# kowaalczyk/reformer-tts

Measured on AMD Instinct MI355X. Metric: mel-frames/sec training step, LJSpeech-shape batch, higher is better.
Workload: dtype bf16; 1 GPU; config/baseline.yml full Reformer-TTS training step (enc 3 / dec 3 layers, d=512, LSH 8 rounds, buckets 64/128), per-GPU batch 12, text 200->256, mel 1024x80; global_batch=12, parallelism=dp1, reversible_recompute=full

## Files before the change

### include/rtts.h

```cpp
#ifndef RTTS_H
#define RTTS_H

#include <stdint.h>

#ifdef __cplusplus
extern "C" {
#endif

#define RTTS_VERSION 1

int rtts_version(void);
const char* rtts_last_error(void);

int rtts_lsh_hash_sort(const void* qk, int64_t ld_qk, const float* rotations, int rot_rows,
                       int B, int H, int T, int dh, int n_hashes, int bucket_size,
                       int32_t* buckets, int32_t* st, int32_t* undo, void* stream);
int rtts_lsh_hash_sort_launches(int T);

int rtts_lsh_hash_sort_hf(const void* qk, int64_t ld_qk, const float* rotations, const uint8_t* mask,
                          int B, int H, int T, int dh, int n_hashes, int chunk, int n_buckets,
                          int32_t* buckets, int32_t* st, int32_t* undo, void* stream);

int rtts_lsh_attn_fwd(const void* qk, const void* v, int64_t ld, const int32_t* st, const uint8_t* mask,
                      int B, int H, int T, int dh, int n_hashes, int bucket_size, int causal,
                      void* o, float* lse, float drop_p, uint32_t drop_seed, const uint32_t* seed_dev, void* stream);
int rtts_lsh_attn_fwd_run_length(int B, int H, int T, int n_hashes, int bucket_size);
int rtts_debug_set_walk(int fwd_run, int bwd_run);

int rtts_lsh_combine_fwd(const void* o, const float* lse, int B, int H, int T, int dh, int n_hashes,
                         void* out, int64_t ld_out, float* lse_tot, void* stream);

int rtts_lsh_bwd_qk_slots(void);
int rtts_lsh_attn_bwd_run_length(int B, int H, int T, int n_hashes, int bucket_size);
int rtts_lsh_bwd_delta(const void* out, int64_t ld_out, const void* dout, int64_t ld_dout,
                       int B, int H, int T, int dh, float* delta, void* stream);
int rtts_lsh_attn_bwd(const void* qk, const void* v, int64_t ld, const int32_t* st, const uint8_t* mask,
                      const void* dout, int64_t ld_dout, const float* lse_tot, const float* delta,
                      int B, int H, int T, int dh, int n_hashes, int bucket_size, int causal,
                      void* dqk_part, void* dv_part, uint8_t* row_flags, float drop_p, uint32_t drop_seed, const uint32_t* seed_dev,
                      void* stream);
int rtts_lsh_bwd_reduce(const void* dqk_part, const void* dv_part, int B, int H, int T, int dh, int n_hashes,
                        void* dqk, void* dv, int64_t ld_d, const uint8_t* row_flags, void* stream);

int rtts_grad_clip_scale(const float* grads, int64_t n, float grad_mult, float max_norm, float* partial_ws,
                         float* scale_out, void* stream);
int rtts_adamw_step(float* params, const float* grads, float* exp_avg, float* exp_avg_sq, const uint8_t* decay_mask,
                    int64_t n, const float* scale, const float* hyper, float beta1, float beta2, float eps,
                    float weight_decay, void* bf16_mirror, void* stream);

int rtts_ln_fwd(const float* x, const float* gamma, const float* beta, void* xn, float* mean, float* rstd,
                int M, int d, void* stream);
int rtts_ln_bwd(const void* dxn, const float* x, const float* mean, const float* rstd, const float* gamma,
                float* dx_io, float* dgamma, float* dbeta, float* partial_ws, int M, int d,
                void* dyb_next, float* partial_next, float drop_p, uint32_t seed, const uint32_t* seed_dev, void* stream);
int rtts_ln_bwd_to(const void* dxn, const float* x, const float* mean, const float* rstd, const float* gamma, const float* dx_in,
                   float* dx_out, float* dgamma, float* dbeta, float* partial_ws, int M, int d,
                   void* dyb_next, float* partial_next, float drop_p, uint32_t seed, const uint32_t* seed_dev, void* stream);
int rtts_ln_bwd_join(const void* dxn, const float* x, const float* mean, const float* rstd, const float* gamma, const float* dx_in,
                     const float* addend, float* dx_out, float* dgamma, float* dbeta, float* partial_ws, int M, int d,
                     void* dyb_next, float* partial_next, float drop_p, uint32_t seed, const uint32_t* seed_dev, void* stream);
int rtts_cast_colsum(const float* dy, void* dyb, float* dbias, float* partial_ws, int M, int d, float drop_p, uint32_t seed,
                     const uint32_t* seed_dev, const float* scale_dev, void* stream);
int rtts_colsum_bf16(void* dh, const void* h, int64_t ld, float* dbias, float* partial_ws, int M, int d,
                     int relu_gate, float gate_scale, void* gated_out, void* stream);
#define RTTS_COLSUM_MAX_GROUP 48
typedef struct {
    const float* partial;
    float* out;
    int32_t nrows, n;
    int32_t ld, reserved;
} rtts_colsum_job;
int rtts_colsum_partial_rows(int M);
int rtts_colsum_final_grouped(const rtts_colsum_job* jobs, int n, void* stream);
int rtts_residual_epilogue(const float* x, const void* g, const float* bias, float sign, float* y,
                           int64_t M, int d, float drop_p, uint32_t seed, const uint32_t* seed_dev, void* stream);
int rtts_residual_ln(float* x, const void* g, const float* bias, float sign, const float* gamma, const float* beta,
                     void* xn, float* mean, float* rstd, int M, int d, float drop_p, uint32_t seed, const uint32_t* seed_dev,
                     float* y, void* stream);
int rtts_sum_streams(const float* a, const float* b, int64_t n, float* out, void* out_bf16, void* stream);
int rtts_bias_act(void* h, const float* bias, int64_t M, int d, int relu, void* stream);
int rtts_cast_f32_bf16(const float* src, void* dst, int64_t n, void* stream);

int rtts_xattn_key_chunks(int Tk);
int rtts_xattn_fwd(const void* q, int64_t ld_q, const void* kv, int64_t ld_kv, const uint8_t* kvalid,
                   int B, int H, int Tq, int Tk, int dh, void* o, int64_t ld_o, float* lse,
                   float drop_p, uint32_t seed, const uint32_t* seed_dev, void* stream);
int rtts_xattn_bwd(const void* q, int64_t ld_q, const void* kv, int64_t ld_kv, const uint8_t* kvalid,
                   const void* dout, int64_t ld_dout, const float* lse, const float* delta,
                   int B, int H, int Tq, int Tk, int dh, void* dq, int64_t ld_dq, void* dkv_part,
                   float drop_p, uint32_t seed, const uint32_t* seed_dev, void* dq_chunks, void* stream);
int rtts_sum_slabs(const void* part, int nslabs, int64_t n, void* out, void* stream);
int rtts_xattn_probs_mean(const void* q, int64_t ld_q, const void* kv, int64_t ld_kv, const uint8_t* kvalid,
                          const float* lse, int B, int H, int Tq, int Tk, int dh, float* a, int64_t ld_a, void* stream);

int rtts_conv1d_k5(const void* x, int64_t ldx, const void* wp, int64_t ldw, int transposed, int M, int C_out, int C_in,
                   void* y, int64_t ldy, const float* bias, int out_f32, void* stream);
int rtts_to_halo(const void* src, int64_t ld_src, int64_t src_batch_stride, int C_src, int src_f32, int B, int L, int halo, int C,
                 void* dst, int lead, int64_t rows, void* stream);
int rtts_conv_w_perm(const float* w, int Co, int Ci, int CP, void* wp, void* stream);
int rtts_conv_dw_unperm(const float* dwp, int Co, int Ci, int CP, float* dw, void* stream);
#define RTTS_CONV_PERM_MAX_GROUP 8
typedef struct {
    const float* w;
    void* wp;
    int32_t Co, Ci, CP, reserved;
} rtts_conv_perm_job;
int rtts_conv_w_perm_grouped(const rtts_conv_perm_job* jobs, int n, void* stream);
int rtts_conv_dw_unperm_grouped(const rtts_conv_perm_job* jobs, int n, void* stream);
int rtts_conv1d_k5_moments(const void* x, int64_t ldx, const void* wp, int64_t ldw, int M, int C_out, int C_in, void* y, int64_t ldy,
                           int B, int L, int halo, float* partial, void* stream);
int rtts_bn_stats_from_partials(const float* partial, int nrows, int B, int L, int C, float* mean, float* rstd, float* run_mean,
                                float* run_var, const float* mean_shift, int64_t* num_batches, void* stream);
int rtts_bn_stats(const float* y, int B, int L, int halo, int C, float* mean, float* rstd, float* run_mean, float* run_var,
                  const float* mean_shift, int64_t* num_batches, float* partial_ws, void* stream);
int rtts_bn_act_fwd(const float* y, const float* mean, const float* rstd, const float* gamma, const float* beta, int act,
                    float drop_p, uint32_t seed, const uint32_t* seed_dev, int B, int L, int halo, int C, void* z, int z_halo,
                    int z_lead, int64_t z_rows, void* stream);
int rtts_bn_act_bwd(const float* y, const void* dz, int dz_halo, const float* mean, const float* rstd, const float* gamma,
                    const float* beta, int act, float drop_p, uint32_t seed, const uint32_t* seed_dev, int B, int L, int halo, int C,
                    void* dy, int dy_lead, int64_t dy_rows, float* dgamma, float* dbeta, float* partial_ws, void* stream);
int rtts_bn_moments(const float* y, int B, int L, int halo, int C, float* moments, float* partial_ws, void* stream);
int rtts_bn_from_moments(const float* moments, int64_t count, int C, float* mean, float* rstd, float* run_mean, float* run_var,
                         const float* mean_shift, int64_t* num_batches, void* stream);
int rtts_bn_act_bwd_sums(const float* y, const void* dz, int dz_halo, const float* mean, const float* rstd, const float* gamma,
                         const float* beta, int act, float drop_p, uint32_t seed, const uint32_t* seed_dev, int B, int L, int halo, int C,
                         float* sums, float* dgamma, float* dbeta, float* partial_ws, void* stream);
int rtts_bn_act_bwd_apply(const float* y, const void* dz, int dz_halo, const float* mean, const float* rstd, const float* gamma,
                          const float* beta, int act, float drop_p, uint32_t seed, const uint32_t* seed_dev, int B, int L, int halo, int C,
                          const float* sums, int64_t count, void* dy, int dy_lead, int64_t dy_rows, void* stream);
int rtts_tts_loss(const float* raw, const float* post, int64_t ld_mel, const float* tgt, const float* mask, const float* stop,
                  int64_t ld_stop, const float* tstop, int rows, int NM, int kind, float pos_weight, float w_raw, float w_post,
                  float w_stop, float* d_raw, float* d_post, int64_t ld_grad, float* d_stop, float* losses, float* partial_ws,
                  int padded_len, int valid_len, const float* res, int64_t ld_res, int halo, int dpost_lead, int64_t dpost_rows,
                  int64_t tgt_batch_stride, const int32_t* valid_len_dev, int64_t mask_batch_stride, int64_t tstop_batch_stride,
                  void* stream);
int rtts_heads_grad(const float* d_raw, const float* d_post, int dpost_lead, const float* dx0, int64_t ld_dx0, const float* d_stop,
                    int B, int L, int halo, int n_mels, int width, float* dheads, const float* scale_dev, void* stream);

#define RTTS_SEGMENTS_MAX 12
enum { RTTS_SEG_COPY_F32 = 0, RTTS_SEG_COPY_BF16 = 1, RTTS_SEG_ADD_F32 = 2, RTTS_SEG_CAST_F32_BF16 = 3 };
typedef struct {
    void* dst;
    const void* src;
    int64_t count;
    int32_t kind, reserved;
} rtts_segment;
int rtts_segments(const rtts_segment* jobs, int n, void* stream);

int rtts_pe_add(const void* y, const float* table, const float* alpha, float drop_p, uint32_t seed, const uint32_t* seed_dev,
                int T, int64_t M, int d, float* out, void* stream);
int rtts_pe_dalpha(const float* dy, const float* table, float drop_p, uint32_t seed, const uint32_t* seed_dev, int T, int64_t M,
                   int d, float* dalpha, float* partial_ws, void* stream);
int rtts_relu_drop(void* h, float drop_p, uint32_t seed, const uint32_t* seed_dev, int64_t n, void* stream);

int rtts_batch_masks(const int64_t* phonemes, int64_t ph_stride, int B, int Lp, int Lp_pad, const float* loss_mask, int64_t lm_bstride,
                     int64_t lm_rstride, int Lm, int Lm_pad, int n_mels, int64_t* pad_phonemes, uint8_t* phoneme_mask,
                     uint8_t* phoneme_pad_mask, uint8_t* frame_mask, void* stream);

int rtts_embedding_fwd(const int64_t* ids, const float* E, int rows, int C, int n_embeddings, float drop_p, uint32_t seed,
                       const uint32_t* seed_dev, float* out, void* stream);
int rtts_embedding_bwd(const int64_t* ids, const float* dx, int rows, int C, int n_embeddings, int padding_idx, float* dE,
                       float drop_p, uint32_t seed, const uint32_t* seed_dev, void* stream);
int rtts_embedding_bwd_strided(const int64_t* ids, const float* dx, int64_t batch_stride, int64_t row_stride, int L, int rows, int C,
                               int n_embeddings, int padding_idx, float* dE, float drop_p, uint32_t seed, const uint32_t* seed_dev, void* stream);

int rtts_gemm_tn(const void* a, int64_t lda, const void* b, int64_t ldb, int M, int N, int K, float* c, int64_t ldc,
                 int accumulate, float* slab_ws, int64_t slab_ws_floats, void* stream);

#define RTTS_GEMM_TN_MAX_GROUP 16
typedef struct {
    const void* a; int64_t lda;
    const void* b; int64_t ldb;
    float* c;      int64_t ldc;
    int32_t M, N, K, accumulate;
} rtts_gemm_tn_problem;
int rtts_gemm_tn_grouped(const rtts_gemm_tn_problem* problems, int n, float* slab_ws, int64_t slab_ws_floats, void* stream);

int rtts_gemm_nt(const void* a, int64_t lda, const void* w, int64_t ldw, int w_is_kn, int M, int N, int K, void* c,
                 int64_t ldc, const float* bias, int epilogue, const void* gate, int64_t ldg, float* colsum_partial,
                 void* stream);
int rtts_gemm_nt_partial_rows(int M, int N);
typedef struct {
    const void* a; int64_t lda;
    const void* w; int64_t ldw;
    void* c; int64_t ldc;
    const float* bias;
    const void* aux; int64_t ld_aux;
    float* aux_out;
    int32_t M, N, K, epilogue;
    int32_t T, H, accumulate, reserved;
} rtts_gemm_nt_problem;
#define RTTS_GEMM_NT_MAX_GROUP 4
int rtts_gemm_nt_grouped(const rtts_gemm_nt_problem* problems, int n, int w_is_kn, void* stream);
int rtts_debug_set_gemm_mode(int mode);
int64_t rtts_gemm_nt_gate_words(int M, int N);
int rtts_gemm_nt_gated(const void* a, int64_t lda, const void* w, int64_t ldw, int w_is_kn, int M, int N, int K, void* c,
                       int64_t ldc, const float* bias, int epilogue, uint64_t* gate_words, float* colsum_partial, void* stream);

int rtts_peak_copy(const void* src, void* dst, int64_t bytes, void* stream);
int rtts_comm_probe(const void* src, void* dst, int64_t bytes, int workgroups, int sleep, void* stream);
int rtts_debug_stamp(void* buf, int slot, void* stream);
int rtts_peak_mfma(float* sink, int workgroups, int iters, void* stream);

int rtts_sw_depthwise_k3(const float* x, const float* w, const float* bias, int B, int L, int C, void* y,
                         const float* edge_lo, const float* edge_hi, void* stream);
int rtts_sw_gate(const void* pw, const void* cond, int64_t ld_cond, int cond_offset, int upsample, int B, int L, int Lm, int C,
                 void* acts, void* stream);
int rtts_sw_coupling_inv(float* audio, int64_t ld_audio, const float* wn_out, int64_t rows, int half, void* stream);
int rtts_sw_depthwise_k3_seg(const float* x, const float* w, const float* bias, const int32_t* moff, int nseg, int upsample,
                             int64_t rows, int C, void* y, const float* edge_lo, const float* edge_hi, void* stream);
int rtts_sw_pack_mel(const float* mel, int64_t stride_b, int64_t stride_c, int64_t stride_t, int L, int n_mel, const int32_t* moff,
                     int nseg, int64_t rows, float* dst, int64_t ld_dst, void* stream);
int rtts_sw_coupling_inv1x1(const float* audio, int64_t ld_audio, const float* wn_out, int64_t ld_wn, const float* winv, int n,
                            int64_t rows, float* out, int64_t ld_out, void* stream);
int rtts_sw_coupling_fwd1x1(const float* x, int64_t ld_x, const float* wn_out, int64_t ld_wn, const float* w, int n_in, int n_early,
                            int64_t rows, float* out, int64_t ld_out, float* z, int64_t ld_z, int z_col, float* ls_row, void* stream);
int rtts_sw_nll_reduce(const float* z, int64_t ld_z, int C, const float* ls_row, const int32_t* moff, int nseg, int upsample, int64_t L,
                       int64_t rows, double* out, void* stream);
int rtts_sw_pack_audio(const float* src, int64_t n_src, const int64_t* start, const int32_t* moff, int nseg, int upsample, int C,
                       int64_t rows, float* dst, void* stream);
int rtts_sw_gate_bwd(const void* pw, const void* cond, int64_t ld_cond, int cond_offset, int upsample, int B, int L, int Lm, int C,
                     const void* dacts, void* dpw, void* dcond, int64_t ld_dcond, void* stream);
int rtts_sw_dwbn_bwd_partial_floats(int64_t rows, int C);
int rtts_sw_dwbn_bwd_sums(const float* h, const void* dy, const float* mean, const float* rstd, const float* gamma, const float* beta,
                          const float* w, int B, int L, int C, float* sums, float* partial_ws, void* stream);
int rtts_sw_dwbn_bwd_apply(const float* h, const void* dy, const float* mean, const float* rstd, const float* gamma, const float* beta,
                           const float* w, const float* sums, int B, int L, int C, float* dh, void* stream);
int rtts_sw_boundary_bwd_blocks(int64_t rows);
int rtts_sw_boundary_bwd(const float* x, int64_t ld_x, const float* wn_out, int64_t ld_wn, const float* w, int n_in, int n_early,
                         int64_t rows, const float* dout, int64_t ld_dout, const float* z, int64_t ld_z, int z_col, float z_scale,
                         float inv_n, float* dx, int64_t ld_dx, float* dwn, int64_t ld_dwn, float* dw, float* partial_ws, void* stream);
#define RTTS_SW_FACTOR_MAX_COUNT 16
#define RTTS_SW_FACTOR_MAX_N 128
int rtts_sw_inv1x1_factor(const float* const* w, const int* n, int count, float* const* winv, double* slogdet, void* stream);
int rtts_sw_draw_segments(const void* audio, int in_format, int64_t n_audio, const int64_t* sample_offsets, const float* mel,
                          int64_t ld_mel, const int64_t* frame_offsets, int n_utt, const int32_t* order, int n_order,
                          const int64_t* state, uint32_t seed, const int32_t* picks_in, int B, int seg_frames, int hop, int C,
                          int n_mel, float* audio_rows, float* mel_rows, int64_t ld_mel_rows, int32_t* picks_out, void* stream);
int rtts_tts_collate(const float* mel, int64_t ld_mel, const int64_t* frame_offsets, const int32_t* phoneme_ids, int64_t n_phonemes,
                     const int64_t* phoneme_offsets, int n_utt, const int32_t* ids, int B, int n_mel, int lm, int64_t* phonemes, int LP,
                     float* spectrogram_input, int R_in, int valid_in, float* spectrogram_target, int R_target, float* stop_tokens,
                     int R_stop, float* loss_mask, int R_mask, int32_t* valid_len, float noise_std, uint32_t seed, void* stream);
int rtts_infer_metrics_tiles(int lm);
int rtts_infer_metrics(const float* gen, int64_t gs_b, int64_t gs_mel, int64_t gs_t, int L, const int64_t* gen_stop, const float* truth,
                       int64_t ts_mel, int64_t ts_t, int64_t truth_frames, const int64_t* frame_offsets, int n_utt, const int32_t* ids,
                       const int64_t* starts, const int32_t* lengths, int B, int n_mel, int lm, int longest, double* partials, double* sse,
                       double* stop_err, double* totals, void* stream);

int64_t rtts_mel_frames(int64_t n_samples, int hop);
int rtts_mel_spectrogram(const float* audio, const int64_t* sample_offsets_host, const int64_t* frame_offsets_host,
                         const int64_t* sample_offsets, const int64_t* frame_offsets, int nseg, const float* dft_basis,
                         const float* mel_basis, int n_fft, int hop, int n_mels, int power, float clip, float* out, int64_t ld_out,
                         void* stream);

#define RTTS_RESAMPLE_TILE 1024
#define RTTS_RESAMPLE_MAX_TAPS 256
#define RTTS_RESAMPLE_MAX_TABLE (1 << 22)
int64_t rtts_resample_len(int64_t n_samples, int orig, int new_);
int rtts_resample(const void* audio, int in_format, int channels, const int64_t* in_offsets_host, const int64_t* out_offsets_host,
                  const int64_t* in_offsets, const int64_t* out_offsets, int nseg, const int32_t* first, const float* taps_table,
                  int orig_red, int new_red, int taps, float* out, void* stream);

#ifdef __cplusplus
}
#endif
#endif
```

### reformer-tts_amd/_lib.py

```python
from __future__ import annotations

import ctypes as C
import os

_HERE = os.path.dirname(os.path.abspath(__file__))
LIB_PATH = os.environ.get("RTTS_LIB") or os.path.join(_HERE, "lib", "librtts_hip.so")

_i64, _i32, _vp, _f32, _u32 = C.c_int64, C.c_int, C.c_void_p, C.c_float, C.c_uint32

class GemmTnProblem(C.Structure):
    _fields_ = [("a", _vp), ("lda", _i64), ("b", _vp), ("ldb", _i64), ("c", _vp), ("ldc", _i64),
                ("M", C.c_int32), ("N", C.c_int32), ("K", C.c_int32), ("accumulate", C.c_int32)]


GEMM_TN_MAX_GROUP = 16


class GemmNtProblem(C.Structure):
    _fields_ = [("a", _vp), ("lda", _i64), ("w", _vp), ("ldw", _i64), ("c", _vp), ("ldc", _i64), ("bias", _vp), ("aux", _vp),
                ("ld_aux", _i64), ("aux_out", _vp), ("M", C.c_int32), ("N", C.c_int32), ("K", C.c_int32), ("epilogue", C.c_int32),
                ("T", C.c_int32), ("H", C.c_int32), ("accumulate", C.c_int32), ("reserved", C.c_int32)]


GEMM_NT_MAX_GROUP = 4


class ColsumJob(C.Structure):
    _fields_ = [("partial", _vp), ("out", _vp), ("nrows", C.c_int32), ("n", C.c_int32), ("ld", C.c_int32), ("reserved", C.c_int32)]


COLSUM_MAX_GROUP = 48


class Segment(C.Structure):
    _fields_ = [("dst", _vp), ("src", _vp), ("count", C.c_int64), ("kind", C.c_int32), ("reserved", C.c_int32)]


SEGMENTS_MAX = 12
SEG_COPY_F32, SEG_COPY_BF16, SEG_ADD_F32, SEG_CAST_F32_BF16 = 0, 1, 2, 3


class ConvPermJob(C.Structure):
    _fields_ = [("w", _vp), ("wp", _vp), ("Co", C.c_int32), ("Ci", C.c_int32), ("CP", C.c_int32), ("reserved", C.c_int32)]


CONV_PERM_MAX_GROUP = 8
SW_FACTOR_MAX_COUNT, SW_FACTOR_MAX_N = 16, 128

SIGNATURES = {
    "rtts_lsh_hash_sort": [_vp, _i64, _vp, _i32, _i32, _i32, _i32, _i32, _i32, _i32, _vp, _vp, _vp, _vp],
    "rtts_lsh_attn_fwd": [_vp, _vp, _i64, _vp, _vp, _i32, _i32, _i32, _i32, _i32, _i32, _i32, _vp, _vp, _f32, _u32, _vp, _vp],
    "rtts_lsh_hash_sort_launches": [_i32],
    "rtts_lsh_hash_sort_hf": [_vp, _i64, _vp, _vp, _i32, _i32, _i32, _i32, _i32, _i32, _i32, _vp, _vp, _vp, _vp],
    "rtts_lsh_attn_fwd_run_length": [_i32, _i32, _i32, _i32, _i32],
    "rtts_lsh_combine_fwd": [_vp, _vp, _i32, _i32, _i32, _i32, _i32, _vp, _i64, _vp, _vp],
    "rtts_lsh_bwd_delta": [_vp, _i64, _vp, _i64, _i32, _i32, _i32, _i32, _vp, _vp],
    "rtts_lsh_attn_bwd": [_vp, _vp, _i64, _vp, _vp, _vp, _i64, _vp, _vp, _i32, _i32, _i32, _i32, _i32, _i32, _i32, _vp, _vp, _vp, _f32, _u32, _vp,
                          _vp],
    "rtts_lsh_bwd_qk_slots": [],
    "rtts_lsh_attn_bwd_run_length": [_i32, _i32, _i32, _i32, _i32],
    "rtts_debug_set_walk": [_i32, _i32],
    "rtts_lsh_bwd_reduce": [_vp, _vp, _i32, _i32, _i32, _i32, _i32, _vp, _vp, _i64, _vp, _vp],
    "rtts_grad_clip_scale": [_vp, _i64, _f32, _f32, _vp, _vp, _vp],
    "rtts_ln_fwd": [_vp, _vp, _vp, _vp, _vp, _vp, _i32, _i32, _vp],
    "rtts_ln_bwd": [_vp, _vp, _vp, _vp, _vp, _vp, _vp, _vp, _vp, _i32, _i32, _vp, _vp, _f32, _u32, _vp, _vp],
    "rtts_ln_bwd_to": [_vp, _vp, _vp, _vp, _vp, _vp, _vp, _vp, _vp, _vp, _i32, _i32, _vp, _vp, _f32, _u32, _vp, _vp],
    "rtts_ln_bwd_join": [_vp, _vp, _vp, _vp, _vp, _vp, _vp, _vp, _vp, _vp, _vp, _i32, _i32, _vp, _vp, _f32, _u32, _vp, _vp],
    "rtts_cast_colsum": [_vp, _vp, _vp, _vp, _i32, _i32, _f32, _u32, _vp, _vp, _vp],
    "rtts_colsum_bf16": [_vp, _vp, _i64, _vp, _vp, _i32, _i32, _i32, _f32, _vp, _vp],
    "rtts_sum_streams": [_vp, _vp, _i64, _vp, _vp, _vp],
    "rtts_residual_epilogue": [_vp, _vp, _vp, _f32, _vp, _i64, _i32, _f32, _u32, _vp, _vp],
    "rtts_colsum_partial_rows": [_i32],
    "rtts_colsum_final_grouped": [C.POINTER(ColsumJob), _i32, _vp],
    "rtts_residual_ln": [_vp, _vp, _vp, _f32, _vp, _vp, _vp, _vp, _vp, _i32, _i32, _f32, _u32, _vp, _vp, _vp],
    "rtts_bias_act": [_vp, _vp, _i64, _i32, _i32, _vp],
    "rtts_cast_f32_bf16": [_vp, _vp, _i64, _vp],
    "rtts_xattn_fwd": [_vp, _i64, _vp, _i64, _vp, _i32, _i32, _i32, _i32, _i32, _vp, _i64, _vp, _f32, _u32, _vp, _vp],
    "rtts_xattn_bwd": [_vp, _i64, _vp, _i64, _vp, _vp, _i64, _vp, _vp, _i32, _i32, _i32, _i32, _i32, _vp, _i64, _vp, _f32, _u32, _vp, _vp, _vp],
    "rtts_xattn_key_chunks": [_i32],
    "rtts_xattn_probs_mean": [_vp, _i64, _vp, _i64, _vp, _vp, _i32, _i32, _i32, _i32, _i32, _vp, _i64, _vp],
    "rtts_sum_slabs": [_vp, _i32, _i64, _vp, _vp],
    "rtts_conv1d_k5": [_vp, _i64, _vp, _i64, _i32, _i32, _i32, _i32, _vp, _i64, _vp, _i32, _vp],
    "rtts_to_halo": [_vp, _i64, _i64, _i32, _i32, _i32, _i32, _i32, _i32, _vp, _i32, _i64, _vp],
    "rtts_heads_grad": [_vp, _vp, _i32, _vp, _i64, _vp, _i32, _i32, _i32, _i32, _i32, _vp, _vp, _vp],
    "rtts_segments": [C.POINTER(Segment), _i32, _vp],
    "rtts_conv_w_perm": [_vp, _i32, _i32, _i32, _vp, _vp],
    "rtts_conv_dw_unperm": [_vp, _i32, _i32, _i32, _vp, _vp],
    "rtts_conv_w_perm_grouped": [C.POINTER(ConvPermJob), _i32, _vp],
    "rtts_conv_dw_unperm_grouped": [C.POINTER(ConvPermJob), _i32, _vp],
    "rtts_conv1d_k5_moments": [_vp, _i64, _vp, _i64, _i32, _i32, _i32, _vp, _i64, _i32, _i32, _i32, _vp, _vp],
    "rtts_bn_stats_from_partials": [_vp, _i32, _i32, _i32, _i32, _vp, _vp, _vp, _vp, _vp, _vp, _vp],
    "rtts_bn_stats": [_vp, _i32, _i32, _i32, _i32, _vp, _vp, _vp, _vp, _vp, _vp, _vp, _vp],
    "rtts_bn_act_fwd": [_vp, _vp, _vp, _vp, _vp, _i32, _f32, _u32, _vp, _i32, _i32, _i32, _i32, _vp, _i32, _i32, _i64, _vp],
    "rtts_bn_act_bwd": [_vp, _vp, _i32, _vp, _vp, _vp, _vp, _i32, _f32, _u32, _vp, _i32, _i32, _i32, _i32, _vp, _i32, _i64, _vp, _vp, _vp, _vp],
    "rtts_bn_moments": [_vp, _i32, _i32, _i32, _i32, _vp, _vp, _vp],
    "rtts_bn_from_moments": [_vp, _i64, _i32, _vp, _vp, _vp, _vp, _vp, _vp, _vp],
    "rtts_bn_act_bwd_sums": [_vp, _vp, _i32, _vp, _vp, _vp, _vp, _i32, _f32, _u32, _vp, _i32, _i32, _i32, _i32, _vp, _vp, _vp, _vp, _vp],
    "rtts_bn_act_bwd_apply": [_vp, _vp, _i32, _vp, _vp, _vp, _vp, _i32, _f32, _u32, _vp, _i32, _i32, _i32, _i32, _vp, _i64, _vp, _i32, _i64, _vp],
    "rtts_tts_loss": [_vp, _vp, _i64, _vp, _vp, _vp, _i64, _vp, _i32, _i32, _i32, _f32, _f32, _f32, _f32, _vp, _vp, _i64, _vp, _vp, _vp, _i32, _i32,
                      _vp, _i64, _i32, _i32, _i64, _i64, _vp, _i64, _i64, _vp],
    "rtts_pe_add": [_vp, _vp, _vp, _f32, _u32, _vp, _i32, _i64, _i32, _vp, _vp],
    "rtts_debug_stamp": [_vp, _i32, _vp],
    "rtts_batch_masks": [_vp, _i64, _i32, _i32, _i32, _vp, _i64, _i64, _i32, _i32, _i32, _vp, _vp, _vp, _vp, _vp],
    "rtts_pe_dalpha": [_vp, _vp, _f32, _u32, _vp, _i32, _i64, _i32, _vp, _vp, _vp],
    "rtts_relu_drop": [_vp, _f32, _u32, _vp, _i64, _vp],
    "rtts_embedding_bwd": [_vp, _vp, _i32, _i32, _i32, _i32, _vp, _f32, _u32, _vp, _vp],
    "rtts_embedding_bwd_strided": [_vp, _vp, _i64, _i64, _i32, _i32, _i32, _i32, _i32, _vp, _f32, _u32, _vp, _vp],
    "rtts_embedding_fwd": [_vp, _vp, _i32, _i32, _i32, _f32, _u32, _vp, _vp, _vp],
    "rtts_gemm_tn": [_vp, _i64, _vp, _i64, _i32, _i32, _i32, _vp, _i64, _i32, _vp, _i64, _vp],
    "rtts_gemm_tn_grouped": [C.POINTER(GemmTnProblem), _i32, _vp, _i64, _vp],
    "rtts_gemm_nt": [_vp, _i64, _vp, _i64, _i32, _i32, _i32, _i32, _vp, _i64, _vp, _i32, _vp, _i64, _vp, _vp],
    "rtts_gemm_nt_partial_rows": [_i32, _i32],
    "rtts_gemm_nt_grouped": [C.POINTER(GemmNtProblem), _i32, _i32, _vp],
    "rtts_debug_set_gemm_mode": [_i32],
    "rtts_gemm_nt_gate_words": [_i32, _i32],
    "rtts_gemm_nt_gated": [_vp, _i64, _vp, _i64, _i32, _i32, _i32, _i32, _vp, _i64, _vp, _i32, _vp, _vp, _vp],
    "rtts_peak_copy": [_vp, _vp, _i64, _vp],
    "rtts_comm_probe": [_vp, _vp, _i64, _i32, _i32, _vp],
    "rtts_peak_mfma": [_vp, _i32, _i32, _vp],
    "rtts_sw_depthwise_k3": [_vp, _vp, _vp, _i32, _i32, _i32, _vp, _vp, _vp, _vp],
    "rtts_sw_gate": [_vp, _vp, _i64, _i32, _i32, _i32, _i32, _i32, _i32, _vp, _vp],
    "rtts_sw_coupling_inv": [_vp, _i64, _vp, _i64, _i32, _vp],
    "rtts_sw_depthwise_k3_seg": [_vp, _vp, _vp, _vp, _i32, _i32, _i64, _i32, _vp, _vp, _vp, _vp],
    "rtts_sw_pack_mel": [_vp, _i64, _i64, _i64, _i32, _i32, _vp, _i32, _i64, _vp, _i64, _vp],
    "rtts_sw_coupling_inv1x1": [_vp, _i64, _vp, _i64, _vp, _i32, _i64, _vp, _i64, _vp],
    "rtts_sw_coupling_fwd1x1": [_vp, _i64, _vp, _i64, _vp, _i32, _i32, _i64, _vp, _i64, _vp, _i64, _i32, _vp, _vp],
    "rtts_sw_nll_reduce": [_vp, _i64, _i32, _vp, _vp, _i32, _i32, _i64, _i64, _vp, _vp],
    "rtts_sw_pack_audio": [_vp, _i64, _vp, _vp, _i32, _i32, _i32, _i64, _vp, _vp],
    "rtts_sw_gate_bwd": [_vp, _vp, _i64, _i32, _i32, _i32, _i32, _i32, _i32, _vp, _vp, _vp, _i64, _vp],
    "rtts_sw_dwbn_bwd_partial_floats": [_i64, _i32],
    "rtts_sw_dwbn_bwd_sums": [_vp, _vp, _vp, _vp, _vp, _vp, _vp, _i32, _i32, _i32, _vp, _vp, _vp],
    "rtts_sw_dwbn_bwd_apply": [_vp, _vp, _vp, _vp, _vp, _vp, _vp, _vp, _i32, _i32, _i32, _vp, _vp],
    "rtts_sw_boundary_bwd_blocks": [_i64],
    "rtts_sw_boundary_bwd": [_vp, _i64, _vp, _i64, _vp, _i32, _i32, _i64, _vp, _i64, _vp, _i64, _i32, _f32, _f32, _vp, _i64, _vp, _i64, _vp, _vp,
                             _vp],
    "rtts_sw_inv1x1_factor": [C.POINTER(_vp), C.POINTER(_i32), _i32, C.POINTER(_vp), _vp, _vp],
    "rtts_sw_draw_segments": [_vp, _i32, _i64, _vp, _vp, _i64, _vp, _i32, _vp, _i32, _vp, _u32, _vp, _i32, _i32, _i32, _i32, _i32, _vp, _vp, _i64,
                              _vp, _vp],
    "rtts_tts_collate": [_vp, _i64, _vp, _vp, _i64, _vp, _i32, _vp, _i32, _i32, _i32, _vp, _i32, _vp, _i32, _i32, _vp, _i32, _vp, _i32, _vp, _i32,
                         _vp, _f32, _u32, _vp],
    "rtts_infer_metrics_tiles": [_i32],
    "rtts_infer_metrics": [_vp, _i64, _i64, _i64, _i32, _vp, _vp, _i64, _i64, _i64, _vp, _i32, _vp, _vp, _vp, _i32, _i32, _i32, _i32, _vp, _vp, _vp,
                           _vp, _vp],
    "rtts_adamw_step": [_vp, _vp, _vp, _vp, _vp, _i64, _vp, _vp, _f32, _f32, _f32, _f32, _vp, _vp],
    "rtts_mel_frames": [_i64, _i32],
    "rtts_mel_spectrogram": [_vp, C.POINTER(_i64), C.POINTER(_i64), _vp, _vp, _i32, _vp, _vp, _i32, _i32, _i32, _i32, _f32, _vp, _i64, _vp],
    "rtts_resample_len": [_i64, _i32, _i32],
    "rtts_resample": [_vp, _i32, _i32, C.POINTER(_i64), C.POINTER(_i64), _vp, _vp, _i32, _vp, _vp, _i32, _i32, _i32, _vp, _vp],
}

_lib = None


class RttsError(RuntimeError):
    pass


_NOTED = set()
PATHS_LEFT = []


def note_general_path(where: str, reason: str) -> None:
    key = (where, reason)
    if key in _NOTED:
        return
    _NOTED.add(key)
    PATHS_LEFT.append(key)
    import logging
    logging.getLogger("reformer_tts_amd").warning("%s: general (eager) path instead of the explicit HIP executor -- %s", where, reason)


def log_once(key: str, message: str) -> None:
    if key in _NOTED:
        return
    _NOTED.add(key)
    import logging
    logging.getLogger("reformer_tts_amd").warning("%s", message)


def load() -> C.CDLL:
    global _lib
    if _lib is None:
        if not os.path.exists(LIB_PATH):
            raise RttsError(
                f"{LIB_PATH} is missing: build it with `python reformer-tts_amd/build.py` "
                "(or __graft_entry__.build()). There is no CPU fallback for the HIP path.")
        import torch
        lib = C.CDLL(LIB_PATH)
        lib.rtts_version.restype = C.c_int
        lib.rtts_last_error.restype = C.c_char_p
        for name, args in SIGNATURES.items():
            fn = getattr(lib, name)
            fn.argtypes = args
            fn.restype = C.c_int
        lib.rtts_gemm_nt_gate_words.restype = C.c_int64
        lib.rtts_mel_frames.restype = C.c_int64
        lib.rtts_resample_len.restype = C.c_int64
        _lib = lib
        fw, bw = os.environ.get("RTTS_LSH_FWD_WALK"), os.environ.get("RTTS_LSH_BWD_WALK")
        if fw is not None or bw is not None:
            _WALK[:] = [-1 if fw is None else int(fw), -1 if bw is None else int(bw)]
            lib.rtts_debug_set_walk(*_WALK)
        gs = os.environ.get("RTTS_GEMM_STORE")
        if gs is not None:
            lib.rtts_debug_set_gemm_mode(10 + int(gs))
    return _lib


_WALK = [-1, -1]


class forced_walk:

    def __init__(self, fwd=None, bwd=None):
        self.want = (fwd, bwd)

    def __enter__(self):
        self.old = list(_WALK)
        new = [o if w is None else int(w) for o, w in zip(self.old, self.want)]
        call("rtts_debug_set_walk", *new)
        _WALK[:] = new
        return self

    def __exit__(self, *exc):
        call("rtts_debug_set_walk", *self.old)
        _WALK[:] = self.old
        return False


def call(name: str, *args) -> None:
    lib = load()
    rc = getattr(lib, name)(*args)
    if rc != 0:
        raise RttsError(lib.rtts_last_error().decode() or f"{name} failed with code {rc}")
```

### reformer-tts_amd/csrc/edges.hip

```cpp
#include "rtts_common.h"

#define ED_THREADS 256
#define ED_PBLOCKS 256

#define ed_drop rtts_drop_keep

struct EdHalo {
    int B, L, P, H;
};
__device__ __forceinline__ bool ed_valid(const EdHalo& g, long long m, int& b, int& t) {
    if (m < 0 || m >= (long long)g.B * g.P) return false;
    const int mi = (int)m;
    int q = (int)((float)mi * __builtin_amdgcn_rcpf((float)g.P));
    int r = mi - q * g.P;
    if (r < 0) { --q; r += g.P; }
    if (r >= g.P) { ++q; r -= g.P; }
    b = q;
    t = r - g.H;
    return (unsigned)t < (unsigned)g.L;
}
__device__ __forceinline__ void ed_row_col(unsigned e, int C, int cshift, unsigned& row, int& c) {
    if (cshift >= 0) {
        row = e >> cshift;
        c = (int)(e & (unsigned)(C - 1));
    } else {
        row = e / (unsigned)C;
        c = (int)(e - row * (unsigned)C);
    }
}
static inline int ed_cshift(int C) { return (C & (C - 1)) == 0 ? __builtin_ctz((unsigned)C) : -1; }
__device__ __forceinline__ float ed_tanh(float x) {
    const float t = __builtin_amdgcn_exp2f(x * 2.885390081777927f);
    return 1.f - 2.f * __builtin_amdgcn_rcpf(t + 1.f);
}
static inline EdHalo ed_halo(int B, int L, int halo) { return EdHalo{B, L, L + 2 * halo, halo}; }

template <bool SRC_F32>
__global__ __launch_bounds__(ED_THREADS) void to_halo_kernel(const void* __restrict__ src, int64_t ld_src, int64_t bs_src, int C_src, EdHalo g, int C,
                                                             int lead, long long rows, bf16_t* __restrict__ dst) {
    const int pieces = C / 8;
    const size_t total = (size_t)rows * pieces;
    for (size_t i = (size_t)blockIdx.x * blockDim.x + threadIdx.x; i < total; i += (size_t)gridDim.x * blockDim.x) {
        const int pc = (int)(i % pieces);
        const long long r = (long long)(i / pieces);
        int b, t;
        uint4 o = make_uint4(0, 0, 0, 0);
        if (pc * 8 < C_src && ed_valid(g, r - lead, b, t)) {
            const size_t soff = (size_t)b * bs_src + (size_t)t * ld_src;
            if (SRC_F32) {
                const float* p = reinterpret_cast<const float*>(src) + soff + pc * 8;
                const float4 v0 = *reinterpret_cast<const float4*>(p), v1 = *reinterpret_cast<const float4*>(p + 4);
                o.x = pack_bf16x2(v0.x, v0.y); o.y = pack_bf16x2(v0.z, v0.w);
                o.z = pack_bf16x2(v1.x, v1.y); o.w = pack_bf16x2(v1.z, v1.w);
            } else {
                o = *reinterpret_cast<const uint4*>(reinterpret_cast<const bf16_t*>(src) + soff + pc * 8);
            }
        }
        *reinterpret_cast<uint4*>(dst + (size_t)r * C + pc * 8) = o;
    }
}

__global__ __launch_bounds__(ED_THREADS) void conv_w_perm_kernel(const float* __restrict__ w, int Co, int Ci, int CP, bf16_t* __restrict__ wp) {
    const size_t total = (size_t)Co * 5 * CP;
    for (size_t i = (size_t)blockIdx.x * blockDim.x + threadIdx.x; i < total; i += (size_t)gridDim.x * blockDim.x) {
        const int ci = (int)(i % CP), k = (int)((i / CP) % 5), co = (int)(i / ((size_t)CP * 5));
        wp[i] = ci < Ci ? f32_to_bf16(w[((size_t)co * Ci + ci) * 5 + k]) : (bf16_t)0;
    }
}
struct CwGroup {
    rtts_conv_perm_job j[RTTS_CONV_PERM_MAX_GROUP];
    int blk_start[RTTS_CONV_PERM_MAX_GROUP + 1];
    int n;
};
__global__ __launch_bounds__(ED_THREADS) void conv_w_perm_grouped_kernel(const CwGroup g) {
    int ji = 0;
#pragma unroll
    for (int i = 1; i < RTTS_CONV_PERM_MAX_GROUP; ++i)
        if (i < g.n && (int)blockIdx.x >= g.blk_start[i]) ji = i;
    const rtts_conv_perm_job& J = g.j[ji];
    const int Co = J.Co, Ci = J.Ci, CP = J.CP;
    const float* __restrict__ w = J.w;
    bf16_t* __restrict__ wp = (bf16_t*)J.wp;
    const size_t total = (size_t)Co * CP;
    const size_t nthr = (size_t)(g.blk_start[ji + 1] - g.blk_start[ji]) * blockDim.x;
    for (size_t i = (size_t)((int)blockIdx.x - g.blk_start[ji]) * blockDim.x + threadIdx.x; i < total; i += nthr) {
        const int ci = (int)(i % CP), co = (int)(i / CP);
        float t[5] = {0.f, 0.f, 0.f, 0.f, 0.f};
        if (ci < Ci) {
            const float* src = w + ((size_t)co * Ci + ci) * 5;
#pragma unroll
            for (int k = 0; k < 5; ++k) t[k] = src[k];
        }
#pragma unroll
        for (int k = 0; k < 5; ++k) wp[((size_t)co * 5 + k) * CP + ci] = f32_to_bf16(t[k]);
    }
}
__global__ __launch_bounds__(ED_THREADS) void conv_dw_unperm_grouped_kernel(const CwGroup g) {
    int ji = 0;
#pragma unroll
    for (int i = 1; i < RTTS_CONV_PERM_MAX_GROUP; ++i)
        if (i < g.n && (int)blockIdx.x >= g.blk_start[i]) ji = i;
    const rtts_conv_perm_job& J = g.j[ji];
    const int Co = J.Co, Ci = J.Ci, CP = J.CP;
    const float* __restrict__ dwp = J.w;
    float* __restrict__ dw = (float*)J.wp;
    const size_t total = (size_t)Co * Ci;
    const size_t nthr = (size_t)(g.blk_start[ji + 1] - g.blk_start[ji]) * blockDim.x;
    for (size_t i = (size_t)((int)blockIdx.x - g.blk_start[ji]) * blockDim.x + threadIdx.x; i < total; i += nthr) {
        const int ci = (int)(i % Ci), co = (int)(i / Ci);
        float* dst = dw + i * 5;
#pragma unroll
        for (int k = 0; k < 5; ++k) dst[k] += dwp[((size_t)co * 5 + k) * CP + ci];
    }
}
__global__ __launch_bounds__(ED_THREADS) void conv_dw_unperm_kernel(const float* __restrict__ dwp, int Co, int Ci, int CP, float* __restrict__ dw) {
    const size_t total = (size_t)Co * Ci * 5;
    for (size_t i = (size_t)blockIdx.x * blockDim.x + threadIdx.x; i < total; i += (size_t)gridDim.x * blockDim.x) {
        const int k = (int)(i % 5), ci = (int)((i / 5) % Ci), co = (int)(i / ((size_t)Ci * 5));
        dw[i] += dwp[((size_t)co * 5 + k) * CP + ci];
    }
}

template <int MODE>
__global__ __launch_bounds__(ED_THREADS) void col_partial_kernel(const float* __restrict__ y, const bf16_t* __restrict__ dz,
                                                                 const float* __restrict__ mean, const float* __restrict__ rstd,
                                                                 const float* __restrict__ gamma, const float* __restrict__ beta, int act,
                                                                 uint32_t seed, const uint32_t* __restrict__ seed_dev, uint32_t thresh, float dscale, EdHalo g,
                                                                 int dz_halo, int C, float* __restrict__ partial) {
    if (seed_dev) seed += seed_dev[0];
    const int M = g.B * g.P;
    const int cq = threadIdx.x & 63, rl = threadIdx.x >> 6;
    const int c = blockIdx.y * 256 + cq * 4;
    __shared__ float red[2][4][256];
    float sa[4] = {0, 0, 0, 0}, sb[4] = {0, 0, 0, 0};
    if (c < C) {
        float mu[4] = {0, 0, 0, 0}, rs[4] = {1, 1, 1, 1}, ga[4] = {1, 1, 1, 1}, be[4] = {0, 0, 0, 0};
        if (MODE == 1) {
#pragma unroll
            for (int j = 0; j < 4; ++j) { mu[j] = mean[c + j]; rs[j] = rstd[c + j]; ga[j] = gamma[c + j]; be[j] = beta[c + j]; }
        }
        for (int row = blockIdx.x * 4 + rl; row < M; row += gridDim.x * 4) {
            int sb_, st_;
            if (!ed_valid(g, row, sb_, st_)) continue;
            const float4 yv = *reinterpret_cast<const float4*>(y + (size_t)row * C + c);
            const float yy[4] = {yv.x, yv.y, yv.z, yv.w};
            if (MODE == 0) {
#pragma unroll
                for (int j = 0; j < 4; ++j) { sa[j] += yy[j]; sb[j] = __builtin_fmaf(yy[j], yy[j], sb[j]); }
            } else {
                const size_t drow = dz_halo ? (size_t)row : (size_t)sb_ * g.L + st_;
                const uint2 dv = *reinterpret_cast<const uint2*>(dz + drow * C + c);
                const float dd[4] = {__uint_as_float(dv.x << 16), __uint_as_float(dv.x & 0xffff0000u), __uint_as_float(dv.y << 16),
                                     __uint_as_float(dv.y & 0xffff0000u)};
#pragma unroll
                for (int j = 0; j < 4; ++j) {
                    const float yh = (yy[j] - mu[j]) * rs[j];
                    const float pre = __builtin_fmaf(yh, ga[j], be[j]);
                    float da;
                    if (act == 1) da = pre > 0.f ? 1.f : 0.f;
                    else { const float th = ed_tanh(pre); da = 1.f - th * th; }
                    const float g = dd[j] * da * (thresh ? ed_drop(seed, (uint32_t)((size_t)row * C + c + j), thresh, dscale) : 1.f);
                    sa[j] += g;
                    sb[j] = __builtin_fmaf(g, yh, sb[j]);
                }
            }
        }
    }
#pragma unroll
    for (int j = 0; j < 4; ++j) { red[0][rl][cq * 4 + j] = sa[j]; red[1][rl][cq * 4 + j] = sb[j]; }
    __syncthreads();
    const int t = threadIdx.x;
    if (blockIdx.y * 256 + t < C) {
        float* prow = partial + (size_t)blockIdx.x * 2 * C;
        prow[blockIdx.y * 256 + t] = (red[0][0][t] + red[0][1][t]) + (red[0][2][t] + red[0][3][t]);
        prow[C + blockIdx.y * 256 + t] = (red[1][0][t] + red[1][1][t]) + (red[1][2][t] + red[1][3][t]);
    }
}

#define ED_FIN_WAVES 16
__device__ __forceinline__ void ed_reduce_partials(const float* __restrict__ partial, int nrows, int C, int c, float& s, float& q,
                                                   float (*red)[ED_FIN_WAVES][64]) {
    const int lane = threadIdx.x & 63, wave = threadIdx.x >> 6;
    float a = 0.f, b = 0.f;
    if (c < C) {
        float va[16], vb[16];
        for (int r0 = wave; r0 < nrows; r0 += ED_FIN_WAVES * 16) {
#pragma unroll
            for (int u = 0; u < 16; ++u) {
                const int r = r0 + u * ED_FIN_WAVES;
                va[u] = r < nrows ? partial[(size_t)r * 2 * C + c] : 0.f;
                vb[u] = r < nrows ? partial[(size_t)r * 2 * C + C + c] : 0.f;
            }
#pragma unroll
            for (int u = 0; u < 16; ++u) {
                a += va[u];
                b += vb[u];
            }
        }
    }
    red[0][wave][lane] = a;
    red[1][wave][lane] = b;
    __syncthreads();
    s = 0.f;
    q = 0.f;
#pragma unroll
    for (int w = 0; w < ED_FIN_WAVES; ++w) {
        s += red[0][w][lane];
        q += red[1][w][lane];
    }
}

__global__ __launch_bounds__(64 * ED_FIN_WAVES) void bn_finalize_stats_kernel(const float* __restrict__ partial, int nrows, int M, int C,
                                                                       float* __restrict__ mean, float* __restrict__ rstd,
                                                                       float* __restrict__ run_mean, float* __restrict__ run_var,
                                                                       const float* __restrict__ mean_shift, long long* __restrict__ num_batches) {
    __shared__ float red[2][ED_FIN_WAVES][64];
    const int c = blockIdx.x * 64 + (threadIdx.x & 63);
    float s, q;
    ed_reduce_partials(partial, nrows, C, c, s, q, red);
    if (num_batches && blockIdx.x == 0 && threadIdx.x == 0) num_batches[0] += 1;
    if (threadIdx.x >= 64 || c >= C) return;
    const float mu = s / M;
    const float var = fmaxf(q / M - mu * mu, 0.f);
    mean[c] = mu;
    rstd[c] = rsqrtf(var + 1e-5f);
    if (run_mean) {
        run_mean[c] = 0.9f * run_mean[c] + 0.1f * (mu + (mean_shift ? mean_shift[c] : 0.f));
        run_var[c] = 0.9f * run_var[c] + 0.1f * var * ((float)M / (float)(M > 1 ? M - 1 : 1));
    }
}

__global__ __launch_bounds__(64 * ED_FIN_WAVES) void bn_finalize_bwd_kernel(const float* __restrict__ partial, int nrows, int C,
                                                                     float* __restrict__ sums, float* __restrict__ dgamma,
                                                                     float* __restrict__ dbeta) {
    __shared__ float red[2][ED_FIN_WAVES][64];
    const int c = blockIdx.x * 64 + (threadIdx.x & 63);
    float s, q;
    ed_reduce_partials(partial, nrows, C, c, s, q, red);
    if (threadIdx.x >= 64 || c >= C) return;
    sums[c] = s;
    sums[C + c] = q;
    dbeta[c] += s;
    dgamma[c] += q;
}

__global__ __launch_bounds__(64 * ED_FIN_WAVES) void bn_moments_kernel(const float* __restrict__ partial, int nrows, int C, float* __restrict__ moments) {
    __shared__ float red[2][ED_FIN_WAVES][64];
    const int c = blockIdx.x * 64 + (threadIdx.x & 63);
    float s, q;
    ed_reduce_partials(partial, nrows, C, c, s, q, red);
    if (threadIdx.x >= 64 || c >= C) return;
    moments[c] = s;
    moments[C + c] = q;
}
__global__ void bn_from_moments_kernel(const float* __restrict__ moments, float count, int C, float* __restrict__ mean, float* __restrict__ rstd,
                                       float* __restrict__ run_mean, float* __restrict__ run_var, const float* __restrict__ mean_shift,
                                       long long* __restrict__ num_batches) {
    const int c = blockIdx.x * blockDim.x + threadIdx.x;
    if (num_batches && c == 0) num_batches[0] += 1;
    if (c >= C) return;
    if (count <= 0.f) count = moments[2 * C];
    const float mu = moments[c] / count;
    const float var = fmaxf(moments[C + c] / count - mu * mu, 0.f);
    mean[c] = mu;
    rstd[c] = rsqrtf(var + 1e-5f);
    if (run_mean) {
        run_mean[c] = 0.9f * run_mean[c] + 0.1f * (mu + (mean_shift ? mean_shift[c] : 0.f));
        run_var[c] = 0.9f * run_var[c] + 0.1f * var * (count / (count > 1.f ? count - 1.f : 1.f));
    }
}

__global__ __launch_bounds__(ED_THREADS) void bn_act_fwd_kernel(const float* __restrict__ y, const float* __restrict__ mean,
                                                                const float* __restrict__ rstd, const float* __restrict__ gamma,
                                                                const float* __restrict__ beta, int act, uint32_t seed, const uint32_t* __restrict__ seed_dev,
                                                                uint32_t thresh, float dscale, EdHalo g, int z_halo, int z_lead, size_t n4, int C,
                                                                int cshift, bf16_t* __restrict__ z) {
    if (seed_dev) seed += seed_dev[0];
    for (size_t i = (size_t)blockIdx.x * blockDim.x + threadIdx.x; i < n4; i += (size_t)gridDim.x * blockDim.x) {
        unsigned zrow;
        int c;
        ed_row_col((unsigned)i * 4u, C, cshift, zrow, c);
        const long long zr = (long long)zrow;
        long long ym;
        bool ok = true;
        if (z_halo) {
            int b, t;
            ym = zr - z_lead;
            ok = ed_valid(g, ym, b, t);
        } else {
            const long long b = zr / g.L;
            ym = b * g.P + g.H + (zr - b * g.L);
        }
        uint2 pk = make_uint2(0u, 0u);
        if (ok) {
            const size_t e = (size_t)ym * C + c;
            const float4 yv = *reinterpret_cast<const float4*>(y + e);
            const float yy[4] = {yv.x, yv.y, yv.z, yv.w};
            const float4 m4 = *reinterpret_cast<const float4*>(mean + c), r4 = *reinterpret_cast<const float4*>(rstd + c);
            const float4 g4 = *reinterpret_cast<const float4*>(gamma + c), b4 = *reinterpret_cast<const float4*>(beta + c);
            const float mu[4] = {m4.x, m4.y, m4.z, m4.w}, rs[4] = {r4.x, r4.y, r4.z, r4.w};
            const float ga[4] = {g4.x, g4.y, g4.z, g4.w}, be[4] = {b4.x, b4.y, b4.z, b4.w};
            float o[4];
#pragma unroll
            for (int j = 0; j < 4; ++j) {
                const float pre = __builtin_fmaf((yy[j] - mu[j]) * rs[j], ga[j], be[j]);
                float a = act == 1 ? fmaxf(pre, 0.f) : ed_tanh(pre);
                if (thresh) a *= ed_drop(seed, (uint32_t)(e + j), thresh, dscale);
                o[j] = a;
            }
            pk.x = pack_bf16x2(o[0], o[1]);
            pk.y = pack_bf16x2(o[2], o[3]);
        }
        reinterpret_cast<uint2*>(z)[i] = pk;
    }
}

__global__ __launch_bounds__(ED_THREADS) void bn_act_bwd_apply_kernel(const float* __restrict__ y, const bf16_t* __restrict__ dz,
                                                                      const float* __restrict__ mean, const float* __restrict__ rstd,
                                                                      const float* __restrict__ gamma, const float* __restrict__ beta, int act,
                                                                      uint32_t seed, const uint32_t* __restrict__ seed_dev, uint32_t thresh, float dscale,
                                                                      const float* __restrict__ sums, float inv_m, EdHalo g, int dz_halo, int dy_lead,
                                                                      size_t n4, int C, int cshift, bf16_t* __restrict__ dy) {
    if (seed_dev) seed += seed_dev[0];
    if (inv_m < 0.f) inv_m = 1.f / sums[2 * C];
    for (size_t i = (size_t)blockIdx.x * blockDim.x + threadIdx.x; i < n4; i += (size_t)gridDim.x * blockDim.x) {
        unsigned drow_;
        int c;
        ed_row_col((unsigned)i * 4u, C, cshift, drow_, c);
        const long long ym = (long long)drow_ - dy_lead;
        int b, t;
        uint2 pk = make_uint2(0u, 0u);
        if (ed_valid(g, ym, b, t)) {
            const size_t e = (size_t)ym * C + c;
            const float4 yv = *reinterpret_cast<const float4*>(y + e);
            const size_t drow = dz_halo ? (size_t)ym : (size_t)b * g.L + t;
            const uint2 dv = *reinterpret_cast<const uint2*>(dz + drow * C + c);
            const float yy[4] = {yv.x, yv.y, yv.z, yv.w};
            const float dd[4] = {__uint_as_float(dv.x << 16), __uint_as_float(dv.x & 0xffff0000u), __uint_as_float(dv.y << 16),
                                 __uint_as_float(dv.y & 0xffff0000u)};
            const float4 m4 = *reinterpret_cast<const float4*>(mean + c), r4 = *reinterpret_cast<const float4*>(rstd + c);
            const float4 g4 = *reinterpret_cast<const float4*>(gamma + c), b4 = *reinterpret_cast<const float4*>(beta + c);
            const float4 s0 = *reinterpret_cast<const float4*>(sums + c), s1 = *reinterpret_cast<const float4*>(sums + C + c);
            const float mu4[4] = {m4.x, m4.y, m4.z, m4.w}, rs4[4] = {r4.x, r4.y, r4.z, r4.w};
            const float ga4[4] = {g4.x, g4.y, g4.z, g4.w}, be4[4] = {b4.x, b4.y, b4.z, b4.w};
            const float sa4[4] = {s0.x, s0.y, s0.z, s0.w}, sb4[4] = {s1.x, s1.y, s1.z, s1.w};
            float o[4];
#pragma unroll
            for (int j = 0; j < 4; ++j) {
                const float rs = rs4[j], ga = ga4[j];
                const float yh = (yy[j] - mu4[j]) * rs;
                const float pre = __builtin_fmaf(yh, ga, be4[j]);
                float da;
                if (act == 1) da = pre > 0.f ? 1.f : 0.f;
                else { const float th = ed_tanh(pre); da = 1.f - th * th; }
                const float gg = dd[j] * da * (thresh ? ed_drop(seed, (uint32_t)(e + j), thresh, dscale) : 1.f);
                o[j] = ga * rs * (gg - sa4[j] * inv_m - yh * sb4[j] * inv_m);
            }
            pk.x = pack_bf16x2(o[0], o[1]);
            pk.y = pack_bf16x2(o[2], o[3]);
        }
        reinterpret_cast<uint2*>(dy)[i] = pk;
    }
}

__global__ __launch_bounds__(ED_THREADS) void tts_loss_kernel(const float* __restrict__ raw, const float* __restrict__ post, int64_t ld_mel,
                                                              const float* __restrict__ tgt, const float* __restrict__ mask,
                                                              const float* __restrict__ stop, int64_t ld_stop, const float* __restrict__ tstop,
                                                              int rows, int NM, int kind, float pos_weight, float w_raw, float w_post,
                                                              float w_stop, float* __restrict__ d_raw, float* __restrict__ d_post,
                                                              int64_t ld_grad, float* __restrict__ d_stop, float* __restrict__ partial,
                                                              int Lp, int Lv, const float* __restrict__ res, int64_t ld_res, int hp, int dp_lead,
                                                              long long dp_rows, long long tgt_bs, const int* __restrict__ lv_dev,
                                                              long long mask_bs, long long tstop_bs, int vec4) {
    if (lv_dev) Lv = min(max(lv_dev[0], 1), Lv);
    const int PH = Lp + 2 * hp;
    float s_raw = 0.f, s_post = 0.f, s_stop = 0.f;
    const size_t nel = (size_t)rows * NM;
    const size_t vrows = (size_t)(rows / Lp) * Lv;
    const float inv_el = 1.f / ((float)vrows * NM), inv_rows = 1.f / (float)vrows;
    if (vec4) {
        const unsigned NQ = (unsigned)NM / 4, nq = (unsigned)rows * NQ;
        for (unsigned i = blockIdx.x * blockDim.x + threadIdx.x; i < nq; i += gridDim.x * blockDim.x) {
            const unsigned row = i / NQ, c = (i % NQ) * 4;
            const unsigned t = row % (unsigned)Lp, bi = row / (unsigned)Lp;
            const size_t hrow = (size_t)bi * PH + hp + t;
            const size_t prow = (size_t)dp_lead + hrow;
            float4 gr = make_float4(0.f, 0.f, 0.f, 0.f), gp = gr;
            if ((int)t < Lv) {
                const float4 mk = *reinterpret_cast<const float4*>(mask + (size_t)bi * mask_bs + (size_t)t * NM + c);
                const float4 tg = *reinterpret_cast<const float4*>(tgt + (size_t)bi * tgt_bs + (size_t)t * NM + c);
                const float4 rv = *reinterpret_cast<const float4*>(raw + (size_t)row * ld_mel + c);
                float4 pv;
                if (res) {
                    const float4 rs = *reinterpret_cast<const float4*>(res + hrow * ld_res + c);
                    pv = make_float4(rv.x + rs.x, rv.y + rs.y, rv.z + rs.z, rv.w + rs.w);
                } else {
                    pv = *reinterpret_cast<const float4*>(post + (size_t)row * ld_mel + c);
                }
                const float mkv[4] = {mk.x, mk.y, mk.z, mk.w}, tgv[4] = {tg.x, tg.y, tg.z, tg.w};
                const float rvv[4] = {rv.x, rv.y, rv.z, rv.w}, pvv[4] = {pv.x, pv.y, pv.z, pv.w};
                float grv[4], gpv[4];
#pragma unroll
                for (int e = 0; e < 4; ++e) {
                    const float r = rvv[e] * mkv[e] - tgv[e], p = pvv[e] * mkv[e] - tgv[e];
                    if (kind == 0) {
                        s_raw = __builtin_fmaf(r, r, s_raw);
                        s_post = __builtin_fmaf(p, p, s_post);
                        grv[e] = w_raw * 2.f * r * mkv[e] * inv_el;
                        gpv[e] = w_post * 2.f * p * mkv[e] * inv_el;
                    } else {
                        s_raw += fabsf(r);
                        s_post += fabsf(p);
                        grv[e] = w_raw * (r > 0.f ? 1.f : (r < 0.f ? -1.f : 0.f)) * mkv[e] * inv_el;
                        gpv[e] = w_post * (p > 0.f ? 1.f : (p < 0.f ? -1.f : 0.f)) * mkv[e] * inv_el;
                    }
                }
                gr = make_float4(grv[0], grv[1], grv[2], grv[3]);
                gp = make_float4(gpv[0], gpv[1], gpv[2], gpv[3]);
            }
            *reinterpret_cast<float4*>(d_raw + (size_t)row * ld_grad + c) = gr;
            *reinterpret_cast<float4*>(d_post + prow * ld_grad + c) = gp;
        }
    } else
    for (size_t i = (size_t)blockIdx.x * blockDim.x + threadIdx.x; i < nel; i += (size_t)gridDim.x * blockDim.x) {
        const size_t row = i / NM;
        const int c = (int)(i % NM);
        const int t = (int)(row % Lp);
        const size_t hrow = (row / Lp) * PH + hp + t;
        const size_t prow = (size_t)dp_lead + hrow;
        if (t >= Lv) {
            d_raw[row * ld_grad + c] = 0.f;
            d_post[prow * ld_grad + c] = 0.f;
            continue;
        }
        const float mk = mask[(row / Lp) * (size_t)mask_bs + (size_t)t * NM + c], tg = tgt[(row / Lp) * (size_t)tgt_bs + (size_t)t * NM + c];
        const float rv = raw[row * ld_mel + c];
        const float pv = res ? rv + res[hrow * ld_res + c] : post[row * ld_mel + c];
        const float r = rv * mk - tg, p = pv * mk - tg;
        if (kind == 0) {
            s_raw = __builtin_fmaf(r, r, s_raw);
            s_post = __builtin_fmaf(p, p, s_post);
            d_raw[row * ld_grad + c] = w_raw * 2.f * r * mk * inv_el;
            d_post[prow * ld_grad + c] = w_post * 2.f * p * mk * inv_el;
        } else {
            s_raw += fabsf(r);
            s_post += fabsf(p);
            d_raw[row * ld_grad + c] = w_raw * (r > 0.f ? 1.f : (r < 0.f ? -1.f : 0.f)) * mk * inv_el;
            d_post[prow * ld_grad + c] = w_post * (p > 0.f ? 1.f : (p < 0.f ? -1.f : 0.f)) * mk * inv_el;
        }
    }
    const int npad = (int)ld_grad - NM;
    for (size_t i = (size_t)blockIdx.x * blockDim.x + threadIdx.x; i < (size_t)rows * npad; i += (size_t)gridDim.x * blockDim.x) {
        const size_t row = i / npad;
        const int c = NM + (int)(i % npad);
        d_raw[row * ld_grad + c] = 0.f;
        d_post[((size_t)dp_lead + (row / Lp) * PH + hp + row % Lp) * ld_grad + c] = 0.f;
    }
    if (hp > 0) {
        const EdHalo g{rows / Lp, Lp, PH, hp};
        for (size_t i = (size_t)blockIdx.x * blockDim.x + threadIdx.x; i < (size_t)dp_rows * ld_grad; i += (size_t)gridDim.x * blockDim.x) {
            int b, t;
            if (!ed_valid(g, (long long)(i / ld_grad) - dp_lead, b, t)) d_post[i] = 0.f;
        }
    }
    for (size_t i = (size_t)blockIdx.x * blockDim.x + threadIdx.x; i < (size_t)rows; i += (size_t)gridDim.x * blockDim.x) {
        const int tt = (int)(i % Lp);
        if (tt >= Lv) {
            d_stop[i] = 0.f;
            continue;
        }
        const float x = stop[i * ld_stop], t = tstop[(i / Lp) * (size_t)tstop_bs + tt];
        const float lw = 1.f + (pos_weight - 1.f) * t;
        const float sp = fmaxf(-x, 0.f) + log1pf(expf(-fabsf(x)));
        s_stop += (1.f - t) * x + lw * sp;
        const float sig = 1.f / (1.f + expf(-x));
        d_stop[i] = w_stop * ((1.f - t) - lw * (1.f - sig)) * inv_rows;
    }
    __shared__ float red[3][ED_THREADS / 64];
#pragma unroll
    for (int o = 32; o > 0; o >>= 1) {
        s_raw += __shfl_xor(s_raw, o);
        s_post += __shfl_xor(s_post, o);
        s_stop += __shfl_xor(s_stop, o);
    }
    if ((threadIdx.x & 63) == 0) {
        red[0][threadIdx.x >> 6] = s_raw;
        red[1][threadIdx.x >> 6] = s_post;
        red[2][threadIdx.x >> 6] = s_stop;
    }
    __syncthreads();
    if (threadIdx.x < 3) partial[blockIdx.x * 3 + threadIdx.x] = red[threadIdx.x][0] + red[threadIdx.x][1] + red[threadIdx.x][2] + red[threadIdx.x][3];
}

__global__ void tts_loss_finalize_kernel(const float* __restrict__ partial, int nblocks, float inv_el, float inv_rows, float w_raw,
                                         float w_post, float w_stop, float* __restrict__ losses, const int* __restrict__ lv_dev, int batch,
                                         int Lv, int NM) {
    if (lv_dev) {
        const float vrows = (float)batch * (float)min(max(lv_dev[0], 1), Lv);
        inv_el = 1.f / (vrows * NM);
        inv_rows = 1.f / vrows;
    }
    float a = 0.f, b = 0.f, c = 0.f;
    for (int i = threadIdx.x; i < nblocks; i += 64) { a += partial[i * 3]; b += partial[i * 3 + 1]; c += partial[i * 3 + 2]; }
#pragma unroll
    for (int o = 32; o > 0; o >>= 1) {
        a += __shfl_xor(a, o);
        b += __shfl_xor(b, o);
        c += __shfl_xor(c, o);
    }
    if (threadIdx.x != 0) return;
    a *= inv_el; b *= inv_el; c *= inv_rows;
    losses[0] = w_raw * a + w_post * b + w_stop * c;
    losses[1] = a; losses[2] = b; losses[3] = c;
}

__global__ __launch_bounds__(ED_THREADS) void heads_grad_kernel(const float* __restrict__ d_raw, const float* __restrict__ d_post, int dp_lead,
                                                                const float* __restrict__ dx0, int64_t ld_dx0, const float* __restrict__ d_stop,
                                                                EdHalo g, int NM, int W, float* __restrict__ out,
                                                                const float* __restrict__ scale_dev) {
    const float up = scale_dev ? scale_dev[0] : 1.f;
    const size_t total = (size_t)g.B * g.L * (W / 4);
    for (size_t i = (size_t)blockIdx.x * blockDim.x + threadIdx.x; i < total; i += (size_t)gridDim.x * blockDim.x) {
        const int c = (int)(i % (W / 4)) * 4;
        const size_t row = i / (W / 4);
        const size_t hrow = (row / g.L) * g.P + g.H + row % g.L;
        const float4 a = *reinterpret_cast<const float4*>(d_raw + row * W + c);
        const float4 b = *reinterpret_cast<const float4*>(d_post + ((size_t)dp_lead + hrow) * W + c);
        float o[4] = {(a.x + b.x) * up, (a.y + b.y) * up, (a.z + b.z) * up, (a.w + b.w) * up};
#pragma unroll
        for (int j = 0; j < 4; ++j) {
            if (c + j < NM) o[j] += dx0[hrow * ld_dx0 + c + j];
            else if (c + j == NM) o[j] = d_stop[row] * up;
        }
        *reinterpret_cast<float4*>(out + row * W + c) = make_float4(o[0], o[1], o[2], o[3]);
    }
}

__global__ __launch_bounds__(ED_THREADS) void embedding_bwd_kernel(const int64_t* __restrict__ ids, const float* __restrict__ dx, int64_t bstride,
                                                                   int64_t rstride, int L, int rows,
                                                                   int C, int padding_idx, float* __restrict__ dE, uint32_t seed,
                                                                   const uint32_t* __restrict__ seed_dev, uint32_t thresh, float dscale) {
    __shared__ float red[4][64];
    const int id = blockIdx.x;
    const int lane = threadIdx.x & 63, wave = threadIdx.x >> 6;
    const int c = blockIdx.y * 64 + lane;
    if (id == padding_idx) return;
    if (thresh && seed_dev) seed += seed_dev[0];
    float acc = 0.f;
    for (int base = wave * 64; base < rows; base += 4 * 64) {
        const int r = base + lane;
        unsigned long long m = __ballot(r < rows && ids[r] == (int64_t)id);
        while (m) {
            const int rr = base + __builtin_ctzll(m);
            m &= m - 1;
            const int bb = rr / L;
            if (c < C) acc += dx[(size_t)bb * bstride + (size_t)(rr - bb * L) * rstride + c] * (thresh ? rtts_drop_keep(seed, (uint32_t)rr * C + c, thresh, dscale) : 1.f);
        }
    }
    red[wave][lane] = acc;
    __syncthreads();
    if (wave == 0 && c < C) dE[(size_t)id * C + c] += (red[0][lane] + red[1][lane]) + (red[2][lane] + red[3][lane]);
}

__global__ __launch_bounds__(ED_THREADS) void embedding_fwd_kernel(const int64_t* __restrict__ ids, const float* __restrict__ E, size_t n4, int C,
                                                                   int n_emb, uint32_t seed, const uint32_t* __restrict__ seed_dev, uint32_t thresh,
                                                                   float dscale, float* __restrict__ out) {
    if (thresh && seed_dev) seed += seed_dev[0];
    for (size_t i = (size_t)blockIdx.x * blockDim.x + threadIdx.x; i < n4; i += (size_t)gridDim.x * blockDim.x) {
        const size_t e = i * 4, row = e / C;
        const int c = (int)(e % C);
        long long id = ids[row];
        id = id < 0 ? 0 : (id >= n_emb ? n_emb - 1 : id);
        float4 v = *reinterpret_cast<const float4*>(E + (size_t)id * C + c);
        if (thresh) {
            v.x *= rtts_drop_keep(seed, (uint32_t)e, thresh, dscale);
            v.y *= rtts_drop_keep(seed, (uint32_t)e + 1, thresh, dscale);
            v.z *= rtts_drop_keep(seed, (uint32_t)e + 2, thresh, dscale);
            v.w *= rtts_drop_keep(seed, (uint32_t)e + 3, thresh, dscale);
        }
        reinterpret_cast<float4*>(out)[i] = v;
    }
}

struct SgJob {
    void* dst;
    const void* src;
    long long count;
    int kind, blk_start;
};
struct SgGroup {
    SgJob j[RTTS_SEGMENTS_MAX];
    int n;
};
__global__ __launch_bounds__(ED_THREADS) void segments_kernel(const SgGroup grp) {
    int ji = 0;
#pragma unroll 1
    for (int i = 1; i < grp.n; ++i)
        if ((int)blockIdx.x >= grp.j[i].blk_start) ji = i;
    const SgJob& J = grp.j[ji];
    const int nblk = (ji + 1 < grp.n ? grp.j[ji + 1].blk_start : (int)gridDim.x) - J.blk_start;
    for (long long i = (long long)((int)blockIdx.x - J.blk_start) * ED_THREADS + threadIdx.x; i < J.count; i += (long long)nblk * ED_THREADS) {
        switch (J.kind) {
        case RTTS_SEG_COPY_F32: reinterpret_cast<float*>(J.dst)[i] = reinterpret_cast<const float*>(J.src)[i]; break;
        case RTTS_SEG_COPY_BF16: reinterpret_cast<bf16_t*>(J.dst)[i] = reinterpret_cast<const bf16_t*>(J.src)[i]; break;
        case RTTS_SEG_ADD_F32: reinterpret_cast<float*>(J.dst)[i] += reinterpret_cast<const float*>(J.src)[i]; break;
        default: reinterpret_cast<bf16_t*>(J.dst)[i] = f32_to_bf16(reinterpret_cast<const float*>(J.src)[i]); break;
        }
    }
}

__global__ __launch_bounds__(ED_THREADS) void pe_add_kernel(const bf16_t* __restrict__ y, const float* __restrict__ table,
                                                            const float* __restrict__ alpha, uint32_t seed, const uint32_t* __restrict__ seed_dev,
                                                            uint32_t thresh, float dscale, int T, size_t n4, int d, float* __restrict__ out) {
    if (seed_dev) seed += seed_dev[0];
    const float a = alpha[0];
    for (size_t i = (size_t)blockIdx.x * blockDim.x + threadIdx.x; i < n4; i += (size_t)gridDim.x * blockDim.x) {
        const size_t e = i * 4;
        const int c = (int)(e % d);
        const int t = (int)((e / d) % T);
        const uint2 yv = reinterpret_cast<const uint2*>(y)[i];
        const float4 tv = *reinterpret_cast<const float4*>(table + (size_t)t * d + c);
        const float tt[4] = {tv.x, tv.y, tv.z, tv.w};
        const float yy[4] = {__uint_as_float(yv.x << 16), __uint_as_float(yv.x & 0xffff0000u), __uint_as_float(yv.y << 16),
                             __uint_as_float(yv.y & 0xffff0000u)};
        float o[4];
#pragma unroll
        for (int j = 0; j < 4; ++j)
            o[j] = yy[j] + a * tt[j] * (thresh ? ed_drop(seed, (uint32_t)(t * d + c + j), thresh, dscale) : 1.f);
        reinterpret_cast<float4*>(out)[i] = make_float4(o[0], o[1], o[2], o[3]);
    }
}

__global__ __launch_bounds__(ED_THREADS) void pe_dalpha_partial_kernel(const float* __restrict__ dy, const float* __restrict__ table,
                                                                       uint32_t seed, const uint32_t* __restrict__ seed_dev, uint32_t thresh, float dscale, int T,
                                                                       size_t n4, int d, float* __restrict__ partial) {
    if (seed_dev) seed += seed_dev[0];
    float s = 0.f;
    for (size_t i = (size_t)blockIdx.x * blockDim.x + threadIdx.x; i < n4; i += (size_t)gridDim.x * blockDim.x) {
        const size_t e = i * 4;
        const int c = (int)(e % d);
        const int t = (int)((e / d) % T);
        const float4 dv = reinterpret_cast<const float4*>(dy)[i];
        const float4 tv = *reinterpret_cast<const float4*>(table + (size_t)t * d + c);
        const float dd[4] = {dv.x, dv.y, dv.z, dv.w}, tt[4] = {tv.x, tv.y, tv.z, tv.w};
#pragma unroll
        for (int j = 0; j < 4; ++j)
            s = __builtin_fmaf(dd[j], tt[j] * (thresh ? ed_drop(seed, (uint32_t)(t * d + c + j), thresh, dscale) : 1.f), s);
    }
    __shared__ float red[ED_THREADS / 64];
#pragma unroll
    for (int o = 32; o > 0; o >>= 1) s += __shfl_xor(s, o);
    if ((threadIdx.x & 63) == 0) red[threadIdx.x >> 6] = s;
    __syncthreads();
    if (threadIdx.x == 0) partial[blockIdx.x] = (red[0] + red[1]) + (red[2] + red[3]);
}
__global__ void pe_dalpha_final_kernel(const float* __restrict__ partial, int n, float* __restrict__ dalpha) {
    float s = 0.f;
    for (int i = threadIdx.x; i < n; i += 64) s += partial[i];
#pragma unroll
    for (int o = 32; o > 0; o >>= 1) s += __shfl_xor(s, o);
    if (threadIdx.x == 0) dalpha[0] += s;
}

__global__ __launch_bounds__(ED_THREADS) void relu_drop_kernel(bf16_t* __restrict__ h, uint32_t seed, const uint32_t* __restrict__ seed_dev,
                                                               uint32_t thresh, float dscale, size_t n8) {
    if (seed_dev) seed += seed_dev[0];
    for (size_t i = (size_t)blockIdx.x * blockDim.x + threadIdx.x; i < n8; i += (size_t)gridDim.x * blockDim.x) {
        uint4 t = reinterpret_cast<uint4*>(h)[i];
        uint32_t u[4] = {t.x, t.y, t.z, t.w};
#pragma unroll
        for (int j = 0; j < 4; ++j) {
            float lo = fmaxf(__uint_as_float(u[j] << 16), 0.f), hi = fmaxf(__uint_as_float(u[j] & 0xffff0000u), 0.f);
            if (thresh) {
                lo *= ed_drop(seed, (uint32_t)(i * 8 + 2 * j), thresh, dscale);
                hi *= ed_drop(seed, (uint32_t)(i * 8 + 2 * j + 1), thresh, dscale);
            }
            u[j] = pack_bf16x2(lo, hi);
        }
        t.x = u[0]; t.y = u[1]; t.z = u[2]; t.w = u[3];
        reinterpret_cast<uint4*>(h)[i] = t;
    }
}

static inline unsigned ed_grid(size_t items) {
    size_t b = (items + ED_THREADS - 1) / ED_THREADS;
    if (b > 4096) b = 4096;
    if (b < 1) b = 1;
    return (unsigned)b;
}
static inline uint32_t ed_thresh(float p) { return p <= 0.f ? 0u : (uint32_t)((double)p * 4294967296.0); }

extern "C" int rtts_to_halo(const void* src, int64_t ld_src, int64_t src_batch_stride, int C_src, int src_f32, int B, int L, int halo, int C,
                            void* dst, int lead, int64_t rows, void* stream) {
    RTTS_ENTER(stream);
    RTTS_REQUIRE(src && dst && B > 0 && L > 0 && halo >= 0 && C > 0 && C % 8 == 0 && C_src > 0 && C_src % 8 == 0 && C_src <= C && ld_src >= C_src &&
                     ld_src % (src_f32 ? 4 : 8) == 0, "rtts_to_halo: bad arguments");
    if (src_batch_stride == 0) src_batch_stride = (int64_t)L * ld_src;
    RTTS_REQUIRE(src_batch_stride >= (int64_t)L * ld_src && src_batch_stride % (src_f32 ? 4 : 8) == 0,
                 "rtts_to_halo: src_batch_stride must cover L rows and keep 16-byte alignment");
    RTTS_REQUIRE(lead >= 0 && rows >= lead + (int64_t)B * (L + 2 * halo), "rtts_to_halo: dst has %lld rows, needs %lld", (long long)rows,
                 (long long)(lead + (int64_t)B * (L + 2 * halo)));
    const dim3 grid(ed_grid((size_t)rows * (C / 8)));
    if (src_f32)
        hipLaunchKernelGGL(to_halo_kernel<true>, grid, dim3(ED_THREADS), 0, (hipStream_t)stream, src, ld_src, src_batch_stride, C_src, ed_halo(B, L, halo), C,
                           lead, (long long)rows, (bf16_t*)dst);
    else
        hipLaunchKernelGGL(to_halo_kernel<false>, grid, dim3(ED_THREADS), 0, (hipStream_t)stream, src, ld_src, src_batch_stride, C_src, ed_halo(B, L, halo), C,
                           lead, (long long)rows, (bf16_t*)dst);
    RTTS_LAUNCH_CHECK("rtts_to_halo");
    return 0;
}

extern "C" int rtts_heads_grad(const float* d_raw, const float* d_post, int dpost_lead, const float* dx0, int64_t ld_dx0, const float* d_stop,
                               int B, int L, int halo, int n_mels, int width, float* dheads, const float* scale_dev, void* stream) {
    RTTS_ENTER(stream);
    RTTS_REQUIRE(d_raw && d_post && dx0 && d_stop && dheads && B > 0 && L > 0 && halo >= 0 && width % 4 == 0 && n_mels < width && dpost_lead >= 0,
                 "rtts_heads_grad: bad arguments");
    hipLaunchKernelGGL(heads_grad_kernel, dim3(ed_grid((size_t)B * L * (width / 4))), dim3(ED_THREADS), 0, (hipStream_t)stream, d_raw, d_post,
                       dpost_lead, dx0, ld_dx0, d_stop, ed_halo(B, L, halo), n_mels, width, dheads, scale_dev);
    RTTS_LAUNCH_CHECK("rtts_heads_grad");
    return 0;
}

extern "C" int rtts_conv_w_perm(const float* w, int Co, int Ci, int CP, void* wp, void* stream) {
    RTTS_ENTER(stream);
    RTTS_REQUIRE(w && wp && Co > 0 && Ci > 0 && CP >= Ci, "rtts_conv_w_perm: bad arguments");
    hipLaunchKernelGGL(conv_w_perm_kernel, dim3(ed_grid((size_t)Co * 5 * CP)), dim3(ED_THREADS), 0, (hipStream_t)stream, w, Co, Ci, CP, (bf16_t*)wp);
    RTTS_LAUNCH_CHECK("rtts_conv_w_perm");
    return 0;
}

extern "C" int rtts_conv_w_perm_grouped(const rtts_conv_perm_job* jobs, int n, void* stream) {
    RTTS_ENTER(stream);
    RTTS_REQUIRE(jobs && n > 0 && n <= RTTS_CONV_PERM_MAX_GROUP, "rtts_conv_w_perm_grouped: 1..%d jobs", RTTS_CONV_PERM_MAX_GROUP);
    CwGroup g;
    g.n = n;
    int blk = 0;
    for (int i = 0; i < n; ++i) {
        RTTS_REQUIRE(jobs[i].w && jobs[i].wp && jobs[i].Co > 0 && jobs[i].Ci > 0 && jobs[i].CP >= jobs[i].Ci, "rtts_conv_w_perm_grouped: bad job %d", i);
        g.j[i] = jobs[i];
        g.blk_start[i] = blk;
        blk += (int)ed_grid((size_t)jobs[i].Co * jobs[i].CP);
    }
    for (int i = n; i <= RTTS_CONV_PERM_MAX_GROUP; ++i) g.blk_start[i] = blk;
    hipLaunchKernelGGL(conv_w_perm_grouped_kernel, dim3(blk), dim3(ED_THREADS), 0, (hipStream_t)stream, g);
    RTTS_LAUNCH_CHECK("rtts_conv_w_perm_grouped");
    return 0;
}

extern "C" int rtts_conv_dw_unperm_grouped(const rtts_conv_perm_job* jobs, int n, void* stream) {
    RTTS_ENTER(stream);
    RTTS_REQUIRE(jobs && n > 0 && n <= RTTS_CONV_PERM_MAX_GROUP, "rtts_conv_dw_unperm_grouped: 1..%d jobs", RTTS_CONV_PERM_MAX_GROUP);
    CwGroup g;
    g.n = n;
    int blk = 0;
    for (int i = 0; i < n; ++i) {
        RTTS_REQUIRE(jobs[i].w && jobs[i].wp && jobs[i].Co > 0 && jobs[i].Ci > 0 && jobs[i].CP >= jobs[i].Ci, "rtts_conv_dw_unperm_grouped: bad job %d", i);
        g.j[i] = jobs[i];
        g.blk_start[i] = blk;
        blk += (int)ed_grid((size_t)jobs[i].Co * jobs[i].Ci);
    }
    for (int i = 1; i < n; ++i)
        for (int k = 0; k < i; ++k)
            RTTS_REQUIRE((const float*)jobs[i].wp >= (const float*)jobs[k].wp + (size_t)jobs[k].Co * jobs[k].Ci * 5 ||
                             (const float*)jobs[k].wp >= (const float*)jobs[i].wp + (size_t)jobs[i].Co * jobs[i].Ci * 5,
                         "rtts_conv_dw_unperm_grouped: jobs %d and %d add into overlapping gradients (launch them one after the other)", k, i);
    for (int i = n; i <= RTTS_CONV_PERM_MAX_GROUP; ++i) g.blk_start[i] = blk;
    hipLaunchKernelGGL(conv_dw_unperm_grouped_kernel, dim3(blk), dim3(ED_THREADS), 0, (hipStream_t)stream, g);
    RTTS_LAUNCH_CHECK("rtts_conv_dw_unperm_grouped");
    return 0;
}

extern "C" int rtts_conv_dw_unperm(const float* dwp, int Co, int Ci, int CP, float* dw, void* stream) {
    RTTS_ENTER(stream);
    RTTS_REQUIRE(dwp && dw && Co > 0 && Ci > 0 && CP >= Ci, "rtts_conv_dw_unperm: bad arguments");
    hipLaunchKernelGGL(conv_dw_unperm_kernel, dim3(ed_grid((size_t)Co * Ci * 5)), dim3(ED_THREADS), 0, (hipStream_t)stream, dwp, Co, Ci, CP, dw);
    RTTS_LAUNCH_CHECK("rtts_conv_dw_unperm");
    return 0;
}

static inline dim3 ed_col_grid(int M, int C) {
    int slabs = (M + 3) / 4;
    if (slabs > ED_PBLOCKS) slabs = ED_PBLOCKS;
    return dim3(slabs, (C + 255) / 256);
}

extern "C" int rtts_bn_stats(const float* y, int B, int L, int halo, int C, float* mean, float* rstd, float* run_mean, float* run_var,
                             const float* mean_shift, int64_t* num_batches, float* partial_ws, void* stream) {
    RTTS_ENTER(stream);
    RTTS_REQUIRE(y && mean && rstd && partial_ws && B > 0 && L > 0 && halo >= 0 && C > 0 && C % 4 == 0, "rtts_bn_stats: bad arguments");
    const EdHalo g = ed_halo(B, L, halo);
    const dim3 grid = ed_col_grid(B * g.P, C);
    hipLaunchKernelGGL((col_partial_kernel<0>), grid, dim3(ED_THREADS), 0, (hipStream_t)stream, y, (const bf16_t*)nullptr, (const float*)nullptr,
                       (const float*)nullptr, (const float*)nullptr, (const float*)nullptr, 0, 0u, (const uint32_t*)nullptr, 0u, 1.f, g, 1, C,
                       partial_ws);
    hipLaunchKernelGGL(bn_finalize_stats_kernel, dim3((C + 63) / 64), dim3(64 * ED_FIN_WAVES), 0, (hipStream_t)stream, partial_ws,
                       (int)grid.x, B * L, C, mean, rstd, run_mean, run_var, mean_shift, (long long*)num_batches);
    RTTS_LAUNCH_CHECK("rtts_bn_stats");
    return 0;
}

extern "C" int rtts_bn_stats_from_partials(const float* partial, int nrows, int B, int L, int C, float* mean, float* rstd, float* run_mean,
                                           float* run_var, const float* mean_shift, int64_t* num_batches, void* stream) {
    RTTS_ENTER(stream);
    RTTS_REQUIRE(partial && mean && rstd && nrows > 0 && B > 0 && L > 0 && C > 0 && C % 4 == 0, "rtts_bn_stats_from_partials: bad arguments");
    hipLaunchKernelGGL(bn_finalize_stats_kernel, dim3((C + 63) / 64), dim3(64 * ED_FIN_WAVES), 0, (hipStream_t)stream, partial, nrows, B * L, C, mean,
                       rstd, run_mean, run_var, mean_shift, (long long*)num_batches);
    RTTS_LAUNCH_CHECK("rtts_bn_stats_from_partials");
    return 0;
}

extern "C" int rtts_bn_act_fwd(const float* y, const float* mean, const float* rstd, const float* gamma, const float* beta, int act,
                               float drop_p, uint32_t seed, const uint32_t* seed_dev, int B, int L, int halo, int C, void* z, int z_halo,
                               int z_lead, int64_t z_rows, void* stream) {
    RTTS_ENTER(stream);
    RTTS_REQUIRE(y && mean && rstd && gamma && beta && z && B > 0 && L > 0 && halo >= 0 && C % 4 == 0 && (act == 1 || act == 2) && drop_p >= 0.f &&
                     drop_p < 1.f, "rtts_bn_act_fwd: bad arguments");
    const EdHalo g = ed_halo(B, L, halo);
    RTTS_REQUIRE(z_halo ? (halo > 0 && z_lead >= 0 && z_rows >= z_lead + (int64_t)B * g.P) : (z_rows == (int64_t)B * L && z_lead == 0),
                 "rtts_bn_act_fwd: z must be a halo array with room for B*(L+2*halo) rows behind its lead-in, or B*L plain rows");
    const size_t n4 = (size_t)z_rows * C / 4;
    RTTS_REQUIRE(n4 < (1ull << 30), "rtts_bn_act_fwd: more than 2^32 elements");
    hipLaunchKernelGGL(bn_act_fwd_kernel, dim3(ed_grid(n4)), dim3(ED_THREADS), 0, (hipStream_t)stream, y, mean, rstd, gamma, beta, act, seed, seed_dev,
                       ed_thresh(drop_p), 1.f / (1.f - drop_p), g, z_halo, z_lead, n4, C, ed_cshift(C), (bf16_t*)z);
    RTTS_LAUNCH_CHECK("rtts_bn_act_fwd");
    return 0;
}

extern "C" int rtts_bn_act_bwd(const float* y, const void* dz, int dz_halo, const float* mean, const float* rstd, const float* gamma,
                               const float* beta, int act, float drop_p, uint32_t seed, const uint32_t* seed_dev, int B, int L, int halo, int C,
                               void* dy, int dy_lead, int64_t dy_rows, float* dgamma, float* dbeta, float* partial_ws, void* stream) {
    RTTS_ENTER(stream);
    RTTS_REQUIRE(y && dz && mean && rstd && gamma && beta && dy && dgamma && dbeta && partial_ws && B > 0 && L > 0 && halo >= 0 && C % 4 == 0 &&
                     (act == 1 || act == 2), "rtts_bn_act_bwd: bad arguments");
    RTTS_REQUIRE(drop_p >= 0.f && drop_p < 1.f, "rtts_bn_act_bwd: drop_p must be in [0, 1)");
    const EdHalo g = ed_halo(B, L, halo);
    RTTS_REQUIRE(dy_lead >= 0 && dy_rows >= dy_lead + (int64_t)B * g.P,
                 "rtts_bn_act_bwd: dy needs room for B*(L+2*halo) rows behind its lead-in");
    const size_t n4 = (size_t)dy_rows * C / 4;
    RTTS_REQUIRE(n4 < (1ull << 30), "rtts_bn_act_bwd: more than 2^32 elements");
    const dim3 grid = ed_col_grid(B * g.P, C);
    const uint32_t th = ed_thresh(drop_p);
    const float ds = 1.f / (1.f - drop_p);
    float* sums = partial_ws + (size_t)ED_PBLOCKS * 2 * C;
    const int dzh = (halo > 0 && dz_halo) ? 1 : 0;
    hipLaunchKernelGGL((col_partial_kernel<1>), grid, dim3(ED_THREADS), 0, (hipStream_t)stream, y, (const bf16_t*)dz, mean, rstd, gamma, beta, act,
                       seed, seed_dev, th, ds, g, dzh, C, partial_ws);
    hipLaunchKernelGGL(bn_finalize_bwd_kernel, dim3((C + 63) / 64), dim3(64 * ED_FIN_WAVES), 0, (hipStream_t)stream, partial_ws,
                       (int)grid.x, C, sums, dgamma, dbeta);
    hipLaunchKernelGGL(bn_act_bwd_apply_kernel, dim3(ed_grid(n4)), dim3(ED_THREADS), 0, (hipStream_t)stream, y, (const bf16_t*)dz, mean, rstd,
                       gamma, beta, act, seed, seed_dev, th, ds, sums, 1.f / (float)((size_t)B * L), g, dzh, dy_lead, n4, C, ed_cshift(C), (bf16_t*)dy);
    RTTS_LAUNCH_CHECK("rtts_bn_act_bwd");
    return 0;
}

extern "C" int rtts_bn_moments(const float* y, int B, int L, int halo, int C, float* moments, float* partial_ws, void* stream) {
    RTTS_ENTER(stream);
    RTTS_REQUIRE(y && moments && partial_ws && B > 0 && L > 0 && halo >= 0 && C > 0 && C % 4 == 0, "rtts_bn_moments: bad arguments");
    const EdHalo g = ed_halo(B, L, halo);
    const dim3 grid = ed_col_grid(B * g.P, C);
    hipLaunchKernelGGL((col_partial_kernel<0>), grid, dim3(ED_THREADS), 0, (hipStream_t)stream, y, (const bf16_t*)nullptr, (const float*)nullptr,
                       (const float*)nullptr, (const float*)nullptr, (const float*)nullptr, 0, 0u, (const uint32_t*)nullptr, 0u, 1.f, g, 1, C,
                       partial_ws);
    hipLaunchKernelGGL(bn_moments_kernel, dim3((C + 63) / 64), dim3(64 * ED_FIN_WAVES), 0, (hipStream_t)stream, partial_ws, (int)grid.x, C, moments);
    RTTS_LAUNCH_CHECK("rtts_bn_moments");
    return 0;
}

extern "C" int rtts_bn_from_moments(const float* moments, int64_t count, int C, float* mean, float* rstd, float* run_mean, float* run_var,
                                    const float* mean_shift, int64_t* num_batches, void* stream) {
    RTTS_ENTER(stream);
    RTTS_REQUIRE(moments && mean && rstd && count >= 0 && C > 0, "rtts_bn_from_moments: bad arguments");
    hipLaunchKernelGGL(bn_from_moments_kernel, dim3((C + 255) / 256), dim3(256), 0, (hipStream_t)stream, moments, (float)count, C, mean, rstd,
                       run_mean, run_var, mean_shift, (long long*)num_batches);
    RTTS_LAUNCH_CHECK("rtts_bn_from_moments");
    return 0;
}

extern "C" int rtts_bn_act_bwd_sums(const float* y, const void* dz, int dz_halo, const float* mean, const float* rstd, const float* gamma,
                                    const float* beta, int act, float drop_p, uint32_t seed, const uint32_t* seed_dev, int B, int L, int halo,
                                    int C, float* sums, float* dgamma, float* dbeta, float* partial_ws, void* stream) {
    RTTS_ENTER(stream);
    RTTS_REQUIRE(y && dz && mean && rstd && gamma && beta && sums && dgamma && dbeta && partial_ws && B > 0 && L > 0 && halo >= 0 && C % 4 == 0 &&
                     (act == 1 || act == 2), "rtts_bn_act_bwd_sums: bad arguments");
    RTTS_REQUIRE(drop_p >= 0.f && drop_p < 1.f, "rtts_bn_act_bwd_sums: drop_p must be in [0, 1)");
    const EdHalo g = ed_halo(B, L, halo);
    const dim3 grid = ed_col_grid(B * g.P, C);
    const int dzh = (halo > 0 && dz_halo) ? 1 : 0;
    hipLaunchKernelGGL((col_partial_kernel<1>), grid, dim3(ED_THREADS), 0, (hipStream_t)stream, y, (const bf16_t*)dz, mean, rstd, gamma, beta, act,
                       seed, seed_dev, ed_thresh(drop_p), 1.f / (1.f - drop_p), g, dzh, C, partial_ws);
    hipLaunchKernelGGL(bn_finalize_bwd_kernel, dim3((C + 63) / 64), dim3(64 * ED_FIN_WAVES), 0, (hipStream_t)stream, partial_ws,
                       (int)grid.x, C, sums, dgamma, dbeta);
    RTTS_LAUNCH_CHECK("rtts_bn_act_bwd_sums");
    return 0;
}

extern "C" int rtts_bn_act_bwd_apply(const float* y, const void* dz, int dz_halo, const float* mean, const float* rstd, const float* gamma,
                                     const float* beta, int act, float drop_p, uint32_t seed, const uint32_t* seed_dev, int B, int L, int halo,
                                     int C, const float* sums, int64_t count, void* dy, int dy_lead, int64_t dy_rows, void* stream) {
    RTTS_ENTER(stream);
    RTTS_REQUIRE(y && dz && mean && rstd && gamma && beta && sums && dy && count >= 0 && B > 0 && L > 0 && halo >= 0 && C % 4 == 0 &&
                     (act == 1 || act == 2), "rtts_bn_act_bwd_apply: bad arguments");
    RTTS_REQUIRE(drop_p >= 0.f && drop_p < 1.f, "rtts_bn_act_bwd_apply: drop_p must be in [0, 1)");
    const EdHalo g = ed_halo(B, L, halo);
    RTTS_REQUIRE(dy_lead >= 0 && dy_rows >= dy_lead + (int64_t)B * g.P, "rtts_bn_act_bwd_apply: dy needs room for B*(L+2*halo) rows behind its lead-in");
    const int dzh = (halo > 0 && dz_halo) ? 1 : 0;
    const size_t n4 = (size_t)dy_rows * C / 4;
    RTTS_REQUIRE(n4 < (1ull << 30), "rtts_bn_act_bwd_apply: more than 2^32 elements");
    hipLaunchKernelGGL(bn_act_bwd_apply_kernel, dim3(ed_grid(n4)), dim3(ED_THREADS), 0, (hipStream_t)stream, y, (const bf16_t*)dz, mean, rstd,
                       gamma, beta, act, seed, seed_dev, ed_thresh(drop_p), 1.f / (1.f - drop_p), sums, count > 0 ? 1.f / (float)count : -1.f, g, dzh,
                       dy_lead, n4, C, ed_cshift(C), (bf16_t*)dy);
    RTTS_LAUNCH_CHECK("rtts_bn_act_bwd_apply");
    return 0;
}

extern "C" int rtts_tts_loss(const float* raw, const float* post, int64_t ld_mel, const float* tgt, const float* mask, const float* stop,
                             int64_t ld_stop, const float* tstop, int rows, int NM, int kind, float pos_weight, float w_raw, float w_post,
                             float w_stop, float* d_raw, float* d_post, int64_t ld_grad, float* d_stop, float* losses, float* partial_ws,
                             int padded_len, int valid_len, const float* res, int64_t ld_res, int halo, int dpost_lead, int64_t dpost_rows,
                             int64_t tgt_batch_stride, const int32_t* valid_len_dev, int64_t mask_batch_stride, int64_t tstop_batch_stride,
                             void* stream) {
    RTTS_ENTER(stream);
    RTTS_REQUIRE(raw && (post || res) && tgt && mask && stop && tstop && d_raw && d_post && d_stop && losses && partial_ws && rows > 0 && NM > 0 &&
                     ld_grad >= NM, "rtts_tts_loss: bad arguments");
    RTTS_REQUIRE(padded_len > 0 && valid_len > 0 && valid_len <= padded_len && rows % padded_len == 0,
                 "rtts_tts_loss: rows must be batch * padded_len and 0 < valid_len <= padded_len");
    RTTS_REQUIRE(kind == 0 || kind == 1, "rtts_tts_loss: Unsupported loss type: %d", kind);
    RTTS_REQUIRE(res ? (halo > 0 && ld_res >= NM && dpost_lead >= 0 &&
                        dpost_rows >= dpost_lead + (int64_t)(rows / padded_len) * (padded_len + 2 * halo))
                     : (halo == 0 && dpost_lead == 0),
                 "rtts_tts_loss: res / d_post in halo rows need halo > 0 and room for B*(L+2*halo) rows; without res: halo = lead = 0");
    if (tgt_batch_stride == 0) tgt_batch_stride = (int64_t)valid_len * NM;
    RTTS_REQUIRE(tgt_batch_stride >= (int64_t)valid_len * NM, "rtts_tts_loss: tgt_batch_stride below valid_len * NM");
    if (mask_batch_stride == 0) mask_batch_stride = (int64_t)valid_len * NM;
    if (tstop_batch_stride == 0) tstop_batch_stride = valid_len;
    RTTS_REQUIRE(mask_batch_stride >= (int64_t)valid_len * NM && tstop_batch_stride >= valid_len,
                 "rtts_tts_loss: mask / tstop batch strides below valid_len rows");
    const int blocks = 512;
    const uintptr_t bits = (uintptr_t)raw | (uintptr_t)post | (uintptr_t)res | (uintptr_t)tgt | (uintptr_t)mask | (uintptr_t)d_raw | (uintptr_t)d_post;
    const int vec4 = NM % 4 == 0 && (bits & 15) == 0 && ld_mel % 4 == 0 && ld_grad % 4 == 0 && (!res || ld_res % 4 == 0) &&
                     tgt_batch_stride % 4 == 0 && mask_batch_stride % 4 == 0 && (int64_t)rows * (NM / 4) < (1ll << 31);
    hipLaunchKernelGGL(tts_loss_kernel, dim3(blocks), dim3(ED_THREADS), 0, (hipStream_t)stream, raw, post, ld_mel, tgt, mask, stop, ld_stop,
                       tstop, rows, NM, kind, pos_weight, w_raw, w_post, w_stop, d_raw, d_post, ld_grad, d_stop, partial_ws, padded_len,
                       valid_len, res, ld_res, halo, dpost_lead, (long long)dpost_rows, (long long)tgt_batch_stride, valid_len_dev,
                       (long long)mask_batch_stride, (long long)tstop_batch_stride, vec4);
    const float vrows = (float)(rows / padded_len) * (float)valid_len;
    hipLaunchKernelGGL(tts_loss_finalize_kernel, dim3(1), dim3(64), 0, (hipStream_t)stream, partial_ws, blocks, 1.f / (vrows * NM),
                       1.f / vrows, w_raw, w_post, w_stop, losses, valid_len_dev, rows / padded_len, valid_len, NM);
    RTTS_LAUNCH_CHECK("rtts_tts_loss");
    return 0;
}

extern "C" int rtts_embedding_bwd(const int64_t* ids, const float* dx, int rows, int C, int n_embeddings, int padding_idx, float* dE,
                                  float drop_p, uint32_t seed, const uint32_t* seed_dev, void* stream) {
    RTTS_ENTER(stream);
    RTTS_REQUIRE(ids && dx && dE && rows > 0 && C > 0 && n_embeddings > 0 && drop_p >= 0.f && drop_p < 1.f, "rtts_embedding_bwd: bad arguments");
    hipLaunchKernelGGL(embedding_bwd_kernel, dim3(n_embeddings, (C + 63) / 64), dim3(ED_THREADS), 0, (hipStream_t)stream,
                       ids, dx, (int64_t)0, (int64_t)C, rows, rows, C, padding_idx, dE, seed, seed_dev, ed_thresh(drop_p), 1.f / (1.f - drop_p));
    RTTS_LAUNCH_CHECK("rtts_embedding_bwd");
    return 0;
}

extern "C" int rtts_embedding_bwd_strided(const int64_t* ids, const float* dx, int64_t batch_stride, int64_t row_stride, int L, int rows, int C,
                                          int n_embeddings, int padding_idx, float* dE, float drop_p, uint32_t seed, const uint32_t* seed_dev,
                                          void* stream) {
    RTTS_ENTER(stream);
    RTTS_REQUIRE(ids && dx && dE && rows > 0 && L > 0 && rows % L == 0 && C > 0 && row_stride >= C && batch_stride >= 0 && n_embeddings > 0 &&
                     drop_p >= 0.f && drop_p < 1.f, "rtts_embedding_bwd_strided: bad arguments");
    hipLaunchKernelGGL(embedding_bwd_kernel, dim3(n_embeddings, (C + 63) / 64), dim3(ED_THREADS), 0, (hipStream_t)stream,
                       ids, dx, batch_stride, row_stride, L, rows, C, padding_idx, dE, seed, seed_dev, ed_thresh(drop_p), 1.f / (1.f - drop_p));
    RTTS_LAUNCH_CHECK("rtts_embedding_bwd_strided");
    return 0;
}

extern "C" int rtts_embedding_fwd(const int64_t* ids, const float* E, int rows, int C, int n_embeddings, float drop_p, uint32_t seed,
                                  const uint32_t* seed_dev, float* out, void* stream) {
    RTTS_ENTER(stream);
    RTTS_REQUIRE(ids && E && out && rows > 0 && C > 0 && C % 4 == 0 && n_embeddings > 0 && drop_p >= 0.f && drop_p < 1.f,
                 "rtts_embedding_fwd: bad arguments");
    const size_t n4 = (size_t)rows * C / 4;
    hipLaunchKernelGGL(embedding_fwd_kernel, dim3(ed_grid(n4)), dim3(ED_THREADS), 0, (hipStream_t)stream, ids, E, n4, C, n_embeddings, seed,
                       seed_dev, ed_thresh(drop_p), 1.f / (1.f - drop_p), out);
    RTTS_LAUNCH_CHECK("rtts_embedding_fwd");
    return 0;
}

extern "C" int rtts_segments(const rtts_segment* jobs, int n, void* stream) {
    RTTS_ENTER(stream);
    RTTS_REQUIRE(jobs && n > 0 && n <= RTTS_SEGMENTS_MAX, "rtts_segments: 1..%d jobs", RTTS_SEGMENTS_MAX);
    SgGroup g;
    g.n = n;
    int blk = 0;
    for (int i = 0; i < n; ++i) {
        RTTS_REQUIRE(jobs[i].dst && jobs[i].src && jobs[i].count > 0 && jobs[i].kind >= 0 && jobs[i].kind <= RTTS_SEG_CAST_F32_BF16,
                     "rtts_segments: bad job %d", i);
        g.j[i].dst = jobs[i].dst;
        g.j[i].src = jobs[i].src;
        g.j[i].count = jobs[i].count;
        g.j[i].kind = jobs[i].kind;
        g.j[i].blk_start = blk;
        long long b = (jobs[i].count + ED_THREADS * 4 - 1) / (ED_THREADS * 4);
        blk += (int)(b > 256 ? 256 : b);
    }
    hipLaunchKernelGGL(segments_kernel, dim3(blk), dim3(ED_THREADS), 0, (hipStream_t)stream, g);
    RTTS_LAUNCH_CHECK("rtts_segments");
    return 0;
}

extern "C" int rtts_pe_add(const void* y, const float* table, const float* alpha, float drop_p, uint32_t seed, const uint32_t* seed_dev,
                           int T, int64_t M, int d, float* out, void* stream) {
    RTTS_ENTER(stream);
    RTTS_REQUIRE(y && table && alpha && out && T > 0 && M > 0 && d > 0 && d % 4 == 0 && M % T == 0 && drop_p >= 0.f && drop_p < 1.f,
                 "rtts_pe_add: bad arguments");
    const size_t n4 = (size_t)M * d / 4;
    hipLaunchKernelGGL(pe_add_kernel, dim3(ed_grid(n4)), dim3(ED_THREADS), 0, (hipStream_t)stream, (const bf16_t*)y, table, alpha, seed, seed_dev,
                       ed_thresh(drop_p), 1.f / (1.f - drop_p), T, n4, d, out);
    RTTS_LAUNCH_CHECK("rtts_pe_add");
    return 0;
}

extern "C" int rtts_pe_dalpha(const float* dy, const float* table, float drop_p, uint32_t seed, const uint32_t* seed_dev, int T, int64_t M,
                              int d, float* dalpha, float* partial_ws, void* stream) {
    RTTS_ENTER(stream);
    RTTS_REQUIRE(dy && table && dalpha && partial_ws && T > 0 && M > 0 && d % 4 == 0 && M % T == 0, "rtts_pe_dalpha: bad arguments");
    RTTS_REQUIRE(d > 0, "rtts_pe_dalpha: d must be positive");
    RTTS_REQUIRE(drop_p >= 0.f && drop_p < 1.f, "rtts_pe_dalpha: drop_p must be in [0, 1)");
    const size_t n4 = (size_t)M * d / 4;
    const int blocks = 512;
    hipLaunchKernelGGL(pe_dalpha_partial_kernel, dim3(blocks), dim3(ED_THREADS), 0, (hipStream_t)stream, dy, table, seed, seed_dev, ed_thresh(drop_p),
                       1.f / (1.f - drop_p), T, n4, d, partial_ws);
    hipLaunchKernelGGL(pe_dalpha_final_kernel, dim3(1), dim3(64), 0, (hipStream_t)stream, partial_ws, blocks, dalpha);
    RTTS_LAUNCH_CHECK("rtts_pe_dalpha");
    return 0;
}

__global__ __launch_bounds__(256) void batch_masks_kernel(const int64_t* __restrict__ phonemes, int64_t ph_stride, int B, int Lp, int Lp_pad,
                                                          const float* __restrict__ loss_mask, int64_t lm_bstride, int64_t lm_rstride, int Lm,
                                                          int Lm_pad, int n_mels, int64_t* __restrict__ pad_ph, uint8_t* __restrict__ ph_mask,
                                                          uint8_t* __restrict__ ph_not, uint8_t* __restrict__ sp_mask) {
    const int per_b = Lp_pad + Lm_pad;
    for (int i = blockIdx.x * blockDim.x + threadIdx.x; i < B * per_b; i += gridDim.x * blockDim.x) {
        const int b = i / per_b, j = i % per_b;
        if (j < Lp_pad) {
            const int64_t v = j < Lp ? phonemes[(int64_t)b * ph_stride + j] : 0;
            pad_ph[(size_t)b * Lp_pad + j] = v;
            ph_mask[(size_t)b * Lp_pad + j] = v != 0;
            ph_not[(size_t)b * Lp_pad + j] = v == 0;
        } else {
            const int t = j - Lp_pad;
            bool on = false;
            if (t < Lm) {
                const float* row = loss_mask + (int64_t)b * lm_bstride + (int64_t)t * lm_rstride;
                float sum = 0.f;
                for (int c = 0; c < n_mels; ++c) sum += row[c];
                on = (sum / (float)n_mels) != 0.f;
            }
            sp_mask[(size_t)b * Lm_pad + t] = on;
        }
    }
}

extern "C" int rtts_batch_masks(const int64_t* phonemes, int64_t ph_stride, int B, int Lp, int Lp_pad, const float* loss_mask, int64_t lm_bstride,
                                int64_t lm_rstride, int Lm, int Lm_pad, int n_mels, int64_t* pad_phonemes, uint8_t* phoneme_mask,
                                uint8_t* phoneme_pad_mask, uint8_t* frame_mask, void* stream) {
    RTTS_ENTER(stream);
    RTTS_REQUIRE(phonemes && loss_mask && pad_phonemes && phoneme_mask && phoneme_pad_mask && frame_mask, "rtts_batch_masks: null pointer");
    RTTS_REQUIRE(B > 0 && Lp > 0 && Lp_pad >= Lp && Lm > 0 && Lm_pad >= Lm && n_mels > 0 && ph_stride >= Lp, "rtts_batch_masks: bad shape");
    const int n = B * (Lp_pad + Lm_pad);
    hipLaunchKernelGGL(batch_masks_kernel, dim3((n + 255) / 256), dim3(256), 0, (hipStream_t)stream, phonemes, ph_stride, B, Lp, Lp_pad, loss_mask,
                       lm_bstride, lm_rstride, Lm, Lm_pad, n_mels, pad_phonemes, phoneme_mask, phoneme_pad_mask, frame_mask);
    RTTS_LAUNCH_CHECK("rtts_batch_masks");
    return 0;
}

extern "C" int rtts_relu_drop(void* h, float drop_p, uint32_t seed, const uint32_t* seed_dev, int64_t n, void* stream) {
    RTTS_ENTER(stream);
    RTTS_REQUIRE(h && n > 0 && n % 8 == 0 && drop_p >= 0.f && drop_p < 1.f, "rtts_relu_drop: bad arguments");
    hipLaunchKernelGGL(relu_drop_kernel, dim3(ed_grid((size_t)n / 8)), dim3(ED_THREADS), 0, (hipStream_t)stream, (bf16_t*)h, seed, seed_dev,
                       ed_thresh(drop_p), 1.f / (1.f - drop_p), (size_t)n / 8);
    RTTS_LAUNCH_CHECK("rtts_relu_drop");
    return 0;
}
```

### reformer-tts_amd/csrc/optim.hip

```cpp
#include "rtts_common.h"

#define OPT_THREADS 256
#define OPT_MAX_BLOCKS 2048

__global__ __launch_bounds__(OPT_THREADS) void sumsq_partial_kernel(const float* __restrict__ g, size_t n, float* __restrict__ partial) {
    float s = 0.f;
    const size_t n4 = n >> 2;
    const float4* g4 = reinterpret_cast<const float4*>(g);
    for (size_t i = (size_t)blockIdx.x * blockDim.x + threadIdx.x; i < n4; i += (size_t)gridDim.x * blockDim.x) {
        const float4 x = g4[i];
        s = __builtin_fmaf(x.x, x.x, s);
        s = __builtin_fmaf(x.y, x.y, s);
        s = __builtin_fmaf(x.z, x.z, s);
        s = __builtin_fmaf(x.w, x.w, s);
    }
    if (blockIdx.x == 0 && threadIdx.x < (n & 3)) {
        const float x = g[(n4 << 2) + threadIdx.x];
        s = __builtin_fmaf(x, x, s);
    }
    __shared__ float red[OPT_THREADS / 64];
#pragma unroll
    for (int o = 32; o > 0; o >>= 1) s += __shfl_xor(s, o);
    if ((threadIdx.x & 63) == 0) red[threadIdx.x >> 6] = s;
    __syncthreads();
    if (threadIdx.x == 0) partial[blockIdx.x] = red[0] + red[1] + red[2] + red[3];
}

__global__ __launch_bounds__(OPT_THREADS) void clip_scale_kernel(const float* __restrict__ partial, int nblocks, float grad_mult,
                                                                 float max_norm, float* __restrict__ scale) {
    float s = 0.f;
    for (int i = threadIdx.x; i < nblocks; i += OPT_THREADS) s += partial[i];
    __shared__ float red[OPT_THREADS / 64];
#pragma unroll
    for (int o = 32; o > 0; o >>= 1) s += __shfl_xor(s, o);
    if ((threadIdx.x & 63) == 0) red[threadIdx.x >> 6] = s;
    __syncthreads();
    if (threadIdx.x == 0) {
        const float norm = sqrtf(red[0] + red[1] + red[2] + red[3]) * grad_mult;
        float c = 1.f;
        if (max_norm > 0.f) c = fminf(1.f, max_norm / (norm + 1e-6f));
        scale[0] = grad_mult * c;
        scale[1] = norm;
    }
}

__global__ __launch_bounds__(OPT_THREADS) void adamw_kernel(float* __restrict__ p, const float* __restrict__ g, float* __restrict__ m,
                                                            float* __restrict__ v, const uint8_t* __restrict__ decay, size_t n4,
                                                            const float* __restrict__ scale, const float* __restrict__ hyper,
                                                            float b1, float b2, float eps, float wd, bf16_t* __restrict__ mirror) {
    const float gs = scale ? scale[0] : 1.f;
    const float lr = hyper[0], step_size = hyper[1];
    for (size_t i = (size_t)blockIdx.x * blockDim.x + threadIdx.x; i < n4; i += (size_t)gridDim.x * blockDim.x) {
        const float4 g4 = reinterpret_cast<const float4*>(g)[i];
        const float4 m4 = reinterpret_cast<const float4*>(m)[i];
        const float4 v4 = reinterpret_cast<const float4*>(v)[i];
        const float4 p4 = reinterpret_cast<const float4*>(p)[i];
        const uint32_t d4 = reinterpret_cast<const uint32_t*>(decay)[i];
        const float gg[4] = {g4.x, g4.y, g4.z, g4.w}, mm[4] = {m4.x, m4.y, m4.z, m4.w}, vv[4] = {v4.x, v4.y, v4.z, v4.w};
        const float pp[4] = {p4.x, p4.y, p4.z, p4.w};
        float mo[4], vo[4], po[4];
#pragma unroll
        for (int j = 0; j < 4; ++j) {
            const float gi = gg[j] * gs;
            mo[j] = b1 * mm[j] + (1.f - b1) * gi;
            vo[j] = b2 * vv[j] + (1.f - b2) * gi * gi;
            float pi = pp[j] - step_size * mo[j] / (sqrtf(vo[j]) + eps);
            if ((d4 >> (8 * j)) & 0xffu) pi -= lr * wd * pi;
            po[j] = pi;
        }
        reinterpret_cast<float4*>(m)[i] = make_float4(mo[0], mo[1], mo[2], mo[3]);
        reinterpret_cast<float4*>(v)[i] = make_float4(vo[0], vo[1], vo[2], vo[3]);
        reinterpret_cast<float4*>(p)[i] = make_float4(po[0], po[1], po[2], po[3]);
        if (mirror) {
            uint2 o;
            o.x = pack_bf16x2(po[0], po[1]);
            o.y = pack_bf16x2(po[2], po[3]);
            reinterpret_cast<uint2*>(mirror)[i] = o;
        }
    }
}

extern "C" int rtts_grad_clip_scale(const float* grads, int64_t n, float grad_mult, float max_norm, float* partial_ws,
                                    float* scale_out, void* stream) {
    RTTS_ENTER(stream);
    RTTS_REQUIRE(grads && partial_ws && scale_out && n > 0, "rtts_grad_clip_scale: bad arguments");
    RTTS_REQUIRE(((uintptr_t)grads & 15) == 0, "rtts_grad_clip_scale: grads must be 16-byte aligned");
    int blocks = (int)((n / 4 + OPT_THREADS - 1) / OPT_THREADS);
    if (blocks < 1) blocks = 1;
    if (blocks > OPT_MAX_BLOCKS) blocks = OPT_MAX_BLOCKS;
    hipLaunchKernelGGL(sumsq_partial_kernel, dim3(blocks), dim3(OPT_THREADS), 0, (hipStream_t)stream, grads, (size_t)n, partial_ws);
    hipLaunchKernelGGL(clip_scale_kernel, dim3(1), dim3(OPT_THREADS), 0, (hipStream_t)stream, partial_ws, blocks, grad_mult,
                       max_norm, scale_out);
    RTTS_LAUNCH_CHECK("rtts_grad_clip_scale");
    return 0;
}

extern "C" int rtts_adamw_step(float* params, const float* grads, float* exp_avg, float* exp_avg_sq, const uint8_t* decay_mask,
                               int64_t n, const float* scale, const float* hyper, float beta1, float beta2, float eps,
                               float weight_decay, void* bf16_mirror, void* stream) {
    RTTS_ENTER(stream);
    RTTS_REQUIRE(params && grads && exp_avg && exp_avg_sq && decay_mask && hyper && n > 0, "rtts_adamw_step: bad arguments");
    RTTS_REQUIRE(n % 4 == 0, "rtts_adamw_step: n must be a multiple of 4 (pad the flat buffers)");
    RTTS_REQUIRE((((uintptr_t)params | (uintptr_t)grads | (uintptr_t)exp_avg | (uintptr_t)exp_avg_sq) & 15) == 0 &&
                     ((uintptr_t)decay_mask & 3) == 0 && ((uintptr_t)bf16_mirror & 7) == 0,
                 "rtts_adamw_step: buffers must be 16-byte aligned (decay mask 4, mirror 8)");
    int blocks = (int)((n / 4 + OPT_THREADS - 1) / OPT_THREADS);
    if (blocks > OPT_MAX_BLOCKS) blocks = OPT_MAX_BLOCKS;
    hipLaunchKernelGGL(adamw_kernel, dim3(blocks), dim3(OPT_THREADS), 0, (hipStream_t)stream, params, grads, exp_avg, exp_avg_sq,
                       decay_mask, (size_t)n / 4, scale, hyper, beta1, beta2, eps, weight_decay, (bf16_t*)bf16_mirror);
    RTTS_LAUNCH_CHECK("rtts_adamw_step");
    return 0;
}
```

### reformer-tts_amd/edges.py

```python
from __future__ import annotations

import threading
from typing import List

import torch

from . import _lib
from . import engine as _engine
from .engine import WEIGHT_EPOCH, _WS, _bf16, _grad, bf16_twin, cast_colsum, gemm, wgrad

from ._seeds import _seed_counter, seed_base


def _s() -> int:
    return torch.cuda.current_stream().cuda_stream


def _ws(device, c: int) -> torch.Tensor:
    key = ("edge", device, c, torch.cuda.current_stream(device).cuda_stream)
    if key not in _WS._cache:
        _WS._cache[key] = torch.empty((2 * 256 + 2) * c, dtype=torch.float32, device=device)
    return _WS._cache[key]


def _pad128(c: int) -> int:
    return -(-c // 128) * 128


class Halo:
    H, LEAD, TILE = 2, 8, 256

    def __init__(self, b: int, l: int):
        self.b, self.l = b, l
        self.p = l + 2 * self.H
        self.rows = b * self.p
        self.mp = -(-self.rows // self.TILE) * self.TILE
        self.alloc = self.mp + 2 * self.LEAD

    def new(self, c: int, device, dtype=torch.bfloat16) -> torch.Tensor:
        return torch.empty(self.alloc, c, dtype=dtype, device=device)

    def body(self, buf: torch.Tensor, shift: int = 0) -> torch.Tensor:
        return buf[self.LEAD + shift:self.LEAD + shift + self.mp]

    def valid(self, body: torch.Tensor) -> torch.Tensor:
        return body[:self.rows].view(self.b, self.p, -1)[:, self.H:self.H + self.l]


import os as _os
CONVS_PER_WGRAD_LAUNCH = int(_os.environ.get("RTTS_CONVS_PER_WGRAD", "4"))


def flush_conv_wgrad(queue=None) -> None:
    queue = _engine._queue() if queue is None else queue
    q = queue.conv_gemms
    wide = [p for p in q if p[0][7] % 256 == 0 and p[0][8] % 256 == 0]
    rest = [p for p in q if not (p[0][7] % 256 == 0 and p[0][8] % 256 == 0)]
    del q[:]
    for part in (wide, rest):
        while part:
            chunk = part[:_lib.GEMM_TN_MAX_GROUP]
            del part[:len(chunk)]
            arr = (_lib.GemmTnProblem * len(chunk))()
            for dst, (fields, _keep) in zip(arr, chunk):
                dst.a, dst.lda, dst.b, dst.ldb, dst.c, dst.ldc, dst.M, dst.N, dst.K, dst.accumulate = fields
            ws = _engine._slab_ws(chunk[0][1][0].device, queue.stream)
            _lib.call("rtts_gemm_tn_grouped", arr, len(chunk), ws.data_ptr(), ws.numel(), queue.stream)


def flush_conv_dw(queue=None) -> None:
    queue = _engine._queue() if queue is None else queue
    flush_conv_wgrad(queue)
    pending = list(queue.conv_items)
    del queue.conv_items[:]
    for chunk in _engine.launch_groups(pending, _lib.CONV_PERM_MAX_GROUP,
                                       lambda a, b: _engine.spans_overlap(a[4].data_ptr(), 20 * a[1] * a[2], b[4].data_ptr(), 20 * b[1] * b[2])):
        jobs = (_lib.ConvPermJob * len(chunk))()
        for j, (dwp, co, ci, cp, gw) in zip(jobs, chunk):
            j.w, j.wp, j.Co, j.Ci, j.CP = dwp.data_ptr(), gw.data_ptr(), co, ci, cp
        _lib.call("rtts_conv_dw_unperm_grouped", jobs, len(chunk), queue.stream)


class ConvK5:

    instances = None

    def __init__(self, conv: torch.nn.Conv1d):
        self.conv = conv
        self.co, self.ci = conv.out_channels, conv.in_channels
        self.cp = _pad128(self.ci)
        self.cop = _pad128(self.co)
        self._wp = None
        self._wp_version = None
        if ConvK5.instances is None:
            import weakref
            ConvK5.instances = weakref.WeakSet()
        ConvK5.instances.add(self)

    def _version(self):
        w = self.conv.weight
        return (w._version, WEIGHT_EPOCH[0], w.data_ptr())

    @staticmethod
    def refresh_all(device) -> None:
        stale = [c for c in (ConvK5.instances or ()) if c.conv.weight.device == device and c._wp_version != c._version()]
        for i in range(0, len(stale), _lib.CONV_PERM_MAX_GROUP):
            chunk = stale[i:i + _lib.CONV_PERM_MAX_GROUP]
            jobs = (_lib.ConvPermJob * len(chunk))()
            for j, c in zip(jobs, chunk):
                if c._wp is None or c._wp.device != device:
                    c._wp = torch.zeros(c.cop, 5 * c.cp, dtype=torch.bfloat16, device=device)
                j.w, j.wp, j.Co, j.Ci, j.CP = c.conv.weight.data_ptr(), c._wp.data_ptr(), c.co, c.ci, c.cp
            _lib.call("rtts_conv_w_perm_grouped", jobs, len(chunk), _s())
            for c in chunk:
                c._wp_version = c._version()

    def weight_perm(self) -> torch.Tensor:
        w = self.conv.weight
        ver = (w._version, WEIGHT_EPOCH[0], w.data_ptr())
        if self._wp is None or self._wp_version != ver or self._wp.device != w.device:
            if self._wp is None or self._wp.device != w.device:
                self._wp = torch.zeros(self.cop, 5 * self.cp, dtype=torch.bfloat16, device=w.device)
            _lib.call("rtts_conv_w_perm", w.data_ptr(), self.co, self.ci, self.cp, self._wp.data_ptr(), _s())
            self._wp_version = ver
        return self._wp

    def forward(self, xh: torch.Tensor, g: Halo, bias=None) -> torch.Tensor:
        y = torch.empty(g.mp, self.cop, dtype=torch.float32, device=xh.device)
        wp = self.weight_perm()
        _lib.call("rtts_conv1d_k5", g.body(xh).data_ptr(), self.cp, wp.data_ptr(), 5 * self.cp, 0, g.mp, self.cop, self.cp, y.data_ptr(),
                  self.cop, None if bias is None else bias.data_ptr(), 1, _s())
        return y

    def forward_moments(self, xh: torch.Tensor, g: Halo):
        y = torch.empty(g.mp, self.cop, dtype=torch.float32, device=xh.device)
        nrows = _lib.load().rtts_gemm_nt_partial_rows(g.mp, self.cop)
        if nrows <= 0:
            raise _lib.RttsError(f"rtts_conv1d_k5_moments: no tile shape for {g.mp} x {self.cop}")
        partial = torch.empty(nrows, 2 * self.cop, dtype=torch.float32, device=xh.device)
        _lib.call("rtts_conv1d_k5_moments", g.body(xh).data_ptr(), self.cp, self.weight_perm().data_ptr(), 5 * self.cp, g.mp, self.cop, self.cp,
                  y.data_ptr(), self.cop, g.b, g.l, g.H, partial.data_ptr(), _s())
        return y, partial, nrows

    def backward(self, dyh: torch.Tensor, xh: torch.Tensor, g: Halo, need_dx: bool = True, dx_f32: bool = False):
        dev = dyh.device
        dwp = torch.empty(self.cop, 5 * self.cp, dtype=torch.float32, device=dev)
        dyb = g.body(dyh)
        dwq = _engine._queue()
        for k in range(5):
            xs, ck = g.body(xh, k - 2), dwp[:, k * self.cp:(k + 1) * self.cp]
            dwq.conv_gemms.append(((dyb.data_ptr(), self.cop, xs.data_ptr(), self.cp, ck.data_ptr(), 5 * self.cp, g.mp, self.cop, self.cp, 0),
                              (dyh, xh, dwp)))
        if len(dwq.conv_gemms) >= 5 * CONVS_PER_WGRAD_LAUNCH:
            flush_conv_wgrad(dwq)
        dwq.conv_items.append((dwp, self.co, self.ci, self.cp, _grad(self.conv.weight)))
        if len(dwq.conv_items) >= _lib.CONV_PERM_MAX_GROUP:
            flush_conv_dw(dwq)
        else:
            from .engine import _queue_final_flush
            _queue_final_flush()
        if not need_dx:
            return None
        dx = torch.empty(g.mp, self.cp, dtype=torch.float32 if dx_f32 else torch.bfloat16, device=dev)
        _lib.call("rtts_conv1d_k5", dyb.data_ptr(), self.cop, self.weight_perm().data_ptr(), 5 * self.cp, 1, g.mp, self.cp, self.cop,
                  dx.data_ptr(), self.cp, None, int(dx_f32), _s())
        return dx


SYNC_BN = None
CONV_MOMENTS = _os.environ.get("RTTS_CONV_MOMENTS", "1") != "0"


class ConvBNAct:

    def __init__(self, conv, bn, act: int, p: float):
        self.c = ConvK5(conv)
        self.bn, self.act, self.p = bn, act, float(p)

    def forward(self, xh, g: Halo, plain_out: bool = False):
        fused = SYNC_BN is None and CONV_MOMENTS
        y, partial, nrows = self.c.forward_moments(xh, g) if fused else (self.c.forward(xh, g), None, 0)
        c = y.shape[1]
        dev = y.device
        mean = torch.empty(c, dtype=torch.float32, device=dev)
        rstd = torch.empty(c, dtype=torch.float32, device=dev)
        bn = self.bn
        if fused:
            _lib.call("rtts_bn_stats_from_partials", partial.data_ptr(), nrows, g.b, g.l, c, mean.data_ptr(), rstd.data_ptr(),
                      bn.running_mean.data_ptr(), bn.running_var.data_ptr(), self.c.conv.bias.data_ptr(), bn.num_batches_tracked.data_ptr(), _s())
        elif SYNC_BN is None:
            _lib.call("rtts_bn_stats", y.data_ptr(), g.b, g.l, g.H, c, mean.data_ptr(), rstd.data_ptr(), bn.running_mean.data_ptr(),
                      bn.running_var.data_ptr(), self.c.conv.bias.data_ptr(), bn.num_batches_tracked.data_ptr(), _ws(dev, c).data_ptr(), _s())
        else:
            import torch.distributed as dist
            mom = torch.empty(2 * c + 1, dtype=torch.float32, device=dev)
            _lib.call("rtts_bn_moments", y.data_ptr(), g.b, g.l, g.H, c, mom.data_ptr(), _ws(dev, c).data_ptr(), _s())
            mom[2 * c:].fill_(float(g.b * g.l))
            dist.all_reduce(mom, group=SYNC_BN)
            _lib.call("rtts_bn_from_moments", mom.data_ptr(), 0, c, mean.data_ptr(), rstd.data_ptr(), bn.running_mean.data_ptr(),
                      bn.running_var.data_ptr(), self.c.conv.bias.data_ptr(), bn.num_batches_tracked.data_ptr(), _s())
        seed = next(_seed_counter) * 2654435761 % (1 << 32)
        if plain_out:
            z = torch.empty(g.b * g.l, c, dtype=torch.bfloat16, device=dev)
            zargs = (0, 0, g.b * g.l)
        else:
            z = g.new(c, dev)
            zargs = (1, g.LEAD, g.alloc)
        _lib.call("rtts_bn_act_fwd", y.data_ptr(), mean.data_ptr(), rstd.data_ptr(), bn.weight.data_ptr(), bn.bias.data_ptr(), self.act,
                  self.p, seed, seed_base(dev).data_ptr(), g.b, g.l, g.H, c, z.data_ptr(), *zargs, _s())
        return z, (xh, y, mean, rstd, seed)

    def backward(self, dz, dz_halo: bool, saved, g: Halo, need_dx=True, dx_f32=False):
        xh, y, mean, rstd, seed = saved
        c = y.shape[1]
        bn = self.bn
        dy = g.new(c, y.device)
        if SYNC_BN is None:
            _lib.call("rtts_bn_act_bwd", y.data_ptr(), dz.data_ptr(), int(dz_halo), mean.data_ptr(), rstd.data_ptr(), bn.weight.data_ptr(),
                      bn.bias.data_ptr(), self.act, self.p, seed, seed_base(y.device).data_ptr(), g.b, g.l, g.H, c, dy.data_ptr(), g.LEAD, g.alloc,
                      _grad(bn.weight).data_ptr(), _grad(bn.bias).data_ptr(), _ws(y.device, c).data_ptr(), _s())
        else:
            import torch.distributed as dist
            sums = torch.empty(2 * c + 1, dtype=torch.float32, device=y.device)
            _lib.call("rtts_bn_act_bwd_sums", y.data_ptr(), dz.data_ptr(), int(dz_halo), mean.data_ptr(), rstd.data_ptr(), bn.weight.data_ptr(),
                      bn.bias.data_ptr(), self.act, self.p, seed, seed_base(y.device).data_ptr(), g.b, g.l, g.H, c, sums.data_ptr(),
                      _grad(bn.weight).data_ptr(), _grad(bn.bias).data_ptr(), _ws(y.device, c).data_ptr(), _s())
            sums[2 * c:].fill_(float(g.b * g.l))
            dist.all_reduce(sums, group=SYNC_BN)
            _lib.call("rtts_bn_act_bwd_apply", y.data_ptr(), dz.data_ptr(), int(dz_halo), mean.data_ptr(), rstd.data_ptr(), bn.weight.data_ptr(),
                      bn.bias.data_ptr(), self.act, self.p, seed, seed_base(y.device).data_ptr(), g.b, g.l, g.H, c, sums.data_ptr(), 0,
                      dy.data_ptr(), g.LEAD, g.alloc, _s())
        _grad(self.c.conv.bias)
        return self.c.backward(dy, xh, g, need_dx, dx_f32)


class ConvStackFn(torch.autograd.Function):

    @staticmethod
    def forward(ctx, x, stack: List[ConvBNAct], training: bool):
        b, l, c = x.shape
        g = Halo(b, l)
        x2 = x.detach().reshape(b * l, c)
        if x2.dtype not in (torch.float32, torch.bfloat16) or x2.stride(1) != 1:
            x2 = x2.float().contiguous()
        cur = g.new(c, x.device)
        _lib.call("rtts_to_halo", x2.data_ptr(), x2.stride(0), 0, c, int(x2.dtype == torch.float32), b, l, g.H, c, cur.data_ptr(), g.LEAD, g.alloc, _s())
        saved = []
        for i, layer in enumerate(stack):
            cur, s = layer.forward(cur, g, plain_out=(i == len(stack) - 1))
            saved.append(s)
        ctx.stack, ctx.saved_state, ctx.geom, ctx.in_dtype = stack, saved, g, x.dtype
        return cur.view(b, l, -1)

    @staticmethod
    def backward(ctx, dz):
        g = ctx.geom
        if ctx.saved_state is None:
            raise RuntimeError("ConvStackFn.backward: state already consumed")
        cur = dz.reshape(g.b * g.l, -1).to(torch.bfloat16).contiguous()
        halo = False
        n = len(ctx.stack)
        for i in range(n - 1, -1, -1):
            cur = ctx.stack[i].backward(cur, halo, ctx.saved_state[i], g, need_dx=True, dx_f32=(i == 0))
            halo = True
        ctx.saved_state = None
        dx = g.valid(cur)
        return (dx if ctx.in_dtype == torch.float32 else dx.to(ctx.in_dtype)), None, None


def encoder_prenet_stack(prenet) -> List[ConvBNAct]:
    c = prenet.convolutions
    return [ConvBNAct(c.conv1, c.bn1, 1, c.dropout1.p), ConvBNAct(c.conv2, c.bn2, 1, c.dropout2.p),
            ConvBNAct(c.conv3, c.bn3, 1, c.dropout3.p)]


def segments(jobs):
    jobs = list(jobs)
    while jobs:
        group, jobs = jobs[:_lib.SEGMENTS_MAX], jobs[_lib.SEGMENTS_MAX:]
        arr = (_lib.Segment * len(group))()
        for j, (dst, src, kind) in zip(arr, group):
            if not (dst.is_contiguous() and src.is_contiguous() and dst.numel() == src.numel()):
                raise ValueError("segments: operands must be contiguous and of equal size")
            j.dst, j.src, j.count, j.kind = dst.data_ptr(), src.data_ptr(), dst.numel(), kind
        _lib.call("rtts_segments", arr, len(group), _s())


class PostnetLoss:

    def __init__(self, model, loss_mod):
        self.model, self.loss_mod = model, loss_mod
        pn = model.postnet.layers
        depth = (len(pn) - 1) // 4
        self.layers = [ConvBNAct(getattr(pn, f"conv{i}"), getattr(pn, f"bn{i}"), 2, getattr(pn, f"dropout{i}").p) for i in range(depth)]
        self.convend = ConvK5(pn.convend)
        self.nm = model.num_mel_coeffs
        self.pos_weight = float(loss_mod.pos_weight)
        self._wh = None

    def _operands(self):
        mel, stop = self.model.dec.mel_linear, self.model.dec.stop_linear
        d, dev = mel.weight.shape[1], mel.weight.device
        if self._wh is None or self._wh.device != dev:
            self._wh = torch.zeros(128, d, dtype=torch.bfloat16, device=dev)
            self._bh = torch.zeros(128, dtype=torch.float32, device=dev)
        c, nm = self.convend, self.nm
        if getattr(c, "_bias_pad", None) is None or c._bias_pad.device != dev:
            c._bias_pad = torch.zeros(c.cop, dtype=torch.float32, device=dev)
        wm, ws = _bf16(mel.weight), _bf16(stop.weight)
        kind_w = _lib.SEG_COPY_BF16 if wm.dtype == torch.bfloat16 else _lib.SEG_CAST_F32_BF16
        segments([(self._wh[:nm], wm.contiguous(), kind_w), (self._wh[nm:nm + 1], ws.contiguous(), kind_w),
                  (self._bh[:nm], mel.bias.detach(), _lib.SEG_COPY_F32), (self._bh[nm:nm + 1], stop.bias.detach(), _lib.SEG_COPY_F32),
                  (c._bias_pad[:c.co], c.conv.bias.detach(), _lib.SEG_COPY_F32)])
        return self._wh, self._bh, c._bias_pad

    def apply(self, y_dec, true_mel, true_stop, true_mask, valid_len=None):
        return _PostnetLossFn.apply(y_dec, true_mel, true_stop, true_mask, self, valid_len)


class _PostnetLossFn(torch.autograd.Function):
    @staticmethod
    def forward(ctx, y_dec, true_mel, true_stop, true_mask, ex: PostnetLoss, valid_len=None):
        b, lp, d = y_dec.shape
        l = true_mel.shape[1]
        nm, dev = ex.nm, y_dec.device
        m = b * lp
        g = Halo(b, lp)
        yb = bf16_twin(y_dec)
        yb = yb.view(m, d) if yb is not None else y_dec.detach().reshape(m, d).to(torch.bfloat16)
        wh, bh, bias_end = ex._operands()
        heads = gemm(yb, wh, bias=bh, out_f32=True)
        x0 = g.new(128, dev)
        _lib.call("rtts_to_halo", heads.data_ptr(), 128, 0, 128, 1, b, lp, g.H, 128, x0.data_ptr(), g.LEAD, g.alloc, _s())
        saved, cur = [], x0
        for layer in ex.layers:
            cur, s = layer.forward(cur, g)
            saved.append(s)
        res = ex.convend.forward(cur, g, bias=bias_end)
        lm = ex.loss_mod
        losses = torch.empty(4, dtype=torch.float32, device=dev)
        n_raw, n_post = m * 128, g.alloc * 128
        gbuf = torch.empty(n_raw + n_post + m, dtype=torch.float32, device=dev)
        d_raw, d_post, g_stop = gbuf[:n_raw].view(m, 128), gbuf[n_raw:n_raw + n_post].view(g.alloc, 128), gbuf[n_raw + n_post:]
        pw = torch.empty(512 * 3, dtype=torch.float32, device=dev)
        if true_mel.dtype != torch.float32 or true_mel.stride(2) != 1 or true_mel.stride(1) != nm:
            true_mel = true_mel.float().contiguous()
        if valid_len is not None and not (valid_len.dtype == torch.int32 and valid_len.is_cuda and valid_len.numel() == 1):
            raise ValueError("PostnetLoss: valid_len must be a one-element int32 device tensor")
        _lib.call("rtts_tts_loss", heads.data_ptr(), None, 128, true_mel.data_ptr(), true_mask.contiguous().data_ptr(),
                  heads[:, nm:].data_ptr(), 128, true_stop.contiguous().data_ptr(), m, nm, lm.kind, ex.pos_weight,
                  float(lm.raw_pred_loss_weight), float(lm.post_pred_loss_weight), float(lm.stop_loss_weight), d_raw.data_ptr(),
                  d_post.data_ptr(), 128, g_stop.data_ptr(), losses.data_ptr(), pw.data_ptr(), lp, l, res.data_ptr(), 128, g.H, g.LEAD,
                  g.alloc, true_mel.stride(0), None if valid_len is None else valid_len.data_ptr(), 0, 0, _s())
        ctx.ex, ctx.state = ex, (yb, wh, saved, cur, gbuf, g, d)
        ctx.set_materialize_grads(False)
        return losses[0], losses[1], losses[2], losses[3]

    @staticmethod
    def backward(ctx, g_total, g_raw, g_post, g_stop_loss):
        ex = ctx.ex
        if g_raw is not None or g_post is not None or g_stop_loss is not None:
            raise NotImplementedError("PostnetLoss: only the total loss is differentiable (the parts are reported values; "
                                      "model.TTSLoss differentiates all four)")
        if g_total is None:
            return None, None, None, None, None, None
        if ctx.state is None:
            raise RuntimeError("PostnetLoss.backward: state already consumed")
        yb, wh, saved, z_last, gbuf, g, d = ctx.state
        ctx.state = None
        nm, dev = ex.nm, yb.device
        b, lp = g.b, g.l
        m = b * lp
        up = g_total.detach().reshape(1)
        up = up if up.dtype == torch.float32 else up.float()
        n_raw, n_post = m * 128, g.alloc * 128
        d_raw, d_post, g_stop = gbuf[:n_raw].view(m, 128), gbuf[n_raw:n_raw + n_post].view(g.alloc, 128), gbuf[n_raw + n_post:]
        dresb = cast_colsum(d_post, [(0, nm, _grad(ex.convend.conv.bias))], scale=up)
        dz = ex.convend.backward(dresb, z_last, g)
        for layer, s in zip(reversed(ex.layers[1:]), reversed(saved[1:])):
            dz = layer.backward(dz, True, s, g)
        dx0 = ex.layers[0].backward(dz, True, saved[0], g, need_dx=True, dx_f32=True)
        dheads = torch.empty(m, 128, dtype=torch.float32, device=dev)
        _lib.call("rtts_heads_grad", d_raw.data_ptr(), d_post.data_ptr(), g.LEAD, dx0.data_ptr(), 128, g_stop.data_ptr(), b, lp, g.H, nm, 128,
                  dheads.data_ptr(), up.data_ptr(), _s())
        mel, stop = ex.model.dec.mel_linear, ex.model.dec.stop_linear
        dhb = cast_colsum(dheads, [(0, nm, _grad(mel.bias)), (nm, 1, _grad(stop.bias))])
        dwh = torch.empty(128, d, dtype=torch.float32, device=dev)
        wgrad(dwh, dhb, yb, accumulate=False)
        segments([(_grad(mel.weight), dwh[:nm], _lib.SEG_ADD_F32), (_grad(stop.weight), dwh[nm:nm + 1], _lib.SEG_ADD_F32)])
        dy = gemm(dhb, wh, kn=True, out_f32=True).view(b, lp, d)
        return dy, None, None, None, None, None


def _seed() -> int:
    return next(_seed_counter) * 2654435761 % (1 << 32)


def _pe_ws(device) -> torch.Tensor:
    key = ("pe", device, torch.cuda.current_stream(device).cuda_stream)
    if key not in _WS._cache:
        _WS._cache[key] = torch.empty(512, dtype=torch.float32, device=device)
    return _WS._cache[key]


class _ProjPEFn(torch.autograd.Function):

    @staticmethod
    def forward(ctx, z, lin, pe, _track):
        b, l, k = z.shape
        d = lin.out_features
        z2 = z.reshape(b * l, k)
        y = gemm(z2, _bf16(lin.weight), bias=lin.bias)
        table = pe.table(l, z.device).contiguous()
        out = torch.empty(b * l, d, dtype=torch.float32, device=z.device)
        p = pe.dropout.p if pe.training else 0.0
        seed = _seed()
        _lib.call("rtts_pe_add", y.data_ptr(), table.data_ptr(), pe.alpha.data_ptr(), float(p), seed, seed_base(z.device).data_ptr(), l, b * l, d,
                  out.data_ptr(), _s())
        ctx.mods, ctx.state = (lin, pe), (z2, table, p, seed, b, l, k, d)
        return out.view(b, l, d)

    @staticmethod
    def backward(ctx, dout):
        lin, pe = ctx.mods
        z2, table, p, seed, b, l, k, d = ctx.state
        dy = dout.reshape(b * l, d).float().contiguous()
        _lib.call("rtts_pe_dalpha", dy.data_ptr(), table.data_ptr(), float(p), seed, seed_base(dy.device).data_ptr(), l, b * l, d, _grad(pe.alpha).data_ptr(),
                  _pe_ws(dy.device).data_ptr(), _s())
        dyb = cast_colsum(dy, _grad(lin.bias))
        wgrad(_grad(lin.weight), dyb, z2)
        dz = gemm(dyb, _bf16(lin.weight), kn=True)
        return dz.view(b, l, k), None, None, None


def proj_pe(z, lin, pe):
    return _ProjPEFn.apply(z, lin, pe, lin.weight)


def _k_padded_weight(lin) -> torch.Tensor:
    w = lin.weight
    ver = (w._version, WEIGHT_EPOCH[0], w.data_ptr())
    cache = getattr(lin, "_rtts_kpad", None)
    if cache is None or cache[0] != ver or cache[1].device != w.device:
        buf = cache[1] if cache is not None and cache[1].device == w.device else torch.zeros(w.shape[0], 128, dtype=torch.bfloat16, device=w.device)
        buf[:, :w.shape[1]].copy_(_bf16(w))
        lin._rtts_kpad = cache = (ver, buf)
    return cache[1]


class _ReluDropLinearFn(torch.autograd.Function):

    @staticmethod
    def forward(ctx, x, lin, p, kpad, _track):
        h = gemm(x, _k_padded_weight(lin) if kpad else _bf16(lin.weight), bias=lin.bias, relu=True)
        seed = _seed()
        if p > 0.0:
            _lib.call("rtts_relu_drop", h.data_ptr(), float(p), seed, seed_base(h.device).data_ptr(), h.numel(), _s())
        ctx.lin, ctx.state = lin, (x, h, p, kpad)
        return h

    @staticmethod
    def backward(ctx, dh):
        from .engine import colsum_bf16
        lin = ctx.lin
        x, h, p, kpad = ctx.state
        if dh.dtype != torch.bfloat16 or not dh.is_contiguous():
            dh = dh.to(torch.bfloat16).contiguous()
        gated = torch.empty_like(dh)
        colsum_bf16(dh, _grad(lin.bias), h, 1.0 / (1.0 - p), out=gated)
        dh = gated
        if kpad:
            k = lin.weight.shape[1]
            tmp = torch.empty(lin.weight.shape[0], 128, dtype=torch.float32, device=dh.device)
            wgrad(tmp, dh, x, accumulate=False)
            _grad(lin.weight).add_(tmp[:, :k])
            return None, None, None, None, None
        wgrad(_grad(lin.weight), dh, x)
        return (gemm(dh, _bf16(lin.weight), kn=True) if ctx.needs_input_grad[0] else None), None, None, None, None


def decoder_prenet_pe(prenet, pe, spec):
    b, l, nm = spec.shape
    lyr = prenet.layer
    training = prenet.training
    m = b * l
    kpad = nm % 64 != 0
    if kpad:
        if nm % 8 != 0 or nm > 128:
            raise NotImplementedError(f"decoder prenet: {nm} mel channels (supported: multiples of 8 up to 128, or multiples of 64)")
        if spec.dtype != torch.float32 or spec.stride(2) != 1 or spec.stride(1) % 4 != 0 or spec.stride(0) % 4 != 0:
            spec = spec.float().contiguous()
        x = torch.empty(m, 128, dtype=torch.bfloat16, device=spec.device)
        _lib.call("rtts_to_halo", spec.data_ptr(), spec.stride(1), spec.stride(0), nm, 1, b, l, 0, 128, x.data_ptr(), 0, m, _s())
    else:
        x = spec.reshape(m, nm).to(torch.bfloat16)
    h = _ReluDropLinearFn.apply(x, lyr.fc1, lyr.dropout1.p if training else 0.0, kpad, lyr.fc1.weight)
    h = _ReluDropLinearFn.apply(h, lyr.fc2, lyr.dropout2.p if training else 0.0, False, lyr.fc2.weight)
    return proj_pe(h.view(b, l, -1), lyr.projection, pe)


def _padded_linear(lin) -> tuple:
    w = lin.weight
    ver = (w._version, WEIGHT_EPOCH[0], w.data_ptr(), None if lin.bias is None else lin.bias._version)
    cache = getattr(lin, "_rtts_padded", None)
    if cache is None or cache[1].device != w.device:
        n, k = w.shape
        npad, kpad = -(-n // 64) * 64, -(-k // 64) * 64
        wb = torch.zeros(npad, kpad, dtype=torch.bfloat16, device=w.device)
        bias = None if lin.bias is None else torch.zeros(npad, dtype=torch.float32, device=w.device)
        lin._rtts_padded = cache = [None, wb, bias]
    if cache[0] != ver:
        n, k = w.shape
# ... 98 lines not shown
```

### reformer-tts_amd/training/trainer.py

```python
from __future__ import annotations

import math
import os
import time
from typing import Dict, List, Optional

import torch
import torch.distributed as dist

from .. import _lib, engine
from .._graphs import capturing
from ..model import ReformerTTS, TTSLoss
from ..model.config import ReformerTTSConfig, TTSTrainingConfig, as_kwargs

NO_DECAY = ("bias", "norm.weight")


def build_model(cfg: ReformerTTSConfig, device=None, seed: int = 42) -> ReformerTTS:
    torch.manual_seed(seed)
    model = ReformerTTS(**as_kwargs(cfg))
    return model.to(device) if device is not None else model


def synthetic_batch(batch: int, text_len: int, mel_len: int, n_mels: int = 80, dict_size: int = 76, seed: int = 42,
# ... 71 lines not shown
        self._decorrelate_replicas()
        self._flatten()
        self._make_buckets()
        self._pending: List = []

    def _decorrelate_replicas(self):
        if self.rank == 0:
            return
        from ..model.lsh_attention import LSHSelfAttention
        for m in self.model.modules():
            if isinstance(m, LSHSelfAttention):
                m.seed = int(m.seed) + 1000003 * self.rank
                m._gen = None
        if self.device.type == "cuda":
            torch.cuda.manual_seed(torch.initial_seed() + 1000003 * self.rank)

    def step_seed(self, step_index: int) -> int:
        return (step_index * 2246822519 + 3266489917 + self.rank * 2654435769) % (1 << 31)

    def _flatten(self):
        named = [(n, p) for n, p in self.model.named_parameters() if p.requires_grad]
        align = 8
        starts, off = [], 0
        for _, p in named:
            starts.append(off)
            off += -(-p.numel() // align) * align
        total = off
        pad = 0
        dev = self.device
        self.flat_p = torch.zeros(total, dtype=torch.float32, device=dev)
        self.flat_g = torch.zeros_like(self.flat_p)
        self.flat_m = torch.zeros_like(self.flat_p)
        self.flat_v = torch.zeros_like(self.flat_p)
        self.decay_mask = torch.zeros(total, dtype=torch.uint8, device=dev)
        self.n_params = total
        self.offsets: Dict[str, tuple] = {}
        for (n, p), off in zip(named, starts):
            k = p.numel()
            self.flat_p[off:off + k].copy_(p.detach().reshape(-1))
            p.data = self.flat_p[off:off + k].view_as(p)
            p.grad = self.flat_g[off:off + k].view_as(p)
            if not any(nd in n for nd in NO_DECAY):
                self.decay_mask[off:off + k] = 1
            self.offsets[n] = (off, off + k)
        if dev.type == "cuda":
            self.ws_partial = torch.zeros(2048, dtype=torch.float32, device=dev)
            self.ws_scale = torch.zeros(2, dtype=torch.float32, device=dev)
            self.hyper = torch.zeros(2, dtype=torch.float32, device=dev)
            self._hyper_ring = [dict(hyper=torch.zeros(2, dtype=torch.float32).pin_memory(),
                                     seed=torch.zeros(1, dtype=torch.int32).pin_memory(), ev=None) for _ in range(8)]
            self._ring_next = 0
            self.flat_pb = torch.zeros(total + pad, dtype=torch.bfloat16, device=dev)
            for n, p in named:
                s, e = self.offsets[n]
                p._bf16_mirror = self.flat_pb[s:e].view_as(p)
            self.refresh_mirror()

    def refresh_mirror(self):
        _lib.call("rtts_cast_f32_bf16", self.flat_p.data_ptr(), self.flat_pb.data_ptr(), self.flat_p.numel(),
                  torch.cuda.current_stream().cuda_stream)

    def _make_buckets(self):
        self.block_bucket: Dict[tuple, tuple] = {}
        covered = []
        for stack_name, seq in (("enc", self.model.enc.reformer.layers), ("dec", self.model.dec.reformer.layers)):
            prefix = f"{stack_name}.reformer.layers.blocks."
            for i in range(len(seq.blocks)):
                rng = [self.offsets[n] for n in self.offsets if n.startswith(f"{prefix}{i}.")]
                if rng:
                    s, e = min(r[0] for r in rng), max(r[1] for r in rng)
                    self.block_bucket[(stack_name, i)] = (s, e)
                    covered.append((s, e))
            seq.block_done_hook = self._make_hook(stack_name)
        covered.sort()
        self.rest: List[tuple] = []
        cur = 0
        for s, e in covered:
            if s > cur:
                self.rest.append((cur, s))
            cur = max(cur, e)
        if cur < self.n_params:
            self.rest.append((cur, self.n_params))

    def _make_hook(self, stack_name):
        def hook(seq, i):
            if self.world > 1 and not self._bulk_allreduce and not self._accumulating and (stack_name, i) in self.block_bucket:
                s, e = self.block_bucket[(stack_name, i)]
                self._pending.append(dist.all_reduce(self.flat_g[s:e], group=self.pg, async_op=True))
        hook.active = lambda: self.world > 1 and not self._bulk_allreduce and not self._accumulating
        return hook

    use_fused_edges = True

    @staticmethod
    def _frames(batch):
        if "spectrogram_input" in batch:
            return batch["spectrogram_input"], batch["spectrogram_target"]
        spec = batch["spectrogram"]
        return spec[:, :-1], spec[:, 1:]

    def _fused_edges_ok(self, batch) -> bool:
        spec = self._frames(batch)[0]
        lm = spec.shape[1]
        lp = -(-lm // self.model.pad_base) * self.model.pad_base
        ok = self.use_fused_edges and self.device.type == "cuda" and self.model.training and (spec.shape[0] * lp) % 64 == 0
        if not ok and self.use_fused_edges and self.device.type == "cuda" and self.model.training:
            _lib.note_general_path("heads / postnet / loss", f"batch x padded length = {spec.shape[0]} x {lp} is not a multiple of 64")
        if ok:
            pn = self.model.postnet.layers
            width = pn.conv0.out_channels
            if width % 128 != 0 or self.model.num_mel_coeffs + 1 > 128 or self.model.num_mel_coeffs % 8 != 0:
                _lib.note_general_path("heads / postnet / loss", f"postnet width {width} (needs a multiple of 128) / {self.model.num_mel_coeffs} "
                                       "mel channels (a multiple of 8, at most 127)")
                ok = False
        return ok

    def _cut_at_encoder(self, keys):
        self._enc_out = keys
        self._enc_in = keys.detach().requires_grad_(True)
        for attr in ("_rtts_bf16", "_rtts_ready"):
            if hasattr(keys, attr):
                setattr(self._enc_in, attr, getattr(keys, attr))
        return self._enc_in

    def _cut_at_enc_stack(self, x):
        self._pre_out = x
        self._pre_in = x.detach().requires_grad_(True)
        return self._pre_in

    HBM_HEADROOM = 0.85

    def stash_estimate(self, batch, mode: str) -> int:
        pb = self.model.pad_base
        b, lp = batch["phonemes"].shape
        lm = self._frames(batch)[0].shape[1]
        te, td = -(-lp // pb) * pb, -(-lm // pb) * pb
        total = 0
        for seq, rows, keys in ((self.model.enc.reformer.layers, b * te, 0), (self.model.dec.reformer.layers, b * td, b * te)):
            if not getattr(seq, "_program_built", True):
                seq._program, seq._program_built = engine.build_program(seq), True
            prog = getattr(seq, "_program", None)
            if prog:
                total += engine.stash_bytes(prog, rows, self.model.dec.mel_linear.in_features, mode, keys)
        return total

    def resolve_recompute(self, batch, free_bytes: Optional[int] = None) -> str:
        key = self._shape_key(batch) if "spectrogram" in batch else tuple(batch["phonemes"].shape) + tuple(self._frames(batch)[0].shape[:2])
        hit = self._recompute_for.get(key)
        if hit is not None and free_bytes is None:
            return hit
        mode = self.recompute
        if self.device.type == "cuda" or free_bytes is not None:
            if free_bytes is None:
                free, _ = torch.cuda.mem_get_info(self.device)
                free += torch.cuda.memory_reserved(self.device) - torch.cuda.memory_allocated(self.device)
            else:
                free = int(free_bytes)
            rank = engine.RECOMPUTE_MODES.index(mode)
            while rank > 0 and self.stash_estimate(batch, engine.RECOMPUTE_MODES[rank]) > self.HBM_HEADROOM * free:
                rank -= 1
            if engine.RECOMPUTE_MODES[rank] != mode:
                need = self.stash_estimate(batch, mode)
                mode = engine.RECOMPUTE_MODES[rank]
                _lib.log_once(f"recompute:{key}", f"tts_training.recompute = {self.recompute!r} would hold ~{need / 2**30:.2f} GiB for the "
                              f"backward at batch shape {key}; {free / 2**30:.2f} GiB of HBM are free: running this shape in mode {mode!r}")
        self._recompute_for[key] = mode
        return mode

    def _apply_modes(self, batch):
        from .. import edges
        edges.SYNC_BN = self._sync_bn
        engine.set_recompute(self.resolve_recompute(batch))

    def forward_loss(self, batch, split: bool = False):
        self._apply_modes(batch)
        spec = self._frames(batch)[0]
        from ..model.lsh_attention import LSHSelfAttention
        if getattr(self, "_graph_rotations", False):
            LSHSelfAttention.rotation_pool = (torch.randn(1 << 18, device=spec.device, dtype=torch.float32), [0])
        if spec.device.type == "cuda":
            from ..edges import ConvK5
            ConvK5.refresh_all(spec.device)
        try:
            return self._forward_loss(batch, split)
        finally:
            LSHSelfAttention.rotation_pool = None

    def _forward_loss(self, batch, split: bool = False):
        spec_in, spec_tgt = self._frames(batch)
        side_enc = bool(split) and self.overlap_encoder and self.device.type == "cuda" and self._fused_edges_ok(batch)
        if side_enc:
            from ..model.lsh_attention import LSHSelfAttention
            if LSHSelfAttention.rotation_pool is not None:
                LSHSelfAttention.rotation_pool[0].record_stream(self._enc_stream())
        if self._fused_edges_ok(batch):
            from ..edges import PostnetLoss
            if getattr(self, "_postnet_loss", None) is None:
                self._postnet_loss = PostnetLoss(self.model, self.loss)
            overlap = split == "overlap"
            y = self.model.decoder_hidden(batch["phonemes"], spec_in, loss_mask=batch["loss_mask"],
                                          keys_hook=self._cut_at_encoder if split else None,
                                          enc_stack_hook=self._cut_at_enc_stack if (split and not overlap) else None,
                                          enc_stream=self._enc_stream() if side_enc else None)
            losses = self._postnet_loss.apply(y, spec_tgt, batch["stop_tokens"], batch["loss_mask"], batch.get("valid_len"))
            return losses[0], losses[1], losses[2], losses[3]
        raw, post, stop, _ = self.model(batch["phonemes"], spec_in, spectrogram_mask=batch["loss_mask"].mean(dim=-1))
        return self.loss(raw, post, stop.view(stop.shape[0], -1), spec_tgt, batch["stop_tokens"], batch["loss_mask"])

    def zero_grad(self):
        self.flat_g.zero_()

    def finish_allreduce(self):
        if self.world > 1 and not self._bulk_allreduce and not self._accumulating:
            for s, e in self.rest:
                self._pending.append(dist.all_reduce(self.flat_g[s:e], group=self.pg, async_op=True))
            for w in self._pending:
                w.wait()
            self._pending.clear()

    def _queue_keys(self):
        if self.device.type != "cuda":
            return None
        idx = self.device.index if self.device.index is not None else torch.cuda.current_device()
        keys = [(idx, torch.cuda.current_stream(self.device).cuda_stream)]
        if getattr(self, "_enc_stream_obj", None) is not None:
            keys.append((idx, self._enc_stream_obj.cuda_stream))
        return keys

    def _warm_stream(self):
        if getattr(self, "_warm_stream_obj", None) is None:
            self._warm_stream_obj = torch.cuda.Stream(self.device)
        return self._warm_stream_obj

    def _run_backward(self, loss):
        keys = self._queue_keys()
        one = getattr(self, "_one", None)
        if one is None or one.device != loss.device or one.dtype != loss.dtype:
            one = self._one = torch.ones((), dtype=loss.dtype, device=loss.device)
        try:
            loss.backward(one if loss.dim() == 0 else None)
            engine.flush_wgrad(keys=keys)
        except BaseException:
            engine.discard_pending(keys)
            raise
        left = engine.pending_all(keys)
        if left:
            engine.discard_pending(keys)
            raise RuntimeError(f"{left} deferred gradient launches were still queued after the flush")

    def backward(self, loss):
        self._run_backward(loss)
        self.finish_allreduce()

    def lr_now(self) -> float:
        return self.lr_now_for(self.global_step)

    def end_epoch(self) -> float:
        self.epoch += 1
        sch = self.cfg.lr_scheduler
        if sch is None:
            return 1.0
        if sch.start_schedule_epoch < 1:
            raise AssertionError("start_schedule_epoch has to be >= 1")
        end = sch.end_schedule_epoch if sch.end_schedule_epoch is not None else self.cfg.max_epochs
        if end is None:
            raise ValueError("lr_scheduler: end_schedule_epoch or max_epochs must be set")
        factor = 1.0
        if sch.start_schedule_epoch <= self.epoch <= end:
            gamma = (math.log(sch.initial_lr) - math.log(sch.final_lr)) / (end - sch.start_schedule_epoch)
            factor = math.exp(-gamma)
        self._lr *= factor
        return factor

    def take_lr(self, step_index: int) -> float:
        lr = self.lr_now_for(step_index)
        if self.cfg.warmup_steps is not None and step_index < self.cfg.warmup_steps:
            self._lr = lr
        return lr

    def set_step_hyper(self, step_index: int):
        lr = self.take_lr(step_index)
        t = step_index + 1
        slot = self._hyper_ring[self._ring_next % len(self._hyper_ring)]
        self._ring_next += 1
        if slot["ev"] is not None:
            slot["ev"].synchronize()
        slot["hyper"][0] = lr
        slot["hyper"][1] = lr * math.sqrt(1.0 - 0.999 ** t) / (1.0 - 0.9 ** t)
        self.hyper.copy_(slot["hyper"], non_blocking=True)
        from .._seeds import seed_base
        slot["seed"][0] = self.step_seed(step_index)
        seed_base(self.device).copy_(slot["seed"], non_blocking=True)
        slot["ev"] = torch.cuda.Event()
        slot["ev"].record(torch.cuda.current_stream())

    def optimizer_step(self, update_hyper: bool = True):
        if self.device.type != "cuda":
            raise _lib.RttsError("optimizer_step runs on the GPU only (no CPU fallback for the HIP path)")
        if update_hyper:
            self.set_step_hyper(self.global_step)
        self.global_step += 1
        n = self.flat_p.numel()
        stream = torch.cuda.current_stream().cuda_stream
        _lib.call("rtts_grad_clip_scale", self.flat_g.data_ptr(), n, 1.0 / self.world, float(self.cfg.gradient_clip_val),
                  self.ws_partial.data_ptr(), self.ws_scale.data_ptr(), stream)
        _lib.call("rtts_adamw_step", self.flat_p.data_ptr(), self.flat_g.data_ptr(), self.flat_m.data_ptr(),
                  self.flat_v.data_ptr(), self.decay_mask.data_ptr(), n, self.ws_scale.data_ptr(), self.hyper.data_ptr(), 0.9, 0.999,
                  1e-6, float(self.cfg.weight_decay), self.flat_pb.data_ptr(), stream)
        from ..engine import WEIGHT_EPOCH
        WEIGHT_EPOCH[0] += 1

    def lr_now_for(self, step: int) -> float:
        if self.cfg.warmup_steps is not None and step < self.cfg.warmup_steps:
            return min(1.0, float(step + 1) / self.cfg.warmup_steps) * self._base_lr
        return self._lr

    def train_step(self, batch, update_hyper: bool = True):
        self.model.train()
        self.zero_grad()
        total, raw_l, post_l, stop_l = self.forward_loss(batch)
        self.backward(total)
        if self._bulk_allreduce:
            self.bulk_allreduce()
        self.optimizer_step(update_hyper)
        return total.detach(), raw_l.detach(), post_l.detach(), stop_l.detach()

    overlap_encoder = True

    def _enc_stream(self):
        cur = torch.cuda.current_stream(self.device).cuda_stream
        s = getattr(self, "_enc_stream_obj", None)
        if s is None or s.cuda_stream == cur:
            for _ in range(64):
                s = torch.cuda.Stream(self.device)
                if s.cuda_stream != cur:
                    break
            else:
                raise RuntimeError("no stream other than the current one could be obtained for the encoder branch")
            self._enc_stream_obj = s
        return s

    def train_step_overlapped(self, batch, update_hyper: bool = True):
        if not self._fused_edges_ok(batch):
            return self.train_step(batch, update_hyper)
        self.model.train()
        self.zero_grad()
        total, raw_l, post_l, stop_l = self.forward_backward_overlapped(batch)
        if self._bulk_allreduce:
            self.bulk_allreduce()
        self.optimizer_step(update_hyper)
        return total.detach(), raw_l.detach(), post_l.detach(), stop_l.detach()

    handover_encoder_wgrads = os.environ.get("RTTS_HANDOVER_WGRADS", "1") != "0"

    def forward_backward_overlapped(self, batch, loss_scale=None):
        main, side = torch.cuda.current_stream(), self._enc_stream()
        dec_seq = self.model.dec.reformer.layers
        dec_seq.manual = {}
        try:
            engine.stamp("step: first kernel of the forward")
            total, raw_l, post_l, stop_l = self.forward_loss(batch, split="overlap")
            engine.stamp("forward + loss done")
            if "call" not in dec_seq.manual:
                raise RuntimeError("the decoder stack did not take the explicit executor: the overlapped step needs it")
            self._run_backward(total if loss_scale is None else total * loss_scale)
            ctx, dec_x, _, dec_out = dec_seq.manual["call"]
            gen = engine.stack_backward_steps(ctx, dec_out.grad, notify_dkeys=True)
            dx = None
            idx = self.device.index if self.device.index is not None else torch.cuda.current_device()
            steal = dict(src=(idx, side.cuda_stream), src_stream=side, pending=[]) if self.handover_encoder_wgrads else None
            while True:
                try:
                    with torch.no_grad():
                        _, item = next(gen)
                except StopIteration as fin:
                    dx = fin.value[0]
                    break
                if isinstance(item, tuple) and item[0] == "dkeys":
                    dkeys = item[1]
                    ev = torch.cuda.Event()
                    ev.record(main)
                    side.wait_event(ev)
                    dkeys.record_stream(side)
                    engine.stamp("backward: d(keys) complete (main stream)")
                    engine.STEAL = steal
                    try:
                        with torch.cuda.stream(side):
                            engine.stamp("encoder branch: backward starts")
                            self._enc_out.backward(dkeys)
                            engine.flush_wgrad()
                            engine.stamp("encoder branch: backward done")
                    finally:
                        engine.STEAL = None
            dec_x.backward(dx)
            engine.flush_wgrad()
            engine.stamp("decoder branch: backward done")
            if steal is not None and steal["pending"]:
                engine.run_handed_over(steal)
                engine.stamp("main stream: the encoder's weight gradients done")
            main.wait_stream(side)
            engine.stamp("backward joined")
            if engine.pending_all():
                raise RuntimeError("deferred gradient launches were still queued at the end of the overlapped step")
        finally:
            dec_seq.manual = None
            self._enc_out = self._enc_in = None
        return total, raw_l, post_l, stop_l

    _accumulating = False

    def train_accumulated(self, batches):
        batches = list(batches)
        n = len(batches)
        self.model.train()
        self.zero_grad()
        total = None
        for i, batch in enumerate(batches):
            self._accumulating = i + 1 < n
            loss = self.forward_loss(batch)[0]
            self._run_backward(loss * (1.0 / n))
            total = loss.detach() if total is None else total + loss.detach()
        self._accumulating = False
        if self.world > 1 and not self._bulk_allreduce:
            self.finish_allreduce()
        elif self._bulk_allreduce:
            self.bulk_allreduce()
        self.optimizer_step(True)
        return total / n

    @torch.no_grad()
    def validate(self, batch, return_attention: bool = False):
        was_training = self.model.training
        stacks = (self.model.enc.reformer.layers, self.model.dec.reformer.layers)
        dec = self.model.dec.reformer
        was_collect = dec.collect_attention
        self.model.eval()
        for st in stacks:
            st.fused_in_eval = True
        dec.collect_attention = bool(return_attention)
        try:
            spec = batch["spectrogram"]
            raw, post, stop, mats = self.model(batch["phonemes"], spec[:, :-1], spectrogram_mask=batch["loss_mask"].mean(dim=-1))
            stop2 = stop.view(stop.shape[0], -1)
            out = (*self.loss(raw, post, stop2, spec[:, 1:], batch["stop_tokens"], batch["loss_mask"]), stop_mae(stop2, batch["stop_tokens"]))
            if return_attention:
                out = (*out, trim_attention_matrices(list(mats), batch["stop_tokens"]))
            return out
        finally:
            for st in stacks:
                st.fused_in_eval = False
            dec.collect_attention = was_collect
            self.model.train(was_training)

    def state_dict(self) -> dict:
        moments = {n: (self.flat_m[s:e].detach().clone(), self.flat_v[s:e].detach().clone()) for n, (s, e) in self.offsets.items()}
        return {"model": {k: v.detach().clone() for k, v in self.model.state_dict().items()}, "adam": moments,
                "global_step": self.global_step, "epoch": self.epoch, "lr": self._lr}

    def load_state_dict(self, state: dict) -> None:
        self.model.load_state_dict(state["model"])
        for n, (m, v) in state["adam"].items():
            s, e = self.offsets[n]
            self.flat_m[s:e].copy_(m.reshape(-1))
            self.flat_v[s:e].copy_(v.reshape(-1))
        self.global_step = int(state["global_step"])
        self.epoch = int(state.get("epoch", 0))
        self._lr = float(state.get("lr", self._base_lr))
        if self.device.type == "cuda":
            self.refresh_mirror()
            engine.WEIGHT_EPOCH[0] += 1

    def fit(self, host_batches, log_every: int = 0, graphs: Optional[bool] = None):
        from ..dataset import BatchPrefetcher
        if getattr(self.cfg, "noise_std", None):
            _lib.note_general_path("Trainer.fit", "input noise (tts_training.noise_std) is applied by fit_corpus only: host batches train without it")
        losses, group = [], []
        acc = max(1, int(self.cfg.accumulate_grad_batches))
        from .. import edges
        use_graphs = (self.device.type == "cuda" and self.use_fused_edges and edges.SYNC_BN is None) if graphs is None else bool(graphs)

        def step(batches):
            if use_graphs:
                return self._train_group_graphed(batches)
            return self.train_step(batches[0])[0] if len(batches) == 1 else self.train_accumulated(batches)

        for batch in BatchPrefetcher(host_batches, self.device):
            group.append(batch)
            if len(group) == acc:
                losses.append(step(group))
                group = []
                if log_every and len(losses) % log_every == 0:
                    print(f"step {self.global_step}: loss {float(losses[-1]):.4f}", flush=True)
        if group:
            losses.append(step(group))
        self.end_epoch()
        return losses

    def fit_corpus(self, corpus, plan, log_every: int = 0, graphs: Optional[bool] = None):
        from .. import edges
        plan = [[int(i) for i in ids] for ids in plan]
        if not plan or any(not ids for ids in plan):
            raise ValueError("fit_corpus: the plan must be a non-empty list of non-empty utterance-id lists")
        use_graphs = (self.device.type == "cuda" and self.use_fused_edges and edges.SYNC_BN is None) if graphs is None else bool(graphs)
        flat = torch.tensor([i for ids in plan for i in ids], dtype=torch.int32).to(corpus.device)
        acc = max(1, int(self.cfg.accumulate_grad_batches))
        pb = self.model.pad_base
        losses, group, at = [], [], 0

        def step(micros):
            if use_graphs:
                return self._train_group_graphed(micros)
            batches = [m.eager(self._noise_seed(i)) for i, m in enumerate(micros)]
            return self.train_step(batches[0])[0] if len(batches) == 1 else self.train_accumulated(batches)

        for ids in plan:
            lp, lm = corpus._shape(ids)
            group.append(_CorpusMicro(corpus, ids, flat[at:at + len(ids)], lm, (len(ids), -(-lp // pb), -(-lm // pb)),
                                      getattr(self.cfg, "noise_std", None)))
            at += len(ids)
            if len(group) == acc:
                losses.append(step(group))
                group = []
                if log_every and len(losses) % log_every == 0:
                    print(f"step {self.global_step}: loss {float(losses[-1]):.4f}", flush=True)
        if group:
            losses.append(step(group))
        self.end_epoch()
        return losses

    def _noise_seed(self, micro: int) -> int:
        return (self.step_seed(self.global_step) * 2654435761 + 40503 * micro + 0x5bd1e995) & 0xFFFFFFFF

    def validate_corpus(self, corpus, ids, return_attention: bool = False):
        return self.validate(corpus.collate(ids), return_attention=return_attention)

    def _eval_flags(self):
        stacks = (self.model.enc.reformer.layers, self.model.dec.reformer.layers)
        return self.model.training, self.model.dec.reformer.collect_attention, [(st, st.fused_in_eval) for st in stacks]

    def _restore_flags(self, flags):
        was_training, was_collect, fused = flags
        for st, f in fused:
            st.fused_in_eval = f
        self.model.dec.reformer.collect_attention = was_collect
        self.model.train(was_training)

    def _validate_inference(self, phonemes, truth_kw, lm, combine_strategy, max_len, stop_threshold, use_graph, cache_encoder, return_outputs):
        from .. import ops
        if combine_strategy not in ("concat", "replace"):
            raise ValueError(f"validate_inference: combine_strategy must be 'concat' or 'replace' (got {combine_strategy!r})")
        if use_graph is None:
            use_graph = combine_strategy == "concat" and self.device.type == "cuda"
        flags = self._eval_flags()
        try:
            start = time.perf_counter()
            spec, stop = self.model.infer(phonemes, combine_strategy=combine_strategy, max_len=max_len, stop_threshold=stop_threshold,
                                          stop_at_stop_token=self.cfg.stop_loss_weight != 0., cache_encoder=cache_encoder,
                                          use_graph=bool(use_graph) and combine_strategy == "concat")
            torch.cuda.synchronize(spec.device)
            inference_time = time.perf_counter() - start
        finally:
            self._restore_flags(flags)
        sse, stop_err, totals = ops.infer_metrics(spec, stop, lm=lm, **truth_kw)
        out = {f"{combine_strategy}_inference_pred_mse": totals[0], f"{combine_strategy}_inference_stop_mae": totals[1],
               f"{combine_strategy}_inference_time": inference_time, "sse": sse, "stop_err": stop_err}
        if return_outputs:
            out["spectrogram"], out["stop"] = spec, stop
        return out

    @torch.no_grad()
    def validate_inference(self, batch, combine_strategy: str = "concat", *, max_len: int = 1024, stop_threshold: float = 0.25,
                           use_graph: Optional[bool] = None, cache_encoder: bool = False, return_outputs: bool = False) -> dict:
        spec = batch["spectrogram"]
        b, rows, n_mel = spec.shape
        spec = spec if spec.is_contiguous() else spec.contiguous()
        truth_kw = dict(truth=spec.view(b * rows, n_mel), truth_frames_last=False,
                        starts=torch.arange(b, dtype=torch.int64, device=spec.device) * rows + 1,
                        lengths=(batch["stop_tokens"].argmax(dim=1) + 1).to(torch.int32))
        return self._validate_inference(batch["phonemes"], truth_kw, rows - 1, combine_strategy, max_len, stop_threshold, use_graph,
                                        cache_encoder, return_outputs)

    @torch.no_grad()
    def validate_inference_corpus(self, corpus, ids, combine_strategy: str = "concat", *, max_len: int = 1024, stop_threshold: float = 0.25,
                                  use_graph: Optional[bool] = None, cache_encoder: bool = False, return_outputs: bool = False) -> dict:
        ids = [int(i) for i in ids]
        lp, lm = corpus._shape(ids)
        dev_ids = torch.tensor(ids, dtype=torch.int32).to(corpus.device)
        phonemes = torch.empty(len(ids), max(lp, 1), dtype=torch.int64, device=corpus.device)
        corpus._launch(dev_ids, lm, None, 0, phonemes=phonemes)
        truth_kw = dict(truth=corpus.mel, frame_offsets=corpus.tables[0], ids=dev_ids, longest=lm)
        return self._validate_inference(phonemes[:, :lp], truth_kw, lm, combine_strategy, max_len, stop_threshold, use_graph, cache_encoder,
                                        return_outputs)

    @torch.no_grad()
    def validation_epoch(self, corpus, ids, batch_size: Optional[int] = None, inference: bool = True, **inference_kwargs) -> Dict[str, float]:
        ids = [int(i) for i in ids]
        bs = int(self.cfg.batch_size if batch_size is None else batch_size)
        if bs < 1 or len(ids) < bs:
            raise ValueError(f"validation_epoch: {len(ids)} utterances make no batch of {bs}")
        acc, n = None, len(ids) // bs
        for k in range(n):
            row = torch.stack(self.validate_corpus(corpus, ids[k * bs:(k + 1) * bs]))
            acc = row if acc is None else acc + row
        values = (acc / n).double()
        names = ["val_loss", "val_raw_pred_loss", "val_post_pred_loss", "val_stop_loss", "val_stop_mae"]
        inference_time = None
        if inference:
            inf = self.validate_inference_corpus(corpus, ids[:bs], "concat", **inference_kwargs)
            values = torch.cat([values, torch.stack([inf["concat_inference_pred_mse"], inf["concat_inference_stop_mae"]])])
            names += ["concat_inference_pred_mse", "concat_inference_stop_mae"]
            inference_time = inf["concat_inference_time"]
# ... 548 lines not shown
```

Measured before the change: 1.959 million mel-frames/s.

## Fuse BN stats finalize into activation, clip into AdamW, batch embedding backward

Adds a kernel that reduces the conv-produced BN partials and applies batchnorm+activation+dropout in one launch, with the loads of y issued before the reduction so they overlap it. Folds the grad-clip finalize into the AdamW kernel for single-GPU runs, so every block recomputes the clip scale from the per-block partials. Rewrites embedding backward to ballot several row groups at once, compact the matching rows into shared memory, and issue eight loads at a time. The goal is fewer launches and more memory-level parallelism, at the cost of redundant partial reductions in every block and a smaller fold grid.

```diff
diff --git a/include/rtts.h b/include/rtts.h
--- a/include/rtts.h
+++ b/include/rtts.h
@@ -47,6 +47,9 @@
 int rtts_adamw_step(float* params, const float* grads, float* exp_avg, float* exp_avg_sq, const uint8_t* decay_mask,
                     int64_t n, const float* scale, const float* hyper, float beta1, float beta2, float eps,
                     float weight_decay, void* bf16_mirror, void* stream);
+int rtts_clip_adamw_step(float* params, const float* grads, float* exp_avg, float* exp_avg_sq, const uint8_t* decay_mask,
+                         int64_t n, float grad_mult, float max_norm, float* partial_ws, float* scale_out, const float* hyper,
+                         float beta1, float beta2, float eps, float weight_decay, void* bf16_mirror, void* stream);
 
 int rtts_ln_fwd(const float* x, const float* gamma, const float* beta, void* xn, float* mean, float* rstd,
                 int M, int d, void* stream);
@@ -119,6 +122,10 @@
 int rtts_bn_act_bwd(const float* y, const void* dz, int dz_halo, const float* mean, const float* rstd, const float* gamma,
                     const float* beta, int act, float drop_p, uint32_t seed, const uint32_t* seed_dev, int B, int L, int halo, int C,
                     void* dy, int dy_lead, int64_t dy_rows, float* dgamma, float* dbeta, float* partial_ws, void* stream);
+int rtts_bn_act_fwd_from_partials(const float* partial, int nrows, const float* y, float* mean, float* rstd, float* run_mean,
+                                  float* run_var, const float* mean_shift, int64_t* num_batches, const float* gamma, const float* beta,
+                                  int act, float drop_p, uint32_t seed, const uint32_t* seed_dev, int B, int L, int halo, int C, void* z,
+                                  int z_halo, int z_lead, int64_t z_rows, void* stream);
 int rtts_bn_moments(const float* y, int B, int L, int halo, int C, float* moments, float* partial_ws, void* stream);
 int rtts_bn_from_moments(const float* moments, int64_t count, int C, float* mean, float* rstd, float* run_mean, float* run_var,
                          const float* mean_shift, int64_t* num_batches, void* stream);
diff --git a/reformer-tts_amd/_lib.py b/reformer-tts_amd/_lib.py
--- a/reformer-tts_amd/_lib.py
+++ b/reformer-tts_amd/_lib.py
@@ -91,6 +91,8 @@
     "rtts_conv1d_k5_moments": [_vp, _i64, _vp, _i64, _i32, _i32, _i32, _vp, _i64, _i32, _i32, _i32, _vp, _vp],
     "rtts_bn_stats_from_partials": [_vp, _i32, _i32, _i32, _i32, _vp, _vp, _vp, _vp, _vp, _vp, _vp],
     "rtts_bn_stats": [_vp, _i32, _i32, _i32, _i32, _vp, _vp, _vp, _vp, _vp, _vp, _vp, _vp],
+    "rtts_bn_act_fwd_from_partials": [_vp, _i32, _vp, _vp, _vp, _vp, _vp, _vp, _vp, _vp, _vp, _i32, _f32, _u32, _vp, _i32, _i32, _i32, _i32, _vp,
+                                      _i32, _i32, _i64, _vp],
     "rtts_bn_act_fwd": [_vp, _vp, _vp, _vp, _vp, _i32, _f32, _u32, _vp, _i32, _i32, _i32, _i32, _vp, _i32, _i32, _i64, _vp],
     "rtts_bn_act_bwd": [_vp, _vp, _i32, _vp, _vp, _vp, _vp, _i32, _f32, _u32, _vp, _i32, _i32, _i32, _i32, _vp, _i32, _i64, _vp, _vp, _vp, _vp],
     "rtts_bn_moments": [_vp, _i32, _i32, _i32, _i32, _vp, _vp, _vp],
@@ -143,6 +145,7 @@
     "rtts_infer_metrics": [_vp, _i64, _i64, _i64, _i32, _vp, _vp, _i64, _i64, _i64, _vp, _i32, _vp, _vp, _vp, _i32, _i32, _i32, _i32, _vp, _vp, _vp,
                            _vp, _vp],
     "rtts_adamw_step": [_vp, _vp, _vp, _vp, _vp, _i64, _vp, _vp, _f32, _f32, _f32, _f32, _vp, _vp],
+    "rtts_clip_adamw_step": [_vp, _vp, _vp, _vp, _vp, _i64, _f32, _f32, _vp, _vp, _vp, _f32, _f32, _f32, _f32, _vp, _vp],
     "rtts_mel_frames": [_i64, _i32],
     "rtts_mel_spectrogram": [_vp, C.POINTER(_i64), C.POINTER(_i64), _vp, _vp, _i32, _vp, _vp, _i32, _i32, _i32, _i32, _f32, _vp, _i64, _vp],
     "rtts_resample_len": [_i64, _i32, _i32],
diff --git a/reformer-tts_amd/csrc/edges.hip b/reformer-tts_amd/csrc/edges.hip
--- a/reformer-tts_amd/csrc/edges.hip
+++ b/reformer-tts_amd/csrc/edges.hip
@@ -210,6 +210,22 @@
     }
 }
 
+__device__ __forceinline__ void ed_bn_stats(float s, float q, int M, float& mu, float& var, float& rs) {
+    mu = s / M;
+    var = fmaxf(q / M - mu * mu, 0.f);
+    rs = rsqrtf(var + 1e-5f);
+}
+__device__ __forceinline__ void ed_bn_store_stats(float mu, float var, float rs, int M, int c, float* __restrict__ mean, float* __restrict__ rstd,
+                                                  float* __restrict__ run_mean, float* __restrict__ run_var,
+                                                  const float* __restrict__ mean_shift) {
+    mean[c] = mu;
+    rstd[c] = rs;
+    if (run_mean) {
+        run_mean[c] = 0.9f * run_mean[c] + 0.1f * (mu + (mean_shift ? mean_shift[c] : 0.f));
+        run_var[c] = 0.9f * run_var[c] + 0.1f * var * ((float)M / (float)(M > 1 ? M - 1 : 1));
+    }
+}
+
 __global__ __launch_bounds__(64 * ED_FIN_WAVES) void bn_finalize_stats_kernel(const float* __restrict__ partial, int nrows, int M, int C,
                                                                        float* __restrict__ mean, float* __restrict__ rstd,
                                                                        float* __restrict__ run_mean, float* __restrict__ run_var,
@@ -220,14 +236,9 @@
     ed_reduce_partials(partial, nrows, C, c, s, q, red);
     if (num_batches && blockIdx.x == 0 && threadIdx.x == 0) num_batches[0] += 1;
     if (threadIdx.x >= 64 || c >= C) return;
-    const float mu = s / M;
-    const float var = fmaxf(q / M - mu * mu, 0.f);
-    mean[c] = mu;
-    rstd[c] = rsqrtf(var + 1e-5f);
-    if (run_mean) {
-        run_mean[c] = 0.9f * run_mean[c] + 0.1f * (mu + (mean_shift ? mean_shift[c] : 0.f));
-        run_var[c] = 0.9f * run_var[c] + 0.1f * var * ((float)M / (float)(M > 1 ? M - 1 : 1));
-    }
+    float mu, var, rs;
+    ed_bn_stats(s, q, M, mu, var, rs);
+    ed_bn_store_stats(mu, var, rs, M, c, mean, rstd, run_mean, run_var, mean_shift);
 }
 
 __global__ __launch_bounds__(64 * ED_FIN_WAVES) void bn_finalize_bwd_kernel(const float* __restrict__ partial, int nrows, int C,
@@ -268,6 +279,14 @@
         run_mean[c] = 0.9f * run_mean[c] + 0.1f * (mu + (mean_shift ? mean_shift[c] : 0.f));
         run_var[c] = 0.9f * run_var[c] + 0.1f * var * (count / (count > 1.f ? count - 1.f : 1.f));
     }
+}
+
+__device__ __forceinline__ float ed_bn_act_fwd_elem(float y, float mu, float rs, float ga, float be, int act, uint32_t seed, uint32_t idx,
+                                                    uint32_t thresh, float dscale) {
+    const float pre = __builtin_fmaf((y - mu) * rs, ga, be);
+    float a = act == 1 ? fmaxf(pre, 0.f) : ed_tanh(pre);
+    if (thresh) a *= ed_drop(seed, idx, thresh, dscale);
+    return a;
 }
 
 __global__ __launch_bounds__(ED_THREADS) void bn_act_fwd_kernel(const float* __restrict__ y, const float* __restrict__ mean,
@@ -302,16 +321,98 @@
             const float ga[4] = {g4.x, g4.y, g4.z, g4.w}, be[4] = {b4.x, b4.y, b4.z, b4.w};
             float o[4];
 #pragma unroll
-            for (int j = 0; j < 4; ++j) {
-                const float pre = __builtin_fmaf((yy[j] - mu[j]) * rs[j], ga[j], be[j]);
-                float a = act == 1 ? fmaxf(pre, 0.f) : ed_tanh(pre);
-                if (thresh) a *= ed_drop(seed, (uint32_t)(e + j), thresh, dscale);
-                o[j] = a;
-            }
+            for (int j = 0; j < 4; ++j) o[j] = ed_bn_act_fwd_elem(yy[j], mu[j], rs[j], ga[j], be[j], act, seed, (uint32_t)(e + j), thresh, dscale);
             pk.x = pack_bf16x2(o[0], o[1]);
             pk.y = pack_bf16x2(o[2], o[3]);
         }
         reinterpret_cast<uint2*>(z)[i] = pk;
+    }
+}
+
+#define ED_FOLD_THREADS (64 * ED_FIN_WAVES)
+#define ED_FOLD_PRE 2
+__device__ __forceinline__ bool ed_z_src(const EdHalo& g, int z_halo, int z_lead, long long zr, long long& ym) {
+    if (z_halo) {
+        int b, t;
+        ym = zr - z_lead;
+        return ed_valid(g, ym, b, t);
+    }
+    const long long b = zr / g.L;
+    ym = b * g.P + g.H + (zr - b * g.L);
+    return true;
+}
+__global__ __launch_bounds__(ED_FOLD_THREADS) void bn_act_fwd_fold_kernel(const float* __restrict__ partial, int nrows, int M,
+                                                                          const float* __restrict__ y, float* __restrict__ mean,
+                                                                          float* __restrict__ rstd, float* __restrict__ run_mean,
+                                                                          float* __restrict__ run_var, const float* __restrict__ mean_shift,
+                                                                          long long* __restrict__ num_batches, const float* __restrict__ gamma,
+                                                                          const float* __restrict__ beta, int act, uint32_t seed,
+                                                                          const uint32_t* __restrict__ seed_dev, uint32_t thresh, float dscale, EdHalo g,
+                                                                          int z_halo, int z_lead, long long z_rows, int C, bf16_t* __restrict__ z) {
+    __shared__ float red[2][ED_FIN_WAVES][64];
+    __shared__ float stat[2][64];
+    if (seed_dev) seed += seed_dev[0];
+    const int cg = blockIdx.y * 64;
+    const int cl = (threadIdx.x & 15) * 4, c = cg + cl;
+    const long long zr0 = (long long)blockIdx.x * 64 + (threadIdx.x >> 4), zstep = (long long)gridDim.x * 64;
+    float4 py[ED_FOLD_PRE];
+    long long pe[ED_FOLD_PRE];
+#pragma unroll
+    for (int k = 0; k < ED_FOLD_PRE; ++k) {
+        const long long zr = zr0 + k * zstep;
+        long long ym;
+        pe[k] = -1;
+        py[k] = make_float4(0.f, 0.f, 0.f, 0.f);
+        if (c < C && zr < z_rows && ed_z_src(g, z_halo, z_lead, zr, ym)) {
+            pe[k] = ym * C + c;
+            py[k] = *reinterpret_cast<const float4*>(y + pe[k]);
+        }
+    }
+    {
+        const int c = cg + (threadIdx.x & 63);
+        float s, q;
+        ed_reduce_partials(partial, nrows, C, c, s, q, red);
+        if (num_batches && blockIdx.x == 0 && blockIdx.y == 0 && threadIdx.x == 0) num_batches[0] += 1;
+        if (threadIdx.x < 64) {
+            float mu = 0.f, var = 0.f, rs = 0.f;
+            if (c < C) {
+                ed_bn_stats(s, q, M, mu, var, rs);
+                if (blockIdx.x == 0) ed_bn_store_stats(mu, var, rs, M, c, mean, rstd, run_mean, run_var, mean_shift);
+            }
+            stat[0][threadIdx.x] = mu;
+            stat[1][threadIdx.x] = rs;
+        }
+        __syncthreads();
+    }
+    if (c >= C) return;
+    const float4 g4 = *reinterpret_cast<const float4*>(gamma + c), b4 = *reinterpret_cast<const float4*>(beta + c);
+    const float mu[4] = {stat[0][cl], stat[0][cl + 1], stat[0][cl + 2], stat[0][cl + 3]};
+    const float rs[4] = {stat[1][cl], stat[1][cl + 1], stat[1][cl + 2], stat[1][cl + 3]};
+    const float ga[4] = {g4.x, g4.y, g4.z, g4.w}, be[4] = {b4.x, b4.y, b4.z, b4.w};
+    auto emit = [&](long long zr, long long e, const float4& yv) {
+        uint2 pk = make_uint2(0u, 0u);
+        if (e >= 0) {
+            const float yy[4] = {yv.x, yv.y, yv.z, yv.w};
+            float o[4];
+#pragma unroll
+            for (int j = 0; j < 4; ++j) o[j] = ed_bn_act_fwd_elem(yy[j], mu[j], rs[j], ga[j], be[j], act, seed, (uint32_t)(e + j), thresh, dscale);
+            pk.x = pack_bf16x2(o[0], o[1]);
+            pk.y = pack_bf16x2(o[2], o[3]);
+        }
+        *reinterpret_cast<uint2*>(z + (size_t)zr * C + c) = pk;
+    };
+#pragma unroll
+    for (int k = 0; k < ED_FOLD_PRE; ++k)
+        if (zr0 + k * zstep < z_rows) emit(zr0 + k * zstep, pe[k], py[k]);
+#pragma unroll 2
+    for (long long zr = zr0 + ED_FOLD_PRE * zstep; zr < z_rows; zr += zstep) {
+        long long ym, e = -1;
+        float4 yv = make_float4(0.f, 0.f, 0.f, 0.f);
+        if (ed_z_src(g, z_halo, z_lead, zr, ym)) {
+            e = ym * C + c;
+            yv = *reinterpret_cast<const float4*>(y + e);
+        }
+        emit(zr, e, yv);
     }
 }
 
@@ -536,26 +637,53 @@
     }
 }
 
+#define EMB_GROUPS 8
 __global__ __launch_bounds__(ED_THREADS) void embedding_bwd_kernel(const int64_t* __restrict__ ids, const float* __restrict__ dx, int64_t bstride,
                                                                    int64_t rstride, int L, int rows,
                                                                    int C, int padding_idx, float* __restrict__ dE, uint32_t seed,
                                                                    const uint32_t* __restrict__ seed_dev, uint32_t thresh, float dscale) {
     __shared__ float red[4][64];
+    __shared__ int list[4][EMB_GROUPS * 64];
     const int id = blockIdx.x;
     const int lane = threadIdx.x & 63, wave = threadIdx.x >> 6;
     const int c = blockIdx.y * 64 + lane;
     if (id == padding_idx) return;
     if (thresh && seed_dev) seed += seed_dev[0];
     float acc = 0.f;
-    for (int base = wave * 64; base < rows; base += 4 * 64) {
-        const int r = base + lane;
-        unsigned long long m = __ballot(r < rows && ids[r] == (int64_t)id);
-        while (m) {
-            const int rr = base + __builtin_ctzll(m);
-            m &= m - 1;
-            const int bb = rr / L;
-            if (c < C) acc += dx[(size_t)bb * bstride + (size_t)(rr - bb * L) * rstride + c] * (thresh ? rtts_drop_keep(seed, (uint32_t)rr * C + c, thresh, dscale) : 1.f);
-        }
+    for (int g0 = wave; g0 * 64 < rows; g0 += 4 * EMB_GROUPS) {
+        unsigned long long mk[EMB_GROUPS];
+#pragma unroll
+        for (int j = 0; j < EMB_GROUPS; ++j) {
+            const int r = (g0 + 4 * j) * 64 + lane;
+            mk[j] = __ballot(r < rows && ids[r] == (int64_t)id);
+        }
+        int n = 0;
+#pragma unroll
+        for (int j = 0; j < EMB_GROUPS; ++j) {
+            if ((mk[j] >> lane) & 1ull) list[wave][n + __popcll(mk[j] & ((1ull << lane) - 1ull))] = (g0 + 4 * j) * 64 + lane;
+            n += __popcll(mk[j]);
+        }
+        __builtin_amdgcn_fence(__ATOMIC_RELEASE, "wavefront");
+        __builtin_amdgcn_wave_barrier();
+        __builtin_amdgcn_fence(__ATOMIC_ACQUIRE, "wavefront");
+        for (int i0 = 0; i0 < n; i0 += 8) {
+            float v[8], k[8];
+#pragma unroll
+            for (int u = 0; u < 8; ++u) {
+                v[u] = 0.f;
+                k[u] = 0.f;
+                if (i0 + u < n && c < C) {
+                    const int rr = list[wave][i0 + u];
+                    const int bb = rr / L;
+                    v[u] = dx[(size_t)bb * bstride + (size_t)(rr - bb * L) * rstride + c];
+                    k[u] = thresh ? rtts_drop_keep(seed, (uint32_t)rr * C + c, thresh, dscale) : 1.f;
+                }
+            }
+#pragma unroll
+            for (int u = 0; u < 8; ++u)
+                if (i0 + u < n && c < C) acc += v[u] * k[u];
+        }
+        __builtin_amdgcn_wave_barrier();
     }
     red[wave][lane] = acc;
     __syncthreads();
@@ -824,6 +952,33 @@
     hipLaunchKernelGGL(bn_act_fwd_kernel, dim3(ed_grid(n4)), dim3(ED_THREADS), 0, (hipStream_t)stream, y, mean, rstd, gamma, beta, act, seed, seed_dev,
                        ed_thresh(drop_p), 1.f / (1.f - drop_p), g, z_halo, z_lead, n4, C, ed_cshift(C), (bf16_t*)z);
     RTTS_LAUNCH_CHECK("rtts_bn_act_fwd");
+    return 0;
+}
+
+static inline dim3 ed_fold_grid(int64_t rows, int C) {
+    const int groups = (C + 63) / 64;
+    int64_t slabs = (rows + 63) / 64;
+    const int64_t cap = groups >= 256 ? 1 : 256 / groups;
+    if (slabs > cap) slabs = cap;
+    if (slabs < 1) slabs = 1;
+    return dim3((unsigned)slabs, (unsigned)groups);
+}
+
+extern "C" int rtts_bn_act_fwd_from_partials(const float* partial, int nrows, const float* y, float* mean, float* rstd, float* run_mean,
+                                             float* run_var, const float* mean_shift, int64_t* num_batches, const float* gamma,
+                                             const float* beta, int act, float drop_p, uint32_t seed, const uint32_t* seed_dev, int B, int L,
+                                             int halo, int C, void* z, int z_halo, int z_lead, int64_t z_rows, void* stream) {
+    RTTS_ENTER(stream);
+    RTTS_REQUIRE(partial && nrows > 0 && y && mean && rstd && gamma && beta && z && B > 0 && L > 0 && halo >= 0 && C > 0 && C % 4 == 0 &&
+                     (act == 1 || act == 2) && drop_p >= 0.f && drop_p < 1.f, "rtts_bn_act_fwd_from_partials: bad arguments");
+    const EdHalo g = ed_halo(B, L, halo);
+    RTTS_REQUIRE(z_halo ? (halo > 0 && z_lead >= 0 && z_rows >= z_lead + (int64_t)B * g.P) : (z_rows == (int64_t)B * L && z_lead == 0),
+                 "rtts_bn_act_fwd_from_partials: z must be a halo array with room for B*(L+2*halo) rows behind its lead-in, or B*L plain rows");
+    RTTS_REQUIRE((size_t)z_rows * C / 4 < (1ull << 30), "rtts_bn_act_fwd_from_partials: more than 2^32 elements");
+    hipLaunchKernelGGL(bn_act_fwd_fold_kernel, ed_fold_grid(z_rows, C), dim3(ED_FOLD_THREADS), 0, (hipStream_t)stream, partial, nrows, B * L, y, mean,
+                       rstd, run_mean, run_var, mean_shift, (long long*)num_batches, gamma, beta, act, seed, seed_dev, ed_thresh(drop_p),
+                       1.f / (1.f - drop_p), g, z_halo, z_lead, (long long)z_rows, C, (bf16_t*)z);
+    RTTS_LAUNCH_CHECK("rtts_bn_act_fwd_from_partials");
     return 0;
 }
 
@@ -954,7 +1109,8 @@
 extern "C" int rtts_embedding_bwd(const int64_t* ids, const float* dx, int rows, int C, int n_embeddings, int padding_idx, float* dE,
                                   float drop_p, uint32_t seed, const uint32_t* seed_dev, void* stream) {
     RTTS_ENTER(stream);
-    RTTS_REQUIRE(ids && dx && dE && rows > 0 && C > 0 && n_embeddings > 0 && drop_p >= 0.f && drop_p < 1.f, "rtts_embedding_bwd: bad arguments");
+    RTTS_REQUIRE(ids && dx && dE && rows > 0 && rows <= (1 << 30) && C > 0 && n_embeddings > 0 && drop_p >= 0.f && drop_p < 1.f,
+                 "rtts_embedding_bwd: bad arguments");
     hipLaunchKernelGGL(embedding_bwd_kernel, dim3(n_embeddings, (C + 63) / 64), dim3(ED_THREADS), 0, (hipStream_t)stream,
                        ids, dx, (int64_t)0, (int64_t)C, rows, rows, C, padding_idx, dE, seed, seed_dev, ed_thresh(drop_p), 1.f / (1.f - drop_p));
     RTTS_LAUNCH_CHECK("rtts_embedding_bwd");
@@ -965,7 +1121,7 @@
                                           int n_embeddings, int padding_idx, float* dE, float drop_p, uint32_t seed, const uint32_t* seed_dev,
                                           void* stream) {
     RTTS_ENTER(stream);
-    RTTS_REQUIRE(ids && dx && dE && rows > 0 && L > 0 && rows % L == 0 && C > 0 && row_stride >= C && batch_stride >= 0 && n_embeddings > 0 &&
+    RTTS_REQUIRE(ids && dx && dE && rows > 0 && rows <= (1 << 30) && L > 0 && rows % L == 0 && C > 0 && row_stride >= C && batch_stride >= 0 && n_embeddings > 0 &&
                      drop_p >= 0.f && drop_p < 1.f, "rtts_embedding_bwd_strided: bad arguments");
     hipLaunchKernelGGL(embedding_bwd_kernel, dim3(n_embeddings, (C + 63) / 64), dim3(ED_THREADS), 0, (hipStream_t)stream,
                        ids, dx, batch_stride, row_stride, L, rows, C, padding_idx, dE, seed, seed_dev, ed_thresh(drop_p), 1.f / (1.f - drop_p));
@@ -1037,27 +1193,44 @@
 __global__ __launch_bounds__(256) void batch_masks_kernel(const int64_t* __restrict__ phonemes, int64_t ph_stride, int B, int Lp, int Lp_pad,
                                                           const float* __restrict__ loss_mask, int64_t lm_bstride, int64_t lm_rstride, int Lm,
                                                           int Lm_pad, int n_mels, int64_t* __restrict__ pad_ph, uint8_t* __restrict__ ph_mask,
-                                                          uint8_t* __restrict__ ph_not, uint8_t* __restrict__ sp_mask) {
-    const int per_b = Lp_pad + Lm_pad;
-    for (int i = blockIdx.x * blockDim.x + threadIdx.x; i < B * per_b; i += gridDim.x * blockDim.x) {
-        const int b = i / per_b, j = i % per_b;
-        if (j < Lp_pad) {
+                                                          uint8_t* __restrict__ ph_not, uint8_t* __restrict__ sp_mask, int ph_blocks) {
+    if ((int)blockIdx.x < ph_blocks) {
+        const int i = blockIdx.x * blockDim.x + threadIdx.x;
+        if (i < B * Lp_pad) {
+            const int b = i / Lp_pad, j = i % Lp_pad;
             const int64_t v = j < Lp ? phonemes[(int64_t)b * ph_stride + j] : 0;
-            pad_ph[(size_t)b * Lp_pad + j] = v;
-            ph_mask[(size_t)b * Lp_pad + j] = v != 0;
-            ph_not[(size_t)b * Lp_pad + j] = v == 0;
-        } else {
-            const int t = j - Lp_pad;
-            bool on = false;
-            if (t < Lm) {
-                const float* row = loss_mask + (int64_t)b * lm_bstride + (int64_t)t * lm_rstride;
-                float sum = 0.f;
-                for (int c = 0; c < n_mels; ++c) sum += row[c];
-                on = (sum / (float)n_mels) != 0.f;
-            }
-            sp_mask[(size_t)b * Lm_pad + t] = on;
-        }
-    }
+            pad_ph[i] = v;
+            ph_mask[i] = v != 0;
+            ph_not[i] = v == 0;
+        }
+        return;
+    }
+    __shared__ float tile[64][65];
+    const int mb = blockIdx.x - ph_blocks, tiles = (Lm_pad + 63) / 64;
+    const int b = mb / tiles, t0 = (mb % tiles) * 64;
+    const int lane = threadIdx.x & 63, wave = threadIdx.x >> 6;
+    const float* base = loss_mask + (int64_t)b * lm_bstride;
+    float sum = 0.f;
+    for (int c0 = 0; c0 < n_mels; c0 += 64) {
+        const int cw = n_mels - c0 < 64 ? n_mels - c0 : 64;
+        float x[16];
+#pragma unroll
+        for (int u = 0; u < 16; ++u) {
+            const int r = wave + 4 * u;
+            x[u] = (t0 + r < Lm && lane < cw) ? base[(int64_t)(t0 + r) * lm_rstride + c0 + lane] : 0.f;
+        }
+#pragma unroll
+        for (int u = 0; u < 16; ++u) tile[wave + 4 * u][lane] = x[u];
+        __syncthreads();
+        if (threadIdx.x < 64) {
+#pragma unroll 8
+            for (int c = 0; c < cw; ++c) sum += tile[threadIdx.x][c];
+        }
+        __syncthreads();
+    }
+    const int t = t0 + threadIdx.x;
+    if (threadIdx.x < 64 && t < Lm_pad)
+        sp_mask[(size_t)b * Lm_pad + t] = t < Lm && (sum / (float)n_mels) != 0.f;
 }
 
 extern "C" int rtts_batch_masks(const int64_t* phonemes, int64_t ph_stride, int B, int Lp, int Lp_pad, const float* loss_mask, int64_t lm_bstride,
@@ -1066,9 +1239,10 @@
     RTTS_ENTER(stream);
     RTTS_REQUIRE(phonemes && loss_mask && pad_phonemes && phoneme_mask && phoneme_pad_mask && frame_mask, "rtts_batch_masks: null pointer");
     RTTS_REQUIRE(B > 0 && Lp > 0 && Lp_pad >= Lp && Lm > 0 && Lm_pad >= Lm && n_mels > 0 && ph_stride >= Lp, "rtts_batch_masks: bad shape");
-    const int n = B * (Lp_pad + Lm_pad);
-    hipLaunchKernelGGL(batch_masks_kernel, dim3((n + 255) / 256), dim3(256), 0, (hipStream_t)stream, phonemes, ph_stride, B, Lp, Lp_pad, loss_mask,
-                       lm_bstride, lm_rstride, Lm, Lm_pad, n_mels, pad_phonemes, phoneme_mask, phoneme_pad_mask, frame_mask);
+    RTTS_REQUIRE((int64_t)B * Lp_pad < (1ll << 31) && (int64_t)B * Lm_pad < (1ll << 31), "rtts_batch_masks: more than 2^31 positions");
+    const int ph_blocks = (int)(((int64_t)B * Lp_pad + 255) / 256), mel_blocks = B * ((Lm_pad + 63) / 64);
+    hipLaunchKernelGGL(batch_masks_kernel, dim3(ph_blocks + mel_blocks), dim3(256), 0, (hipStream_t)stream, phonemes, ph_stride, B, Lp, Lp_pad,
+                       loss_mask, lm_bstride, lm_rstride, Lm, Lm_pad, n_mels, pad_phonemes, phoneme_mask, phoneme_pad_mask, frame_mask, ph_blocks);
     RTTS_LAUNCH_CHECK("rtts_batch_masks");
     return 0;
 }
diff --git a/reformer-tts_amd/csrc/optim.hip b/reformer-tts_amd/csrc/optim.hip
--- a/reformer-tts_amd/csrc/optim.hip
+++ b/reformer-tts_amd/csrc/optim.hip
@@ -26,29 +26,57 @@
     if (threadIdx.x == 0) partial[blockIdx.x] = red[0] + red[1] + red[2] + red[3];
 }
 
-__global__ __launch_bounds__(OPT_THREADS) void clip_scale_kernel(const float* __restrict__ partial, int nblocks, float grad_mult,
-                                                                 float max_norm, float* __restrict__ scale) {
+__device__ __forceinline__ void opt_clip_scale(const float* __restrict__ partial, int nblocks, float grad_mult, float max_norm, float* red,
+                                               float& gs, float& norm) {
     float s = 0.f;
-    for (int i = threadIdx.x; i < nblocks; i += OPT_THREADS) s += partial[i];
-    __shared__ float red[OPT_THREADS / 64];
+    for (int i0 = threadIdx.x; i0 < nblocks; i0 += 8 * OPT_THREADS) {
+        float x[8];
+#pragma unroll
+        for (int u = 0; u < 8; ++u) x[u] = i0 + u * OPT_THREADS < nblocks ? partial[i0 + u * OPT_THREADS] : 0.f;
+#pragma unroll
+        for (int u = 0; u < 8; ++u)
+            if (i0 + u * OPT_THREADS < nblocks) s += x[u];
+    }
 #pragma unroll
     for (int o = 32; o > 0; o >>= 1) s += __shfl_xor(s, o);
     if ((threadIdx.x & 63) == 0) red[threadIdx.x >> 6] = s;
     __syncthreads();
+    norm = sqrtf(red[0] + red[1] + red[2] + red[3]) * grad_mult;
+    float c = 1.f;
+    if (max_norm > 0.f) c = fminf(1.f, max_norm / (norm + 1e-6f));
+    gs = grad_mult * c;
+}
+
+__global__ __launch_bounds__(OPT_THREADS) void clip_scale_kernel(const float* __restrict__ partial, int nblocks, float grad_mult,
+                                                                 float max_norm, float* __restrict__ scale) {
+    __shared__ float red[OPT_THREADS / 64];
+    float gs, norm;
+    opt_clip_scale(partial, nblocks, grad_mult, max_norm, red, gs, norm);
     if (threadIdx.x == 0) {
-        const float norm = sqrtf(red[0] + red[1] + red[2] + red[3]) * grad_mult;
-        float c = 1.f;
-        if (max_norm > 0.f) c = fminf(1.f, max_norm / (norm + 1e-6f));
-        scale[0] = grad_mult * c;
+        scale[0] = gs;
         scale[1] = norm;
     }
 }
 
+template <bool CLIP>
 __global__ __launch_bounds__(OPT_THREADS) void adamw_kernel(float* __restrict__ p, const float* __restrict__ g, float* __restrict__ m,
                                                             float* __restrict__ v, const uint8_t* __restrict__ decay, size_t n4,
                                                             const float* __restrict__ scale, const float* __restrict__ hyper,
-                                                            float b1, float b2, float eps, float wd, bf16_t* __restrict__ mirror) {
-    const float gs = scale ? scale[0] : 1.f;
+                                                            float b1, float b2, float eps, float wd, bf16_t* __restrict__ mirror,
+                                                            const float* __restrict__ partial, int nblocks, float grad_mult, float max_norm,
+                                                            float* __restrict__ scale_out) {
+    float gs;
+    if (CLIP) {
+        __shared__ float red[OPT_THREADS / 64];
+        float norm;
+        opt_clip_scale(partial, nblocks, grad_mult, max_norm, red, gs, norm);
+        if (blockIdx.x == 0 && threadIdx.x == 0) {
+            scale_out[0] = gs;
+            scale_out[1] = norm;
+        }
+    } else {
+        gs = scale ? scale[0] : 1.f;
+    }
     const float lr = hyper[0], step_size = hyper[1];
     for (size_t i = (size_t)blockIdx.x * blockDim.x + threadIdx.x; i < n4; i += (size_t)gridDim.x * blockDim.x) {
         const float4 g4 = reinterpret_cast<const float4*>(g)[i];
@@ -106,8 +134,29 @@
                  "rtts_adamw_step: buffers must be 16-byte aligned (decay mask 4, mirror 8)");
     int blocks = (int)((n / 4 + OPT_THREADS - 1) / OPT_THREADS);
     if (blocks > OPT_MAX_BLOCKS) blocks = OPT_MAX_BLOCKS;
-    hipLaunchKernelGGL(adamw_kernel, dim3(blocks), dim3(OPT_THREADS), 0, (hipStream_t)stream, params, grads, exp_avg, exp_avg_sq,
-                       decay_mask, (size_t)n / 4, scale, hyper, beta1, beta2, eps, weight_decay, (bf16_t*)bf16_mirror);
+    hipLaunchKernelGGL(adamw_kernel<false>, dim3(blocks), dim3(OPT_THREADS), 0, (hipStream_t)stream, params, grads, exp_avg, exp_avg_sq,
+                       decay_mask, (size_t)n / 4, scale, hyper, beta1, beta2, eps, weight_decay, (bf16_t*)bf16_mirror, (const float*)nullptr, 0,
+                       1.f, 0.f, (float*)nullptr);
     RTTS_LAUNCH_CHECK("rtts_adamw_step");
     return 0;
 }
+
+extern "C" int rtts_clip_adamw_step(float* params, const float* grads, float* exp_avg, float* exp_avg_sq, const uint8_t* decay_mask,
+                                    int64_t n, float grad_mult, float max_norm, float* partial_ws, float* scale_out, const float* hyper,
+                                    float beta1, float beta2, float eps, float weight_decay, void* bf16_mirror, void* stream) {
+    RTTS_ENTER(stream);
+    RTTS_REQUIRE(params && grads && exp_avg && exp_avg_sq && decay_mask && partial_ws && scale_out && hyper && n > 0,
+                 "rtts_clip_adamw_step: bad arguments");
+    RTTS_REQUIRE(n % 4 == 0, "rtts_clip_adamw_step: n must be a multiple of 4 (pad the flat buffers)");
+    RTTS_REQUIRE((((uintptr_t)params | (uintptr_t)grads | (uintptr_t)exp_avg | (uintptr_t)exp_avg_sq) & 15) == 0 &&
+                     ((uintptr_t)decay_mask & 3) == 0 && ((uintptr_t)bf16_mirror & 7) == 0,
+                 "rtts_clip_adamw_step: buffers must be 16-byte aligned (decay mask 4, mirror 8)");
+    int blocks = (int)((n / 4 + OPT_THREADS - 1) / OPT_THREADS);
+    if (blocks > OPT_MAX_BLOCKS) blocks = OPT_MAX_BLOCKS;
+    hipLaunchKernelGGL(sumsq_partial_kernel, dim3(blocks), dim3(OPT_THREADS), 0, (hipStream_t)stream, grads, (size_t)n, partial_ws);
+    hipLaunchKernelGGL(adamw_kernel<true>, dim3(blocks), dim3(OPT_THREADS), 0, (hipStream_t)stream, params, grads, exp_avg, exp_avg_sq,
+                       decay_mask, (size_t)n / 4, (const float*)nullptr, hyper, beta1, beta2, eps, weight_decay, (bf16_t*)bf16_mirror,
+                       (const float*)partial_ws, blocks, grad_mult, max_norm, scale_out);
+    RTTS_LAUNCH_CHECK("rtts_clip_adamw_step");
+    return 0;
+}
diff --git a/reformer-tts_amd/edges.py b/reformer-tts_amd/edges.py
--- a/reformer-tts_amd/edges.py
+++ b/reformer-tts_amd/edges.py
@@ -185,13 +185,10 @@
         mean = torch.empty(c, dtype=torch.float32, device=dev)
         rstd = torch.empty(c, dtype=torch.float32, device=dev)
         bn = self.bn
-        if fused:
-            _lib.call("rtts_bn_stats_from_partials", partial.data_ptr(), nrows, g.b, g.l, c, mean.data_ptr(), rstd.data_ptr(),
-                      bn.running_mean.data_ptr(), bn.running_var.data_ptr(), self.c.conv.bias.data_ptr(), bn.num_batches_tracked.data_ptr(), _s())
-        elif SYNC_BN is None:
+        if not fused and SYNC_BN is None:
             _lib.call("rtts_bn_stats", y.data_ptr(), g.b, g.l, g.H, c, mean.data_ptr(), rstd.data_ptr(), bn.running_mean.data_ptr(),
                       bn.running_var.data_ptr(), self.c.conv.bias.data_ptr(), bn.num_batches_tracked.data_ptr(), _ws(dev, c).data_ptr(), _s())
-        else:
+        elif not fused:
             import torch.distributed as dist
             mom = torch.empty(2 * c + 1, dtype=torch.float32, device=dev)
             _lib.call("rtts_bn_moments", y.data_ptr(), g.b, g.l, g.H, c, mom.data_ptr(), _ws(dev, c).data_ptr(), _s())
@@ -206,8 +203,14 @@
         else:
             z = g.new(c, dev)
             zargs = (1, g.LEAD, g.alloc)
-        _lib.call("rtts_bn_act_fwd", y.data_ptr(), mean.data_ptr(), rstd.data_ptr(), bn.weight.data_ptr(), bn.bias.data_ptr(), self.act,
-                  self.p, seed, seed_base(dev).data_ptr(), g.b, g.l, g.H, c, z.data_ptr(), *zargs, _s())
+        if fused:
+            _lib.call("rtts_bn_act_fwd_from_partials", partial.data_ptr(), nrows, y.data_ptr(), mean.data_ptr(), rstd.data_ptr(),
+                      bn.running_mean.data_ptr(), bn.running_var.data_ptr(), self.c.conv.bias.data_ptr(), bn.num_batches_tracked.data_ptr(),
+                      bn.weight.data_ptr(), bn.bias.data_ptr(), self.act, self.p, seed, seed_base(dev).data_ptr(), g.b, g.l, g.H, c,
+                      z.data_ptr(), *zargs, _s())
+        else:
+            _lib.call("rtts_bn_act_fwd", y.data_ptr(), mean.data_ptr(), rstd.data_ptr(), bn.weight.data_ptr(), bn.bias.data_ptr(), self.act,
+                      self.p, seed, seed_base(dev).data_ptr(), g.b, g.l, g.H, c, z.data_ptr(), *zargs, _s())
         return z, (xh, y, mean, rstd, seed)
 
     def backward(self, dz, dz_halo: bool, saved, g: Halo, need_dx=True, dx_f32=False):
diff --git a/reformer-tts_amd/training/trainer.py b/reformer-tts_amd/training/trainer.py
--- a/reformer-tts_amd/training/trainer.py
+++ b/reformer-tts_amd/training/trainer.py
@@ -397,11 +397,17 @@
         self.global_step += 1
         n = self.flat_p.numel()
         stream = torch.cuda.current_stream().cuda_stream
-        _lib.call("rtts_grad_clip_scale", self.flat_g.data_ptr(), n, 1.0 / self.world, float(self.cfg.gradient_clip_val),
-                  self.ws_partial.data_ptr(), self.ws_scale.data_ptr(), stream)
-        _lib.call("rtts_adamw_step", self.flat_p.data_ptr(), self.flat_g.data_ptr(), self.flat_m.data_ptr(),
-                  self.flat_v.data_ptr(), self.decay_mask.data_ptr(), n, self.ws_scale.data_ptr(), self.hyper.data_ptr(), 0.9, 0.999,
-                  1e-6, float(self.cfg.weight_decay), self.flat_pb.data_ptr(), stream)
+        if self.world == 1:
+            _lib.call("rtts_clip_adamw_step", self.flat_p.data_ptr(), self.flat_g.data_ptr(), self.flat_m.data_ptr(),
+                      self.flat_v.data_ptr(), self.decay_mask.data_ptr(), n, 1.0, float(self.cfg.gradient_clip_val),
+                      self.ws_partial.data_ptr(), self.ws_scale.data_ptr(), self.hyper.data_ptr(), 0.9, 0.999, 1e-6,
+                      float(self.cfg.weight_decay), self.flat_pb.data_ptr(), stream)
+        else:
+            _lib.call("rtts_grad_clip_scale", self.flat_g.data_ptr(), n, 1.0 / self.world, float(self.cfg.gradient_clip_val),
+                      self.ws_partial.data_ptr(), self.ws_scale.data_ptr(), stream)
+            _lib.call("rtts_adamw_step", self.flat_p.data_ptr(), self.flat_g.data_ptr(), self.flat_m.data_ptr(),
+                      self.flat_v.data_ptr(), self.decay_mask.data_ptr(), n, self.ws_scale.data_ptr(), self.hyper.data_ptr(), 0.9, 0.999,
+                      1e-6, float(self.cfg.weight_decay), self.flat_pb.data_ptr(), stream)
         from ..engine import WEIGHT_EPOCH
         WEIGHT_EPOCH[0] += 1
 
```

Result: no change. 1.969 million mel-frames/s (median of 6 runs) (+0.5%).
